# sthaha/kepler

Hardware: AMD Instinct MI355X
Metric: process attributions/sec + achieved HBM GB/s, 10k-node fleet, 1/2/4/8 MI355X (higher is better)
Workload: dtype f64+u64; 1 GPU; config3: 10000-node fleet x 2000 procs, Z=4; fleet_nodes=10000, nodes_per_gpu=10000, procs_per_gpu=20000000, containers_per_gpu=1970000, vms_per_gpu=200000, pods_per_gpu=700000, zones=4, namespaces=10000, allreduce_every=8

## Files before the change

kepler_amd/csrc/kacc_derive.hpp:

```cpp
#pragma once

#include <hip/hip_runtime.h>
#include <stdint.h>

#include "kacc_internal.hpp"

namespace kacc {

struct ProcDerive {
  const double *ratio;
  const uint32_t *node;
  const uint64_t *active_energy;
  const double *active_power;
  const double *cpu_delta;
  uint64_t nodes;
  uint32_t zones;
};

__device__ __forceinline__ double proc_power(const ProcDerive &d, uint64_t s, uint32_t z) {
  const uint32_t n = d.node[s];
  if (n >= d.nodes) return 0.0;
  const uint64_t i = static_cast<uint64_t>(n) * d.zones + z;
  const double aP = d.active_power[i];
  if (d.active_energy[i] == 0 || !(d.cpu_delta[n] != 0) || !(aP != 0)) return 0.0;
  return d.ratio[s] * aP;
}

}

inline kacc::ProcDerive kacc_derive(const kacc_ctx *ctx, kacc_kind kind) {
  kacc::ProcDerive d;
  const int tr = kind == KACC_KIND_CTR ? KACC_T_CTR_RATIO : kind == KACC_KIND_VM ? KACC_T_VM_RATIO : KACC_T_PROC_RATIO;
  d.ratio = static_cast<const double *>(ctx->tables[tr]);
  d.node = static_cast<const uint32_t *>(ctx->tables[tr + 1]);
  d.active_energy = static_cast<const uint64_t *>(ctx->tables[KACC_T_NODE_ACTIVE_ENERGY]);
  d.active_power = static_cast<const double *>(ctx->tables[KACC_T_NODE_ACTIVE_POWER]);
  d.cpu_delta = static_cast<const double *>(ctx->tables[KACC_T_NODE_CPU_DELTA]);
  d.nodes = ctx->cfg.nodes;
  d.zones = ctx->cfg.zones;
  return d;
}
inline kacc::ProcDerive kacc_proc_derive(const kacc_ctx *ctx) { return kacc_derive(ctx, KACC_KIND_PROC); }

inline int kacc_derived_kind(int t) {
  return t == KACC_T_PROC_POWER ? KACC_KIND_PROC : t == KACC_T_CTR_POWER ? KACC_KIND_CTR
                                                 : t == KACC_T_VM_POWER ? KACC_KIND_VM : -1;
}

extern "C" int kacc_internal_derived_power(kacc_ctx *ctx, int t, uint64_t first, uint64_t count, double *out,
                                           void *stream);
```

kepler_amd/csrc/kacc_device.hpp:

```cpp
#pragma once

#include <hip/hip_runtime.h>
#include <stdint.h>

namespace kacc {

constexpr double kTwo63 = 9223372036854775808.0;

__device__ __forceinline__ int64_t cvttsd2sq(double x) {
  if (!(x >= -kTwo63 && x < kTwo63)) return INT64_MIN;
  return static_cast<int64_t>(x);
}

__device__ __forceinline__ uint64_t go_f64_to_u64(double x) {
  if (__builtin_expect(x > -1.0 && x < 4294967296.0, 1)) return static_cast<uint32_t>(x);
  if (x < kTwo63) return static_cast<uint64_t>(cvttsd2sq(x));
  return static_cast<uint64_t>(cvttsd2sq(x - kTwo63)) | 0x8000000000000000ull;
}

__device__ __forceinline__ double u2f(uint64_t v) { return static_cast<double>(v); }

__device__ __forceinline__ int64_t go_sub_mono(int64_t t, int64_t u) {
  int64_t d;
  if (__builtin_sub_overflow(t, u, &d)) return t > u ? INT64_MAX : INT64_MIN;
  return d;
}

__device__ __forceinline__ double go_duration_seconds(int64_t d) {
  const int64_t sec = d / 1000000000LL;
  const int64_t nsec = d % 1000000000LL;
  return static_cast<double>(sec) + static_cast<double>(nsec) / 1e9;
}

__device__ __forceinline__ uint64_t energy_delta(uint64_t cur, uint64_t prev, uint64_t max_j) {
  if (cur >= prev) return cur - prev;
  if (max_j > 0) return (max_j - prev) + cur;
  return 0;
}

}
```

kepler_amd/csrc/kacc_engine.hip:

```cpp
#include <hip/hip_runtime.h>

#include <algorithm>
#include <atomic>
#include <thread>
#include <type_traits>
#include <cstdarg>
#include <cstddef>
#include <cstdio>
#include <cstring>
#include <mutex>
#include <string>
#include <vector>

#include "../../include/kepler_accel.h"
#include "kacc_debug.h"
#include "kacc_derive.hpp"
#include "kacc_device.hpp"
#include "kacc_internal.hpp"

namespace kacc {

constexpr int kTree = 256;
constexpr int kRowsLds = 2048;
constexpr int kBlock = 256;
// ... 51 lines not shown
#define KACC_CHUNK_WAVES 4
#endif
constexpr int kChunkThreads = KACC_CHUNK_THREADS;
constexpr int kChunkRpt = 4;
constexpr int kChunkRows = kChunkRpt * kChunkThreads;
static_assert(kChunkRows <= kRowsLds, "a chunk's rows are staged like a fast node's");
constexpr uint32_t kChunkGrid = 256u * 4u * KACC_CHUNK_WAVES / (kChunkThreads / 64);

template <int V>
constexpr int kTpb = 512;
template <int V>
constexpr int kRpt = kRowsLds / kTpb<V>;

constexpr uint32_t kErrNode = 1u << 0;
constexpr uint32_t kErrOffsets = 1u << 1;
constexpr uint32_t kErrSlot = 1u << 2;
constexpr uint32_t kErrNs = 1u << 3;
constexpr uint32_t kErrCapacity = 1u << 4;
constexpr uint32_t kErrBigNode = 1u << 5;
static_assert(kRowsLds == KACC_FAST_MAX_PROCS && kTpb<0> == KACC_FAST_MAX_AGGREGATES,
              "KACC_FAST_* must match the fast path's capacity");

struct ChunkItem {
  uint32_t node, chunk, nchunks, ctr_begin, vm_begin, pod_begin, pad[2];
};

constexpr int kColLoads = 8;
#ifndef KACC_COL_SPLIT_FROM
#define KACC_COL_SPLIT_FROM 16384
#endif
#ifndef KACC_COL_SPLIT_NODES
#define KACC_COL_SPLIT_NODES 4096
#endif
constexpr uint64_t kColSplitFrom = KACC_COL_SPLIT_FROM, kColSplitNodes = KACC_COL_SPLIT_NODES;
struct NodeTotalsArgs {
  uint64_t n_nodes;
  const uint64_t *active_total, *idle_total;
  const double *power, *active_power, *idle_power;
  const uint64_t *node_export;
  uint64_t *out_e;
  double *out_p;
  uint32_t split;
  uint64_t *part;
  uint32_t *arrived;
};

struct DevState {
  uint64_t *node_energy_total, *node_active_energy, *node_active_total, *node_idle_total;
  double *node_power, *node_active_power, *node_idle_power;
  int64_t *node_ts;
  uint32_t *node_has_prev;
  double *node_usage_ratio, *node_cpu_delta;
  uint32_t *node_status;
  uint64_t *proc_energy;
  double *proc_ratio;
  uint32_t *proc_node;
  uint64_t *ctr_energy;
  double *ctr_ratio, *ctr_cpu_delta, *ctr_cpu_total;
  uint32_t *ctr_node;
  uint64_t *vm_energy;
  double *vm_ratio, *vm_cpu_delta;
  uint32_t *vm_node;
  uint64_t *pod_energy;
  double *pod_power, *pod_cpu_delta, *pod_cpu_total;
  uint64_t proc_slots, ctr_slots, vm_slots, pod_slots;
  uint32_t *err;
  uint2 *defer;
  uint32_t *defer_ctr;
  uint32_t defer_cap;
  ChunkItem *items;
  uint32_t *item_ctr;
  uint32_t item_cap;
  uint32_t items_given, keep_items;
  uint64_t *stamps;
};

struct NodeShared {
  uint64_t active_energy[KACC_MAX_ZONES];
  double power[KACC_MAX_ZONES];
  double active_power[KACC_MAX_ZONES];
  double node_delta;
  uint32_t first;
};

__device__ __forceinline__ void raise_err(uint32_t *err, uint32_t bit) { atomicOr(err, bit); }

__device__ __forceinline__ uint64_t uniform_u64(uint64_t x) {
  const uint32_t lo = __builtin_amdgcn_readfirstlane(static_cast<uint32_t>(x));
  const uint32_t hi = __builtin_amdgcn_readfirstlane(static_cast<uint32_t>(x >> 32));
  return (static_cast<uint64_t>(hi) << 32) | lo;
}
__device__ __forceinline__ double uniform_f64(double x) {
  return __longlong_as_double(static_cast<long long>(uniform_u64(static_cast<uint64_t>(__double_as_longlong(x)))));
}
__device__ __forceinline__ uint32_t uniform_u32(uint32_t x) { return __builtin_amdgcn_readfirstlane(x); }

#ifndef KACC_FAST_EXTRA_LDS
#define KACC_FAST_EXTRA_LDS 0
#endif
#ifndef KACC_WT_PROC
#define KACC_WT_PROC 0
#endif
#ifndef KACC_WT_AGG
#define KACC_WT_AGG 0
#endif
template <typename T>
__device__ __forceinline__ void wt_store(T v, T *p) {
  if constexpr (sizeof(T) == 16)
    asm volatile("global_store_dwordx4 %0, %1, off sc0 sc1 nt" ::"v"(p), "v"(v) : "memory");
  else if constexpr (sizeof(T) == 8)
    asm volatile("global_store_dwordx2 %0, %1, off sc0 sc1 nt" ::"v"(p), "v"(v) : "memory");
  else
    asm volatile("global_store_dword %0, %1, off sc0 sc1 nt" ::"v"(p), "v"(v) : "memory");
}
template <typename T>
__device__ __forceinline__ void nt_store(T v, T *p) {
  if constexpr (KACC_WT_PROC != 0)
    wt_store(v, p);
  else
    __builtin_nontemporal_store(v, p);
}

template <int Z>
__device__ __forceinline__ void load_row(const uint64_t *__restrict__ base, uint64_t s,
                                         uint64_t (&out)[Z]) {
  if constexpr (Z % 2 == 0) {
    using u64x2 = __attribute__((ext_vector_type(2))) unsigned long long;
    const u64x2 *p = reinterpret_cast<const u64x2 *>(base + s * Z);
#pragma unroll
    for (int k = 0; k < Z / 2; ++k) {
      const u64x2 x = p[k];
      out[2 * k] = x.x;
      out[2 * k + 1] = x.y;
    }
  } else {
#pragma unroll
    for (int z = 0; z < Z; ++z) out[z] = base[s * Z + z];
  }
}

template <int Z>
__device__ __forceinline__ void load_row_f64(const double *__restrict__ base, uint64_t s,
                                             double (&out)[Z]) {
  if constexpr (Z % 2 == 0) {
    using f64x2 = __attribute__((ext_vector_type(2))) double;
    const f64x2 *p = reinterpret_cast<const f64x2 *>(base + s * Z);
#pragma unroll
    for (int k = 0; k < Z / 2; ++k) {
      const f64x2 x = p[k];
      out[2 * k] = x.x;
      out[2 * k + 1] = x.y;
    }
  } else {
#pragma unroll
    for (int z = 0; z < Z; ++z) out[z] = base[s * Z + z];
  }
}

template <int Z, bool NT, typename T>
__device__ __forceinline__ void store_row(T *__restrict__ base, uint64_t s, const T (&in)[Z]) {
  if constexpr (Z % 2 == 0) {
    using v2 = __attribute__((ext_vector_type(2))) T;
    v2 *p = reinterpret_cast<v2 *>(base + s * Z);
#pragma unroll
    for (int k = 0; k < Z / 2; ++k) {
      v2 x;
      x.x = in[2 * k];
      x.y = in[2 * k + 1];
      if constexpr (NT)
        nt_store(x, p + k);
      else
        p[k] = x;
    }
  } else {
#pragma unroll
    for (int z = 0; z < Z; ++z) {
      if constexpr (NT)
        nt_store(in[z], base + s * Z + z);
      else
        base[s * Z + z] = in[z];
    }
  }
}

constexpr uint64_t kPodRowScale = 2;
__device__ __forceinline__ uint64_t pod_row(uint64_t s) { return s * kPodRowScale; }
__device__ __forceinline__ uint64_t agg_row(uint32_t role, uint64_t s) { return role == 3 ? pod_row(s) : s; }

template <int Z>
struct Attr {
  uint64_t aE[Z];
  double aP[Z];
  uint32_t live;
  uint32_t live_pod;
  double nd;
  uint32_t first;
  uint32_t keep_node;
};

template <int Z>
__device__ __forceinline__ Attr<Z> make_attr(const NodeShared &sh, uint32_t flags) {
  Attr<Z> a;
  a.nd = uniform_f64(sh.node_delta);
  a.first = uniform_u32(sh.first);
  a.keep_node = (flags & KACC_F_STABLE_SLOT_NODES) && !a.first ? 1u : 0u;
  a.live = 0;
  a.live_pod = 0;
#pragma unroll
  for (int z = 0; z < Z; ++z) {
    a.aE[z] = uniform_u64(sh.active_energy[z]);
    a.aP[z] = uniform_f64(sh.active_power[z]);
    const double pw = uniform_f64(sh.power[z]);
    const bool ok = a.aE[z] != 0 && a.nd != 0;
    if (ok && a.aP[z] != 0) a.live |= 1u << z;
    if (ok && (a.first ? a.aP[z] : pw) != 0) a.live_pod |= 1u << z;
  }
  return a;
}

template <int Z>
__device__ __forceinline__ double attribute_row(const Attr<Z> &a, uint32_t live, double delta,
                                                bool is_new, const uint64_t (&prev)[Z],
                                                uint64_t (&E)[Z], double (&P)[Z]) {
  const double ratio = delta / a.nd;
#pragma unroll
  for (int z = 0; z < Z; ++z) {
    if (live & (1u << z)) {
      const uint64_t e = go_f64_to_u64(ratio * u2f(a.aE[z]));
      E[z] = a.first ? e : e + (is_new ? 0ull : prev[z]);
      P[z] = a.first ? 0.0 : ratio * a.aP[z];
    } else {
      E[z] = 0;
      P[z] = 0.0;
    }
  }
  return ratio;
}

template <int Z>
__device__ __forceinline__ double attribute_proc(const Attr<Z> &a, double delta, bool is_new,
                                                 const uint64_t (&prev)[Z], uint64_t (&E)[Z]) {
  const double ratio = delta / a.nd;
#pragma unroll
  for (int z = 0; z < Z; ++z) {
    if (a.live & (1u << z)) {
      const uint64_t e = go_f64_to_u64(ratio * u2f(a.aE[z]));
      E[z] = a.first ? e : e + (is_new ? 0ull : prev[z]);
    } else {
      E[z] = 0;
    }
  }
  return ratio;
}

template <int Z, bool NT>
__device__ __forceinline__ void store_proc(const DevState &st, uint64_t s, const uint64_t (&E)[Z], double ratio,
                                           uint32_t node, bool wnode) {
  store_row<Z, NT, uint64_t>(st.proc_energy, s, E);
  if constexpr (NT) {
    nt_store(ratio, st.proc_ratio + s);
    if (wnode) nt_store(node, st.proc_node + s);
  } else {
    st.proc_ratio[s] = ratio;
    if (wnode) st.proc_node[s] = node;
  }
}

__device__ __forceinline__ uint32_t export_row(const kacc_interval &b, uint32_t q, uint32_t *err) {
  if (!b.pod_export_pos) return q;
  const uint32_t r = b.pod_export_pos[q];
  if (r >= b.n_pods) {
    atomicOr(err, 1u << 1);
    return ~0u;
  }
  return r;
}
template <int Z>
__device__ __forceinline__ void export_pod_at(const kacc_interval &b, uint32_t row, const uint64_t (&E)[Z],
                                              const double (&P)[Z]) {
  if (!b.pod_export || row == ~0u) return;
  uint64_t *o = b.pod_export + static_cast<uint64_t>(row) * (2 * Z);
  store_row<Z, false, uint64_t>(o, 0, E);
  store_row<Z, false, double>(reinterpret_cast<double *>(o), 1, P);
}
template <int Z>
__device__ __forceinline__ void export_pod(const kacc_interval &b, uint32_t q, const uint64_t (&E)[Z],
                                           const double (&P)[Z], uint32_t *err) {
  if (!b.pod_export) return;
  export_pod_at<Z>(b, export_row(b, q, err), E, P);
}
template <int Z>
__device__ __forceinline__ void export_pod_zero(const kacc_interval &b, uint32_t q, uint32_t *err) {
  uint64_t E[Z];
  double P[Z];
#pragma unroll
  for (int z = 0; z < Z; ++z) {
    E[z] = 0;
    P[z] = 0.0;
  }
  export_pod<Z>(b, q, E, P, err);
}
template <int Z>
__device__ __forceinline__ void export_node_zone(const kacc_interval &b, uint32_t n, uint32_t z, uint64_t at,
                                                 uint64_t it, double p, double ap, double ip) {
  if (!b.node_export) return;
  uint64_t *o = b.node_export + static_cast<uint64_t>(n) * (5 * Z) + z;
  o[0] = at;
  o[Z] = it;
  o[2 * Z] = static_cast<uint64_t>(__double_as_longlong(p));
  o[3 * Z] = static_cast<uint64_t>(__double_as_longlong(ap));
  o[4 * Z] = static_cast<uint64_t>(__double_as_longlong(ip));
// ... 23 lines not shown
  if constexpr (KACC_WT_AGG != 0 && !NT) {
    if (role == 3) {
      wt_row<Z, uint64_t>(st.pod_energy, pod_row(s), E);
      wt_row<Z, double>(st.pod_power, pod_row(s), P);
      return;
    }
    wt_row<Z, uint64_t>(role == 1 ? st.ctr_energy : st.vm_energy, s, E);
    wt_store(ratio, (role == 1 ? st.ctr_ratio : st.vm_ratio) + s);
    wt_store(node, (role == 1 ? st.ctr_node : st.vm_node) + s);
    return;
  }
  if (role == 3) {
    store_row<Z, NT, uint64_t>(st.pod_energy, pod_row(s), E);
    store_row<Z, NT, double>(st.pod_power, pod_row(s), P);
    return;
  }
  store_row<Z, NT, uint64_t>(role == 1 ? st.ctr_energy : st.vm_energy, s, E);
  double *r = role == 1 ? st.ctr_ratio : st.vm_ratio;
  uint32_t *nd = role == 1 ? st.ctr_node : st.vm_node;
  if constexpr (NT) {
    nt_store(ratio, r + s);
    nt_store(node, nd + s);
  } else {
    r[s] = ratio;
    nd[s] = node;
  }
}

template <int kB>
__device__ __forceinline__ void segment_load(const double *s_d, uint32_t i, uint32_t e, double (&v)[kB]) {
#pragma unroll
  for (int u = 0; u < kB; ++u) v[u] = s_d[min(i + u, e - 1)];
}
template <int kB>
__device__ __forceinline__ void segment_add(const double (&v)[kB], uint32_t i, uint32_t e, double &delta,
                                            double &total) {
#pragma unroll
  for (int u = 0; u < kB; ++u) {
    const double x = i + u < e ? v[u] : 0.0;
    delta = delta + x;
    total = total + x;
  }
}
template <int kB>
__device__ __forceinline__ void segment_sum(const double *s_d, uint32_t i, uint32_t e, double &delta,
                                            double &total) {
  for (; i < e; i += kB) {
    double v[kB];
    segment_load<kB>(s_d, i, e, v);
    segment_add<kB>(v, i, e, delta, total);
  }
}
template <int Z, bool kMasked, bool kNtLoad = false>
__device__ __forceinline__ void load_group_masked(const uint64_t *__restrict__ base, uint64_t s0,
                                                  uint32_t len, uint64_t safe, uint64_t (&out)[Z]) {
  using u64x2 = __attribute__((ext_vector_type(2))) unsigned long long;
  constexpr int kHalf = Z / 2;
  const uint32_t lane = threadIdx.x & 63u;
  const u64x2 *p = reinterpret_cast<const u64x2 *>(base + s0 * Z);
  const u64x2 *q = reinterpret_cast<const u64x2 *>(base + safe * Z);
#pragma unroll
  for (int j = 0; j < kHalf; ++j) {
    const uint32_t piece = lane + 64u * j;
    if constexpr (!kMasked) {
      const u64x2 x = kNtLoad ? __builtin_nontemporal_load(p + piece) : p[piece];
      out[2 * j] = x.x;
      out[2 * j + 1] = x.y;
      continue;
    }
    const bool ok = piece / kHalf < len;
    const u64x2 *src = ok ? p + piece : q;
    const u64x2 x = kNtLoad ? __builtin_nontemporal_load(src) : *src;
    out[2 * j] = ok ? x.x : 0ull;
    out[2 * j + 1] = ok ? x.y : 0ull;
  }
}

template <int Z, bool NT, bool kInv>
__device__ __forceinline__ void attribute_group_masked(const Attr<Z> &a, const NodeShared &sh,
                                                       const double *s_d, const uint32_t *s_w,
                                                       const uint16_t *s_inv,
                                                       uint32_t row0, uint64_t s0, uint32_t len,
                                                       const uint64_t (&prev)[Z],
                                                       uint64_t *__restrict__ energy,
                                                       double *__restrict__ ratio_tab,
                                                       uint32_t *__restrict__ node_tab, uint32_t node) {
  using u64x2 = __attribute__((ext_vector_type(2))) unsigned long long;
  constexpr int kHalf = Z / 2;
  const uint32_t lane = threadIdx.x & 63u;
  u64x2 *pe = reinterpret_cast<u64x2 *>(energy + s0 * Z);
#pragma unroll
  for (int j = 0; j < kHalf; ++j) {
    const uint32_t piece = lane + 64u * j;
    const uint32_t idx = piece / kHalf;
    const uint32_t zp = piece % kHalf;
    uint32_t row = row0 + idx;
    if constexpr (kInv) {
      if (idx >= len) continue;
      row = s_inv[row];
      if (row == 0xffffu) continue;
    }
    const uint32_t wr = s_w[row];
    const bool is_new = (wr & KACC_SLOT_NEW) != 0;
    const double ratio = s_d[row] / a.nd;
    uint64_t E[2];
#pragma unroll
    for (int h = 0; h < 2; ++h) {
      const uint32_t z = 2 * zp + h;
      const uint64_t aE = sh.active_energy[z];
      if (a.live & (1u << z)) {
        const uint64_t e = go_f64_to_u64(ratio * u2f(aE));
        E[h] = a.first ? e : e + (is_new ? 0ull : prev[2 * j + h]);
      } else {
        E[h] = 0;
      }
    }
    u64x2 ev;
    ev.x = E[0];
    ev.y = E[1];
    if constexpr (NT)
      nt_store(ev, pe + piece);
    else
      pe[piece] = ev;
    if (zp == 0) {
      const bool wnode = !a.keep_node || is_new;
      if constexpr (NT) {
        nt_store(ratio, ratio_tab + s0 + idx);
        if (wnode) nt_store(node, node_tab + s0 + idx);
      } else {
        ratio_tab[s0 + idx] = ratio;
        if (wnode) node_tab[s0 + idx] = node;
      }
    }
  }
}

template <int Z>
__device__ __forceinline__ void node_zone(const kacc_interval &b, const DevState &st, uint32_t n,
                                          int z, NodeShared &sh) {
  const bool first = st.node_has_prev[n] == 0u;
  const uint64_t i = static_cast<uint64_t>(n) * Z + z;
  const double ratio = b.node_usage_ratio[n];
  const uint64_t abs_e = b.zone_energy[i];
  uint64_t active;
  double p = 0.0, ap = 0.0, ip = 0.0;
  uint64_t at, it;
  if (first) {
    active = go_f64_to_u64(u2f(abs_e) * ratio);
    at = active;
    it = abs_e - active;
  } else {
    const double dt = go_duration_seconds(go_sub_mono(b.node_ts_ns[n], st.node_ts[n]));
    const uint64_t delta = energy_delta(abs_e, st.node_energy_total[i], b.zone_max[i]);
    active = go_f64_to_u64(u2f(delta) * ratio);
    at = st.node_active_total[i] + active;
    it = st.node_idle_total[i] + (delta - active);
    p = u2f(delta) / dt;
    ap = p * ratio;
    ip = p - ap;
  }
  st.node_active_total[i] = at;
  st.node_idle_total[i] = it;
  export_node_zone<Z>(b, n, static_cast<uint32_t>(z), at, it, p, ap, ip);
  st.node_energy_total[i] = abs_e;
  st.node_active_energy[i] = active;
  st.node_power[i] = p;
  st.node_active_power[i] = ap;
  st.node_idle_power[i] = ip;
  sh.active_energy[z] = active;
  sh.power[z] = p;
  sh.active_power[z] = ap;
  if (z == 0) sh.first = first ? 1u : 0u;
}

struct NodeRanges {
  uint32_t p0, p1, c0, c1, v0, v1, q0, q1;
};

template <int Z>
__device__ __forceinline__ void export_skipped(const kacc_interval &b, const DevState &st, uint32_t n,
                                               const NodeRanges &r, uint32_t lane, uint32_t nlanes) {
  if (b.node_export) {
    for (uint32_t z = lane; z < static_cast<uint32_t>(Z); z += nlanes) {
      const uint64_t i = static_cast<uint64_t>(n) * Z + z;
      export_node_zone<Z>(b, n, z, st.node_active_total[i], st.node_idle_total[i], st.node_power[i],
                          st.node_active_power[i], st.node_idle_power[i]);
    }
// ... 295 lines not shown
  double d[kRowsPerThread];
  uint32_t w[kRowsPerThread];
#pragma unroll
  for (int k = 0; k < kRowsPerThread; ++k) {
    const uint32_t r = tid + k * kThreads;
    const bool in = r < rows;
    if constexpr (kNtLd) {
      d[k] = in ? __builtin_nontemporal_load(dcpu + r) : 0.0;
      w[k] = in ? __builtin_nontemporal_load(pslot + r) : 0xffffffffu;
    } else {
      d[k] = in ? dcpu[r] : 0.0;
      w[k] = in ? pslot[r] : 0xffffffffu;
    }
  }
  const uint32_t utid = static_cast<uint32_t>(tid);
  auto role_of = [&]() -> uint32_t {
    if ((V & kVarSkipAggregates) != 0) return 0u;
    return utid < nc ? 1u : utid < nc + nv ? 2u : utid < nc + nv + nq ? 3u : 0u;
  };
  auto index_of = [&]() -> uint32_t {
    return utid < nc ? utid : utid < nc + nv ? utid - nc : utid - nc - nv;
  };
  uint32_t a_beg = 0, a_end = 0, a_w = 0xffffffffu;
  {
    const uint32_t role = role_of(), j = index_of();
    if (role == 1) {
      a_beg = j == 0 ? p0 : b.ctr_proc_end[c0 + j - 1];
      a_end = b.ctr_proc_end[c0 + j];
      a_w = b.ctr_slot[c0 + j];
    } else if (role == 2) {
      a_beg = j == 0 ? (nc ? b.ctr_proc_end[c1 - 1] : p0) : b.vm_proc_end[v0 + j - 1];
      a_end = b.vm_proc_end[v0 + j];
      a_w = b.vm_slot[v0 + j];
    } else if (role == 3) {
      a_beg = j == 0 ? c0 : b.pod_ctr_end[q0 + j - 1];
      a_end = b.pod_ctr_end[q0 + j];
      a_w = b.pod_slot[q0 + j];
    }
  }
  auto a_cap = [&]() -> uint64_t {
    const uint32_t role = role_of();
    return role == 1 ? st.ctr_slots : role == 2 ? st.vm_slots : role == 3 ? st.pod_slots : 0;
  };
  const uint32_t a_s = a_w & KACC_SLOT_MASK;
  auto a_ok_f = [&]() -> bool { return role_of() != 0 && a_s < a_cap(); };
  const bool a_ok = a_ok_f();
  const uint32_t role = role_of();
  const uint32_t j = index_of();
  auto a_energy = [&]() { return role == 1 ? st.ctr_energy : role == 2 ? st.vm_energy : st.pod_energy; };
  auto a_cpu_total = [&]() { return role == 1 ? st.ctr_cpu_total : st.pod_cpu_total; };
  auto a_cpu_delta = [&]() {
    return role == 1 ? st.ctr_cpu_delta : role == 2 ? st.vm_cpu_delta : st.pod_cpu_delta;
  };
  uint64_t prev[kRowsPerThread][Z];
  uint32_t contig = 0;
  constexpr bool kSweepable =
      kTransposed<Z> && (V & (kVarNoTranspose | kVarNoSweep | kVarSkipProcs)) == 0;
  constexpr bool kRowSweep = !kTransposed<Z> && (V & (kVarNoSweep | kVarSkipProcs)) == 0;
  uint32_t smin = 0, span = 0;
  bool sweep = false;
  if constexpr (kSweepable || kRowSweep) {
    if (b.node_proc_span) {
      const uint32_t lo = uniform_u32(b.node_proc_span[2 * n]);
      const uint32_t hi = uniform_u32(b.node_proc_span[2 * n + 1]);
      sweep = rows > 0 && hi >= lo && hi - lo < static_cast<uint32_t>(kRowsLds) && hi < st.proc_slots;
      smin = lo;
      span = hi - lo + 1;
      if (sweep) {
#pragma unroll
        for (int k = 0; k < kRowsPerThread; ++k) s_inv[tid + k * kThreads] = 0xffffu;
      }
    }
  }
  const bool swept = (kSweepable || kRowSweep) && sweep;
  if constexpr ((V & kVarSkipProcs) == 0) {
    if (swept) {
      if constexpr (kRowSweep) {
#pragma unroll
        for (int k = 0; k < kRowsPerThread; ++k)
          load_row<Z>(st.proc_energy, static_cast<uint64_t>(smin) + min(tid + k * kThreads, span - 1), prev[k]);
      }
      if constexpr (kSweepable) {
#pragma unroll
        for (int k = 0; k < kRowsPerThread; ++k) {
          const uint32_t pos0 = static_cast<uint32_t>(tid & ~63) + k * kThreads;
          const uint32_t len = pos0 < span ? min(span - pos0, 64u) : 0u;
          load_group_masked<Z, true, kNtLd>(st.proc_energy, static_cast<uint64_t>(smin) + pos0, len, smin,
                                     prev[k]);
        }
      }
    } else {
#pragma unroll
      for (int k = 0; k < kRowsPerThread; ++k) {
        const uint64_t sl = w[k] & KACC_SLOT_MASK;
        if constexpr (kTransposed<Z> && (V & kVarNoTranspose) == 0) {
          const uint64_t g0 = uniform_u32(static_cast<uint32_t>(sl));
          if (__all((tid + k * kThreads) < rows && sl == g0 + (tid & 63) && g0 + 64 <= st.proc_slots)) {
            contig |= 1u << k;
            load_group_masked<Z, false, kNtLd>(st.proc_energy, g0, 64u, g0, prev[k]);
            continue;
          }
        }
        if (sl < st.proc_slots) {
          load_row<Z>(st.proc_energy, sl, prev[k]);
        } else {
#pragma unroll
          for (int z = 0; z < Z; ++z) prev[k][z] = 0;
        }
      }
    }
  }
  uint64_t a_prev[Z];
  double a_total = 0.0;
  if (a_ok) {
    if constexpr (!kLateAgg<V>) load_row<Z>(a_energy(), agg_row(role, a_s), a_prev);
    if (role != 2 && !(a_w & KACC_SLOT_NEW)) a_total = a_cpu_total()[a_s];
  } else {
#pragma unroll
    for (int z = 0; z < Z; ++z) a_prev[z] = 0;
  }
  if (role != 0 && !a_ok) raise_err(st.err, kErrSlot);

#pragma unroll
  for (int k = 0; k < kRowsPerThread; ++k) {
    const uint32_t r = tid + k * kThreads;
    if (r < rows) {
      s_d[r] = d[k];
      s_w[r] = w[k];
    }
  }
  __syncthreads();
  if constexpr (kStamp) {
    if (tid == 0) stamp[1] = __builtin_amdgcn_s_memrealtime();
  }
  if (swept) {
#pragma unroll
    for (int k = 0; k < kRowsPerThread; ++k) {
      const uint32_t r = tid + k * kThreads;
      if (r >= rows) continue;
      const uint32_t sl = s_w[r] & KACC_SLOT_MASK;
      if (sl - smin < span && sl < st.proc_slots)
        s_inv[sl - smin] = static_cast<uint16_t>(r);
      else
        raise_err(st.err, kErrSlot);
    }
  }
  if (b.flags & KACC_F_NODE_CPU_DELTA_GIVEN) {
    if (tid == 0) sh.node_delta = b.node_cpu_delta[n];
  } else {
    if (tid < kTree) {
      double v[kRowsLds / kTree];
#pragma unroll
      for (int u = 0; u < kRowsLds / kTree; ++u) v[u] = s_d[tid + kTree * u];
      double s = 0.0;
#pragma unroll
      for (int u = 0; u < kRowsLds / kTree; ++u) s = s + (tid + kTree * u < rows ? v[u] : 0.0);
      red[tid] = s;
// ... 56 lines not shown
    st.node_ts[n] = b.node_ts_ns[n];
    st.node_has_prev[n] = 1u;
    st.node_usage_ratio[n] = a.first ? 0.0 : b.node_usage_ratio[n];
    st.node_cpu_delta[n] = a.nd;
    st.node_status[n] = a.first ? KACC_NODE_FIRST_READ : KACC_NODE_OK;
  }
  constexpr uint32_t kStageWords = kRowsLds;
  const bool stage = kLateAgg<V> && (V & kVarSkipAggregates) == 0 && b.pod_export && !b.pod_export_pos &&
                     nq * 2u * Z <= kStageWords;
  uint64_t *s_stage = reinterpret_cast<uint64_t *>(s_d);
  auto aggregate_out = [&]() {
    if (!a_ok) {
      if (role == 3) {
        if (stage) {
#pragma unroll
          for (int z = 0; z < 2 * Z; ++z) s_stage[j * 2 * Z + z] = 0;
        } else {
          export_pod_zero<Z>(b, q0 + j, st.err);
        }
      }
      return;
    }
    if constexpr (kLateAgg<V>) load_row<Z>(a_energy(), agg_row(role, a_s), a_prev);
    const uint32_t xrow = role == 3 && b.pod_export && !stage ? export_row(b, q0 + j, st.err) : ~0u;
    uint64_t E[Z];
    double P[Z];
    const double ratio = attribute_row<Z>(a, role == 3 ? a.live_pod : a.live, a_delta,
                                          (a_w & KACC_SLOT_NEW) != 0, a_prev, E, P);
    store_agg<Z, kNtAgg>(st, role, a_s, E, P, ratio, n);
    if (role == 3) {
      if (stage) {
#pragma unroll
        for (int z = 0; z < Z; ++z) {
          s_stage[j * 2 * Z + z] = E[z];
          s_stage[j * 2 * Z + Z + z] = static_cast<uint64_t>(__double_as_longlong(P[z]));
        }
      } else {
        export_pod_at<Z>(b, xrow, E, P);
      }
    }
  };
  if constexpr (!kLateAgg<V>) aggregate_out();
  if (swept) {
    if constexpr (kRowSweep) {
#pragma unroll
      for (int k = 0; k < kRowsPerThread; ++k) {
        const uint32_t pos = tid + k * kThreads;
        if (pos >= span) continue;
        const uint32_t r = s_inv[pos];
        if (r == 0xffffu) continue;
        const uint32_t wk = s_w[r];
        uint64_t E[Z];
        const double ratio = attribute_proc<Z>(a, s_d[r], (wk & KACC_SLOT_NEW) != 0, prev[k], E);
        store_proc<Z, kNT>(st, static_cast<uint64_t>(smin) + pos, E, ratio, n, !a.keep_node || (wk & KACC_SLOT_NEW));
      }
    }
    if constexpr (kSweepable) {
#pragma unroll
      for (int k = 0; k < kRowsPerThread; ++k) {
        const uint32_t pos0 = static_cast<uint32_t>(tid & ~63) + k * kThreads;
        const uint32_t len = pos0 < span ? min(span - pos0, 64u) : 0u;
        attribute_group_masked<Z, kNT, true>(a, sh, s_d, s_w, s_inv, pos0,
                                             static_cast<uint64_t>(smin) + pos0, len, prev[k],
                                             st.proc_energy, st.proc_ratio, st.proc_node, n);
      }
    }
  } else if constexpr ((V & kVarSkipProcs) == 0) {
#pragma unroll
    for (int k = 0; k < kRowsPerThread; ++k) {
      const uint32_t r = tid + k * kThreads;
      if constexpr (kTransposed<Z> && (V & kVarNoTranspose) == 0) {
        if (contig & (1u << k)) {
          const uint32_t pos0 = r - (tid & 63);
          attribute_group_masked<Z, kNT, false>(a, sh, s_d, s_w, s_inv, pos0,
                                                uniform_u32(s_w[pos0] & KACC_SLOT_MASK), 64u, prev[k],
                                                st.proc_energy, st.proc_ratio, st.proc_node, n);
          continue;
        }
      }
      if (r >= rows) continue;
      const uint32_t wk = s_w[r];
      const uint64_t sl = wk & KACC_SLOT_MASK;
      if (sl >= st.proc_slots) {
        raise_err(st.err, kErrSlot);
        continue;
      }
      uint64_t E[Z];
      const double ratio = attribute_proc<Z>(a, s_d[r], (wk & KACC_SLOT_NEW) != 0, prev[k], E);
      store_proc<Z, kNtScat>(st, sl, E, ratio, n, !a.keep_node || (wk & KACC_SLOT_NEW));
    }
  }
  if (stage) __syncthreads();
  if constexpr (kLateAgg<V>) aggregate_out();
  if (stage) {
    __syncthreads();
    using u64x2 = __attribute__((ext_vector_type(2))) unsigned long long;
    const u64x2 *src = reinterpret_cast<const u64x2 *>(s_stage);
    u64x2 *dst = reinterpret_cast<u64x2 *>(b.pod_export + static_cast<uint64_t>(q0) * (2 * Z));
    for (uint32_t i = utid; i < nq * Z; i += kThreads) nt_store(src[i], dst + i);
  }
  if constexpr (kStamp) {
    __syncthreads();
    if (tid == 0) stamp[3] = __builtin_amdgcn_s_memrealtime();
  }
}

template <int Z, int V>
#ifndef KACC_FAST_WAVES
#define KACC_FAST_WAVES 6
#endif
__global__ __launch_bounds__(kTpb<V>, Z > 4 ? 2 : KACC_FAST_WAVES)
void interval_kernel(const kacc_interval b, const DevState st) {
  interval_node<Z, V>(b, st, blockIdx.x);
}

template <int Z, int V>
__global__ __launch_bounds__(kTpb<V>, Z > 4 ? 2 : KACC_FAST_WAVES)
void interval_sums_kernel(const kacc_interval b, const DevState st, const SumsArgs sa) {
  if (blockIdx.x < sa.node_blocks) {
    sums_block<Z, kTpb<V>>(sa, blockIdx.x, st.err);
    return;
  }
  const uint32_t x = blockIdx.x - sa.node_blocks;
  if (x >= b.n_nodes) {
    sums_block<Z, kTpb<V>>(sa, sa.node_blocks + (x - b.n_nodes), st.err);
    return;
  }
  interval_node<Z, V>(b, st, x);
}

constexpr int kCarryMaxZ = 2;

__device__ __forceinline__ void lds_barrier() {
  __builtin_amdgcn_fence(__ATOMIC_RELEASE, "workgroup", "local");
  __builtin_amdgcn_s_barrier();
  __builtin_amdgcn_fence(__ATOMIC_ACQUIRE, "workgroup", "local");
}

#define KACC_GLOBAL __attribute__((address_space(1)))
template <typename T>
__device__ __forceinline__ const T KACC_GLOBAL *gbl(const T *p) {
  return (const T KACC_GLOBAL *)p;
// ... 247 lines not shown
#pragma unroll
    for (int j = 0; j < kR; ++j) {
      const uint32_t r = tid + j * kThreads;
      if (r < rows && fits) {
        s_d[r] = rw.d[j];
        s_w[r] = rw.w[j];
        if (sweep) {
          const uint32_t pos = (rw.w[j] & KACC_SLOT_MASK) - s_lo;
          if (process && pos < span)
            s_inv[pos] = static_cast<uint16_t>(r);
          else
            outside = process;
        } else {
          moved |= (rw.w[j] & KACC_SLOT_MASK) != (s_cw[r] & KACC_SLOT_MASK);
        }
      }
    }
    if (outside) raise_err(st.err, kErrSlot);
    const uint32_t flags = b.flags;
    if constexpr (kPrefetch) {
      const uint32_t k1 = min(k + 1, K - 1);
      uint32_t bad;
      load_rows<Z, T>(bs[k1], carry_ranges(bs[k1], tab.off + (k1 - c) * 8, bad), rw);
    }
    if (bad_offsets) {
      if (tid == 0) raise_err(st.err, kErrOffsets);
    }
    if (status & KACC_NODE_READ_ERROR) {
      if (tid == 0) st.node_status[n] = KACC_NODE_SKIPPED;
    } else if (!fits) {
      if (tid == 0) raise_err(st.err, kErrBigNode);
    } else {
      const uint32_t role = (V & kCarryNoAggregates) ? 0u : is_c ? 1u : is_v ? 2u : is_q ? 3u : 0u;
      const uint32_t a_s = a_w & KACC_SLOT_MASK;
      const uint64_t a_cap = role == 1 ? st.ctr_slots : role == 2 ? st.vm_slots : role == 3 ? st.pod_slots : 0;
      const bool a_ok = role != 0 && a_s < a_cap;
      if (role != 0 && !a_ok) raise_err(st.err, kErrSlot);
      const bool a_moved = a_ok && (role != c_role || a_s != (c_aw & KACC_SLOT_MASK));
      moved |= a_moved;
      if (__any(moved) && (tid & 63) == 0) s_moved = 1u;
      const bool load_window = sweep && c_sbase != s_lo;
      mark(0);
      lds_barrier();
      mark(1);
      if (((V & kCarryNeverMoved) == 0 && s_moved) || load_window) {
        __syncthreads();
        if (load_window) {
#pragma unroll
          for (int j = 0; j < kR; ++j) {
            const uint32_t pos = tid + j * kThreads;
            const uint64_t sl = static_cast<uint64_t>(s_lo) + pos;
            uint64_t pv[Z];
            if (sl < st.proc_slots) {
              load_row<Z>(st.proc_energy, sl, pv);
#pragma unroll
              for (int z = 0; z < Z; ++z) s_cE[pos * Z + z] = pv[z];
            }
          }
          c_sbase = s_lo;
        } else if (!sweep) {
#pragma unroll
          for (int j = 0; j < kR; ++j) {
            const uint32_t r = tid + j * kThreads;
            if (r >= rows) continue;
            const uint32_t sw = s_w[r];
            const uint64_t sl = sw & KACC_SLOT_MASK;
            if (sl == (s_cw[r] & KACC_SLOT_MASK)) continue;
            uint64_t pv[Z];
            if (sl < st.proc_slots) {
              load_row<Z>(st.proc_energy, sl, pv);
            } else {
#pragma unroll
              for (int z = 0; z < Z; ++z) pv[z] = 0;
            }
#pragma unroll
            for (int z = 0; z < Z; ++z) s_cE[r * Z + z] = pv[z];
          }
        }
        if (a_moved) {
          load_row<Z>(role == 1 ? st.ctr_energy : role == 2 ? st.vm_energy : st.pod_energy, agg_row(role, a_s), c_aE);
          c_atotal = role == 1 ? st.ctr_cpu_total[a_s] : role == 3 ? st.pod_cpu_total[a_s] : 0.0;
        }
        lds_barrier();
        if (tid == 0) s_moved = 0;
      }
      double a_total = (role != 2 && a_ok && !(a_w & KACC_SLOT_NEW)) ? c_atotal : 0.0;

      const bool first = c_has_prev == 0u;
      uint64_t z_active = 0;
      double z_p = 0.0, z_ap = 0.0, z_ip = 0.0;
      if (tid < static_cast<uint32_t>(Z)) {
        const uint64_t c_etot = s_zc[tid];
        uint64_t c_atot = s_zc[Z + tid], c_itot = s_zc[2 * Z + tid];
        if (first) {
          z_active = go_f64_to_u64(u2f(ze) * ratio);
          c_atot = z_active;
          c_itot = ze - z_active;
        } else {
          const double dt = go_duration_seconds(go_sub_mono(ts, c_ts));
          const uint64_t delta = energy_delta(ze, c_etot, zm);
          z_active = go_f64_to_u64(u2f(delta) * ratio);
          c_atot = c_atot + z_active;
          c_itot = c_itot + (delta - z_active);
          z_p = u2f(delta) / dt;
          z_ap = z_p * ratio;
          z_ip = z_p - z_ap;
        }
        s_zc[tid] = ze;
        s_zc[Z + tid] = c_atot;
        s_zc[2 * Z + tid] = c_itot;
        sh.active_energy[tid] = z_active;
        sh.power[tid] = z_p;
        sh.active_power[tid] = z_ap;
        if (tid == 0) sh.first = first ? 1u : 0u;
      }
      if (flags & KACC_F_NODE_CPU_DELTA_GIVEN) {
        if (tid == 0) sh.node_delta = nd_given;
      } else if (tid >= static_cast<uint32_t>(kThreads - 64)) {
        const uint32_t t = tid - (kThreads - 64);
        constexpr int kU = kRows / kTree, kB = kU < 4 ? kU : 4;
        double leaf[4];
#pragma unroll
        for (int q = 0; q < 4; ++q) {
// ... 53 lines not shown
      mark(4);
      if (tid < static_cast<uint32_t>(Z)) {
        st.node_active_total[zi] = s_zc[Z + tid];
        st.node_idle_total[zi] = s_zc[2 * Z + tid];
        st.node_energy_total[zi] = ze;
        st.node_active_energy[zi] = z_active;
        st.node_power[zi] = z_p;
        st.node_active_power[zi] = z_ap;
        st.node_idle_power[zi] = z_ip;
      }
      const Attr<Z> a = make_attr<Z>(sh, b.flags);
      if (tid == 0) {
        st.node_ts[n] = ts;
        st.node_has_prev[n] = 1u;
        st.node_usage_ratio[n] = a.first ? 0.0 : ratio;
        st.node_cpu_delta[n] = a.nd;
        st.node_status[n] = a.first ? KACC_NODE_FIRST_READ : KACC_NODE_OK;
      }
      if (a_ok) {
        if (role == 1) {
          st.ctr_cpu_delta[a_s] = a_delta;
          st.ctr_cpu_total[a_s] = a_total;
        } else if (role == 2) {
          st.vm_cpu_delta[a_s] = a_delta;
        } else {
          st.pod_cpu_delta[a_s] = a_delta;
          st.pod_cpu_total[a_s] = a_total;
        }
        uint64_t E[Z];
        double P[Z];
        const double ratio =
            attribute_row<Z>(a, role == 3 ? a.live_pod : a.live, a_delta, (a_w & KACC_SLOT_NEW) != 0, c_aE, E, P);
        store_agg<Z, kNtAggStores || (V & kCarryNtAgg) != 0>(st, role, a_s, E, P, ratio, n);
#pragma unroll
        for (int z = 0; z < Z; ++z) c_aE[z] = E[z];
        c_atotal = a_total;
      }
      c_role = a_ok ? role : 0u;
      c_aw = a_ok ? a_w : 0xffffffffu;
      if (sweep) {
#pragma unroll
        for (int j = 0; j < kR; ++j) {
          const uint32_t pos = tid + j * kThreads;
          if (pos >= span) continue;
          const uint32_t r = s_inv[pos];
          if (r == 0xffffu) continue;
          s_inv[pos] = 0xffffu;
          const uint32_t wk = s_w[r];
          uint64_t pv[Z], E[Z];
#pragma unroll
          for (int z = 0; z < Z; ++z) pv[z] = s_cE[pos * Z + z];
          const double ratio = attribute_proc<Z>(a, s_d[r], (wk & KACC_SLOT_NEW) != 0, pv, E);
          if constexpr ((V & kCarryNoRowStores) == 0) {
            store_proc<Z, true>(st, static_cast<uint64_t>(s_lo) + pos, E, ratio, n, !a.keep_node || (wk & KACC_SLOT_NEW));
          }
#pragma unroll
          for (int z = 0; z < Z; ++z) s_cE[pos * Z + z] = E[z];
        }
      } else {
#pragma unroll
      for (int j = 0; j < kR; ++j) {
        const uint32_t r = tid + j * kThreads;
        if (r >= rows) {
          s_cw[r] = 0xffffffffu;
          continue;
        }
        const uint32_t wk = s_w[r];
        const uint64_t sl = wk & KACC_SLOT_MASK;
        if (sl >= st.proc_slots) {
          raise_err(st.err, kErrSlot);
          s_cw[r] = 0xffffffffu;
          continue;
        }
        uint64_t pv[Z], E[Z];
#pragma unroll
        for (int z = 0; z < Z; ++z) pv[z] = s_cE[r * Z + z];
        const double ratio = attribute_proc<Z>(a, s_d[r], (wk & KACC_SLOT_NEW) != 0, pv, E);
        if constexpr ((V & kCarryNoRowStores) == 0) {
          store_proc<Z, kNtScatterStores>(st, sl, E, ratio, n, !a.keep_node || (wk & KACC_SLOT_NEW));
        }
#pragma unroll
        for (int z = 0; z < Z; ++z) s_cE[r * Z + z] = E[z];
        s_cw[r] = wk;
      }
      }
      c_has_prev = 1u;
      c_ts = ts;
    }
    mark(5);
    lds_barrier();
    mark(6);
  }
  if constexpr ((V & kCarryStamps) != 0) {
    if ((tid & 63u) == 0) {
      uint64_t *out = reinterpret_cast<uint64_t *>(st.items) + (static_cast<uint64_t>(n) * 8 + tid / 64) * kCarryPhases;
#pragma unroll
      for (int ph = 0; ph < kCarryPhases; ++ph) out[ph] = t_acc[ph];
    }
  }
}

constexpr int kSmallRows = 512;
constexpr int kSmallAgg = 128;
constexpr int kSmallWaves = 4;
constexpr int kSmallGroups = kSmallRows / 64;
constexpr int kSmallBatch = 4;
static_assert(kSmallRows == KACC_SMALL_MAX_PROCS && kSmallAgg == KACC_SMALL_MAX_AGGREGATES,
              "KACC_SMALL_* must match the small-node kernel's capacity");
static_assert(kSmallRows <= 2 * kTree && kSmallGroups == 2 * kSmallBatch && kSmallAgg == 128,
              "small-node tree / batch / aggregate loops assume these sizes");

__device__ __forceinline__ void wave_sync() {
  __builtin_amdgcn_fence(__ATOMIC_RELEASE, "wavefront");
  __builtin_amdgcn_wave_barrier();
  __builtin_amdgcn_fence(__ATOMIC_ACQUIRE, "wavefront");
}

template <int Z, bool SW>
constexpr int kSmallWavesPerEu = Z <= 3 ? (SW || Z == 3 ? 5 : 6) : Z == 4 ? 4 : 1;
template <int Z, bool SW>
__global__ __launch_bounds__(64 * kSmallWaves) __attribute__((amdgpu_waves_per_eu(kSmallWavesPerEu<Z, SW>))) void small_kernel(
    const kacc_interval b, const DevState st) {
  constexpr bool kNT = true, kNtLd = true;
  __shared__ double s_d_all[kSmallWaves][kSmallRows];
  constexpr bool kSweepable = kTransposed<Z>;
  constexpr bool kRowSweep = SW && !kTransposed<Z>;
  __shared__ uint32_t s_w_all[kSmallWaves][kSweepable ? kSmallRows : 1];
  __shared__ double s_cd_all[kSmallWaves][kSmallAgg];
  __shared__ double s_ct_all[kSmallWaves][kSmallAgg];
  __shared__ uint16_t s_inv_all[kSmallWaves][kSmallRows];
  __shared__ NodeShared sh_all[kSmallWaves];

// ... 9 lines not shown
  if (blockIdx.x == 0 && threadIdx.x == 0) st.defer_ctr[0] = 0u;
  const uint32_t idx = blockIdx.x * kSmallWaves + wv;
  if (idx >= b.n_nodes) return;
  const uint32_t n = b.node_order ? uniform_u32(b.node_order[idx]) : idx;
  if (n >= b.n_nodes) {
    if (lane == 0) raise_err(st.err, kErrNode);
    return;
  }
  uint32_t status;
  NodeRanges raw;
  node_words(b, n, status, raw);
  if (status & KACC_NODE_READ_ERROR) {
    if (lane == 0) st.node_status[n] = KACC_NODE_SKIPPED;
    if (b.pod_export || b.node_export)
      export_skipped<Z>(b, st, n, clamp_ranges(b, st, raw, static_cast<int>(lane)), lane, 64u);
    return;
  }
  const NodeRanges rg = clamp_ranges(b, st, raw, static_cast<int>(lane));
  const uint32_t p0 = rg.p0, p1 = rg.p1, c0 = rg.c0, c1 = rg.c1, q0 = rg.q0, q1 = rg.q1;
  const uint32_t rows = p1 - p0, nc = c1 - c0, nv = rg.v1 - rg.v0, nq = q1 - q0;
  if (rows > static_cast<uint32_t>(kSmallRows) || nc + nv + nq > static_cast<uint32_t>(kSmallAgg)) {
    if (lane == 0) raise_err(st.err, kErrBigNode);
    return;
  }

  if (lane < static_cast<uint32_t>(Z)) node_zone<Z>(b, st, n, static_cast<int>(lane), sh);

  const double *__restrict__ dcpu = b.proc_cpu_delta + p0;
  const uint32_t *__restrict__ pslot = b.proc_slot + p0;
  double d[kSmallGroups];
  uint32_t w[kSmallGroups];
#pragma unroll
  for (int k = 0; k < kSmallGroups; ++k) {
    const uint32_t r = lane + 64u * k;
    const bool in = r < rows;
    d[k] = in ? __builtin_nontemporal_load(dcpu + r) : 0.0;
    w[k] = in ? __builtin_nontemporal_load(pslot + r) : 0xffffffffu;
  }
  uint32_t smin = 0, span = 0;
  bool swept = false;
  if constexpr (kSweepable || kRowSweep) {
    if (b.node_proc_span) {
      const uint32_t lo = uniform_u32(b.node_proc_span[2 * n]);
      const uint32_t hi = uniform_u32(b.node_proc_span[2 * n + 1]);
      swept = rows > 0 && hi >= lo && hi - lo < static_cast<uint32_t>(kSmallRows) && hi < st.proc_slots;
      smin = lo;
      span = hi - lo + 1;
      if (swept) {
#pragma unroll
        for (int k = 0; k < kSmallGroups; ++k) s_inv[lane + 64u * k] = 0xffffu;
      }
    }
  }
  uint64_t prev[kSmallBatch][Z];
  uint32_t contig = 0;
  auto load_batch = [&](int kb, bool from_regs) {
    contig = 0;
#pragma unroll
    for (int g = 0; g < kSmallBatch; ++g) {
      const int k = kb * kSmallBatch + g;
      const uint32_t pos0 = 64u * k;
      if constexpr (kRowSweep) {
        if (swept) {
          load_row<Z>(st.proc_energy, static_cast<uint64_t>(smin) + min(pos0 + lane, span - 1), prev[g]);
          continue;
        }
      }
      if constexpr (kSweepable) {
        if (swept) {
          const uint32_t len = pos0 < span ? min(span - pos0, 64u) : 0u;
          load_group_masked<Z, true, kNtLd>(st.proc_energy, static_cast<uint64_t>(smin) + pos0, len, smin,
                                            prev[g]);
          continue;
        }
      }
      const uint32_t r = pos0 + lane;
      const uint32_t wk = (from_regs || !kSweepable) ? w[k] : (r < rows ? s_w[r] : 0xffffffffu);
      const uint64_t sl = wk & KACC_SLOT_MASK;
      if constexpr (kTransposed<Z>) {
        const uint64_t g0 = uniform_u32(static_cast<uint32_t>(sl));
        if (__all(r < rows && sl == g0 + lane && g0 + 64 <= st.proc_slots)) {
          contig |= 1u << g;
          load_group_masked<Z, false, kNtLd>(st.proc_energy, g0, 64u, g0, prev[g]);
          continue;
        }
      }
      if (r < rows && sl < st.proc_slots) {
        load_row<Z>(st.proc_energy, sl, prev[g]);
      } else {
#pragma unroll
        for (int z = 0; z < Z; ++z) prev[g][z] = 0;
      }
    }
  };
  load_batch(0, true);

  auto role_of = [&](uint32_t i) -> uint32_t {
    return i < nc ? 1u : i < nc + nv ? 2u : i < nc + nv + nq ? 3u : 0u;
  };
  auto index_of = [&](uint32_t i) -> uint32_t { return i < nc ? i : i < nc + nv ? i - nc : i - nc - nv; };
  auto cap_of = [&](uint32_t role) -> uint64_t {
    return role == 1 ? st.ctr_slots : role == 2 ? st.vm_slots : role == 3 ? st.pod_slots : 0;
  };
  auto energy_of = [&](uint32_t role) { return role == 1 ? st.ctr_energy : role == 2 ? st.vm_energy : st.pod_energy; };
  auto cpu_total_of = [&](uint32_t role) { return role == 1 ? st.ctr_cpu_total : st.pod_cpu_total; };
  auto cpu_delta_of = [&](uint32_t role) {
    return role == 1 ? st.ctr_cpu_delta : role == 2 ? st.vm_cpu_delta : st.pod_cpu_delta;
  };
  uint32_t a_beg[2], a_end[2], a_w[2];
  uint64_t a_prev[2][Z];
  double a_total[2], a_delta[2];
#pragma unroll
  for (int h = 0; h < 2; ++h) {
    const uint32_t i = lane + 64u * h, role = role_of(i), j = index_of(i);
    a_beg[h] = a_end[h] = 0;
    a_w[h] = 0xffffffffu;
    if (role == 1) {
      a_beg[h] = j == 0 ? p0 : b.ctr_proc_end[c0 + j - 1];
      a_end[h] = b.ctr_proc_end[c0 + j];
      a_w[h] = b.ctr_slot[c0 + j];
    } else if (role == 2) {
      a_beg[h] = j == 0 ? (nc ? b.ctr_proc_end[c1 - 1] : p0) : b.vm_proc_end[rg.v0 + j - 1];
      a_end[h] = b.vm_proc_end[rg.v0 + j];
      a_w[h] = b.vm_slot[rg.v0 + j];
    } else if (role == 3) {
      a_beg[h] = j == 0 ? c0 : b.pod_ctr_end[q0 + j - 1];
      a_end[h] = b.pod_ctr_end[q0 + j];
      a_w[h] = b.pod_slot[q0 + j];
    }
    const uint32_t a_s = a_w[h] & KACC_SLOT_MASK;
    const bool a_ok = role != 0 && a_s < cap_of(role);
    a_total[h] = 0.0;
    a_delta[h] = 0.0;
    if (a_ok) {
      load_row<Z>(energy_of(role), agg_row(role, a_s), a_prev[h]);
      if (role != 2 && !(a_w[h] & KACC_SLOT_NEW)) a_total[h] = cpu_total_of(role)[a_s];
    } else {
#pragma unroll
      for (int z = 0; z < Z; ++z) a_prev[h][z] = 0;
    }
    if (role != 0 && !a_ok) raise_err(st.err, kErrSlot);
// ... 96 lines not shown
    }
    double ad = 0.0, at = a_total[h];
    for (uint32_t c = beg - c0; c < end - c0; ++c) {
      ad = ad + s_cd[c];
      at = at + s_ct[c];
    }
    a_delta[h] = ad;
    a_total[h] = at;
    if (a_s < st.pod_slots) {
      st.pod_cpu_delta[a_s] = ad;
      st.pod_cpu_total[a_s] = at;
    }
  }

  const Attr<Z> a = make_attr<Z>(sh, KACC_SMALL_STABLE ? b.flags : (b.flags & ~KACC_F_STABLE_SLOT_NODES));
  if (lane == 0) {
    st.node_ts[n] = b.node_ts_ns[n];
    st.node_has_prev[n] = 1u;
    st.node_usage_ratio[n] = a.first ? 0.0 : b.node_usage_ratio[n];
    st.node_cpu_delta[n] = a.nd;
    st.node_status[n] = a.first ? KACC_NODE_FIRST_READ : KACC_NODE_OK;
  }
  auto aggregate_out = [&]() {
#pragma unroll
    for (int h = 0; h < 2; ++h) {
      const uint32_t i = lane + 64u * h, role = role_of(i);
      const uint32_t a_s = a_w[h] & KACC_SLOT_MASK;
      if (role == 0) continue;
      if (a_s >= cap_of(role)) {
        if (role == 3) export_pod_zero<Z>(b, q0 + index_of(i), st.err);
        continue;
      }
      uint64_t E[Z];
      double P[Z];
      const double ratio = attribute_row<Z>(a, role == 3 ? a.live_pod : a.live, a_delta[h],
                                            (a_w[h] & KACC_SLOT_NEW) != 0, a_prev[h], E, P);
      store_agg<Z, kNT && kNtAggStores>(st, role, a_s, E, P, ratio, n);
      if (role == 3) export_pod<Z>(b, q0 + index_of(i), E, P, st.err);
    }
  };
  if constexpr (KACC_SMALL_LATE_AGG == 0) aggregate_out();
  auto attr_batch = [&](int kb) {
#pragma unroll
    for (int g = 0; g < kSmallBatch; ++g) {
      const uint32_t pos0 = 64u * (kb * kSmallBatch + g);
      if constexpr (kRowSweep) {
        if (swept) {
          const uint32_t pos = pos0 + lane;
          if (pos >= span) continue;
          const uint32_t e = s_inv[pos];
          if (e == 0xffffu) continue;
          uint64_t E[Z];
          const double ratio = attribute_proc<Z>(a, s_d[e & 0x7fffu], (e & 0x8000u) != 0, prev[g], E);
          store_proc<Z, kNT>(st, static_cast<uint64_t>(smin) + pos, E, ratio, n, !a.keep_node || (e & 0x8000u));
          continue;
        }
      }
      if constexpr (kSweepable) {
        if (swept) {
          const uint32_t len = pos0 < span ? min(span - pos0, 64u) : 0u;
          attribute_group_masked<Z, kNT, true>(a, sh, s_d, s_w, s_inv, pos0, static_cast<uint64_t>(smin) + pos0,
                                               len, prev[g], st.proc_energy, st.proc_ratio, st.proc_node, n);
          continue;
        }
        if (contig & (1u << g)) {
          attribute_group_masked<Z, kNT, false>(a, sh, s_d, s_w, s_inv, pos0,
                                                uniform_u32(s_w[pos0] & KACC_SLOT_MASK), 64u, prev[g],
                                                st.proc_energy, st.proc_ratio, st.proc_node, n);
          continue;
        }
      }
      const uint32_t r = pos0 + lane;
      if (r >= rows) continue;
      uint32_t wk;
      if constexpr (kSweepable)
        wk = s_w[r];
      else
        wk = kb == 0 ? w[g] : w[kSmallBatch + g];
      const uint64_t sl = wk & KACC_SLOT_MASK;
      if (sl >= st.proc_slots) {
        raise_err(st.err, kErrSlot);
        continue;
      }
      uint64_t E[Z];
      const double ratio = attribute_proc<Z>(a, s_d[r], (wk & KACC_SLOT_NEW) != 0, prev[g], E);
      store_proc<Z, kNT && kNtScatterStores>(st, sl, E, ratio, n, !a.keep_node || (wk & KACC_SLOT_NEW));
    }
  };
  attr_batch(0);
  const uint32_t extent = swept ? span : rows;
  if (extent > 64u * kSmallBatch) {
    load_batch(1, false);
    attr_batch(1);
  }
  if constexpr (KACC_SMALL_LATE_AGG != 0) aggregate_out();
}

template <int V, uint32_t kGen>
__device__ __forceinline__ void gen_items(const kacc_interval &b, const DevState &st, uint32_t n,
                                          const NodeRanges &rg, uint32_t base, uint32_t nch, uint32_t g) {
  constexpr int kScan = 4;
  const uint32_t p0 = rg.p0, p1 = rg.p1;
  ChunkItem *__restrict__ items = st.items + base;
  const uint32_t c0 = rg.c0, c1 = rg.c1, v0 = rg.v0, v1 = rg.v1, q0 = rg.q0, q1 = rg.q1;
  auto clampr = [&](uint32_t x) { return min(max(x, p0), p1); };
  auto clampc = [&](uint32_t x) { return min(max(x, c0), c1); };
  auto chunk_of = [&](uint32_t start) -> int {
    return static_cast<int>(min((start - p0) / kChunkRows, nch - 1));
  };
  const uint32_t ctr_rows_end = c1 > c0 ? clampr(b.ctr_proc_end[c1 - 1]) : p0;
  auto mark = [&](uint32_t i, int kc, int kp, uint32_t ChunkItem::*field) {
    if (kc < kp) raise_err(st.err, kErrOffsets);
    for (int k = kp + 1; k <= kc; ++k) items[k].*field = i;
  };
  for (uint32_t cb = c0 + g; cb < ((V & kVarBigNoScan) ? c0 : c1); cb += kGen * kScan) {
    uint32_t e1[kScan], e2[kScan];
#pragma unroll
    for (int u = 0; u < kScan; ++u) {
      const uint32_t c = cb + u * kGen;
      e1[u] = (c < c1 && c > c0) ? b.ctr_proc_end[c - 1] : p0;
      e2[u] = (c < c1 && c > c0 + 1) ? b.ctr_proc_end[c - 2] : p0;
    }
#pragma unroll
    for (int u = 0; u < kScan; ++u) {
      const uint32_t c = cb + u * kGen;
      if (c >= c1) continue;
      mark(c, chunk_of(clampr(e1[u])), c > c0 ? chunk_of(clampr(e2[u])) : -1,
           &ChunkItem::ctr_begin);
    }
  }
  for (uint32_t vb = v0 + g; vb < ((V & kVarBigNoScan) ? v0 : v1); vb += kGen * kScan) {
    uint32_t e1[kScan], e2[kScan];
#pragma unroll
    for (int u = 0; u < kScan; ++u) {
      const uint32_t v = vb + u * kGen;
      e1[u] = (v < v1 && v > v0) ? b.vm_proc_end[v - 1] : ctr_rows_end;
      e2[u] = (v < v1 && v > v0 + 1) ? b.vm_proc_end[v - 2] : ctr_rows_end;
    }
#pragma unroll
// ... 185 lines not shown
      f[2] = w0[2];
      f[3] = w0[3];
      f[4] = w0[4];
      f[5] = w0[5];
      f[6] = w1[3];
      f[7] = w1[4];
      f[8] = w1[5];
      asm volatile("" ::"v"(f[0]), "v"(f[1]), "v"(f[2]), "v"(f[3]), "v"(f[4]), "v"(f[5]), "v"(f[6]), "v"(f[7]),
                   "v"(f[8]));
#pragma unroll
      for (int q = 0; q < 9; ++q) f[q] = uniform_u32(f[q]);
    }
    const uint32_t n = f[0], k = f[1], nch = f[2];
    if (n >= b.n_nodes) {
      if (tid == 0) raise_err(st.err, kErrCapacity);
      __syncthreads();
      idx = uniform_u32(s_next[parity]);
      continue;
    }
    uint32_t status;
    NodeRanges raw;
    node_words(b, n, status, raw);
    if (status & KACC_NODE_READ_ERROR) {
      __syncthreads();
      idx = uniform_u32(s_next[parity]);
      continue;
    }
    const NodeRanges rg = clamp_ranges(b, st, raw, tid);
    const bool last = k + 1 >= nch;
    const uint32_t lo = min(rg.p0 + min(k, nch) * static_cast<uint32_t>(kChunkRows), rg.p1);
    const uint32_t hi = last ? rg.p1 : min(lo + static_cast<uint32_t>(kChunkRows), rg.p1);
    const uint32_t rows = hi - lo;
    const uint32_t cb = min(max(f[3], rg.c0), rg.c1);
    const uint32_t ce = max(min(last ? rg.c1 : f[6], rg.c1), cb);
    const uint32_t vb = min(max(f[4], rg.v0), rg.v1);
    const uint32_t ve = max(min(last ? rg.v1 : f[7], rg.v1), vb);
    const uint32_t qb = min(max(f[5], rg.q0), rg.q1);
    const uint32_t qe = max(min(last ? rg.q1 : f[8], rg.q1), qb);
    const uint32_t nca = kAgg ? ce - cb : 0u;
    const uint32_t ncv = kAgg ? nca + (ve - vb) : 0u;
    const uint32_t nagg = kAgg ? ncv + (qe - qb) : 0u;

    const double *__restrict__ dcpu = b.proc_cpu_delta + lo;
    const uint32_t *__restrict__ pslot = b.proc_slot + lo;
    double d[kR];
    uint32_t w[kR];
#pragma unroll
    for (int u = 0; u < kR; ++u) {
      const uint32_t r = utid + u * kThreads;
      const bool in = r < rows;
      d[u] = in ? (kNtLd ? __builtin_nontemporal_load(dcpu + r) : dcpu[r]) : 0.0;
      w[u] = in ? (kNtLd ? __builtin_nontemporal_load(pslot + r) : pslot[r]) : 0xffffffffu;
    }
    uint64_t prev[kR][Z];
    uint32_t contig = 0;
    if constexpr ((V & kVarSkipProcs) == 0) {
#pragma unroll
      for (int u = 0; u < kR; ++u) {
        const uint64_t sl = w[u] & KACC_SLOT_MASK;
        if constexpr (kT) {
          const uint64_t s0 = uniform_u32(static_cast<uint32_t>(sl));
          const bool mine = (utid + u * kThreads) < rows && sl == s0 + (tid & 63) &&
                            s0 + 64 <= st.proc_slots;
          if (__all(mine)) {
            contig |= 1u << u;
            load_group_masked<Z, false, kNtLd>(st.proc_energy, s0, 64u, s0, prev[u]);
            continue;
          }
        }
        if (sl < st.proc_slots) {
          load_row<Z>(st.proc_energy, sl, prev[u]);
        } else {
#pragma unroll
          for (int z = 0; z < Z; ++z) prev[u][z] = 0;
        }
      }
    }
    const uint32_t ctr_rows_end = rg.c1 > rg.c0 ? b.ctr_proc_end[rg.c1 - 1] : rg.p0;
    auto agg = [&](uint32_t j, uint32_t &beg, uint32_t &end, uint32_t &wd) -> uint32_t {
      if (j < nca) {
        const uint32_t c = cb + j;
        beg = c == rg.c0 ? rg.p0 : b.ctr_proc_end[c - 1];
        end = b.ctr_proc_end[c];
        wd = b.ctr_slot[c];
        return 1u;
      }
      if (j < ncv) {
        const uint32_t v = vb + (j - nca);
        beg = v == rg.v0 ? ctr_rows_end : b.vm_proc_end[v - 1];
        end = b.vm_proc_end[v];
        wd = b.vm_slot[v];
        return 2u;
      }
      const uint32_t q = qb + (j - ncv);
      beg = q == rg.q0 ? rg.c0 : b.pod_ctr_end[q - 1];
      end = b.pod_ctr_end[q];
      wd = b.pod_slot[q];
      return 3u;
    };
    auto cap_of = [&](uint32_t role) {
      return role == 1 ? st.ctr_slots : role == 2 ? st.vm_slots : st.pod_slots;
    };
    auto energy_of = [&](uint32_t role) {
      return role == 1 ? st.ctr_energy : role == 2 ? st.vm_energy : st.pod_energy;
    };
    uint32_t a_role = 0, a_beg = 0, a_end = 0, a_w = 0xffffffffu;
    if (utid < nagg) a_role = agg(utid, a_beg, a_end, a_w);
    const uint32_t a_s = a_w & KACC_SLOT_MASK;
    const bool a_ok = a_role != 0 && a_s < cap_of(a_role);
    uint64_t a_prev[Z];
    double a_total = 0.0;
    if (a_ok) {
      load_row<Z>(energy_of(a_role), agg_row(a_role, a_s), a_prev);
      if (a_role != 2 && !(a_w & KACC_SLOT_NEW))
        a_total = (a_role == 1 ? st.ctr_cpu_total : st.pod_cpu_total)[a_s];
    } else {
#pragma unroll
      for (int z = 0; z < Z; ++z) a_prev[z] = 0;
    }
    if (a_role != 0 && !a_ok) raise_err(st.err, kErrSlot);
    node_params_to_lds<Z>(st, n, tid, sh);
#pragma unroll
    for (int u = 0; u < kR; ++u) {
      const uint32_t r = utid + u * kThreads;
// ... 49 lines not shown
      a_delta = segment(a_role, a_beg, a_end, a_w, a_ok, a_total);
      if (a_role == 1) {
        s_cd[utid] = a_ok ? a_delta : 0.0;
        s_ct[utid] = a_ok ? a_total : 0.0;
      }
    }
    __syncthreads();
    bool defer = false;
    if (a_role == 3) {
      uint32_t beg = a_beg, end = a_end;
      if (beg < rg.c0 || end < beg || end > rg.c1) {
        raise_err(st.err, kErrOffsets);
        beg = max(min(beg, rg.c1), rg.c0);
        end = max(min(end, rg.c1), beg);
      }
      if (end <= ce && end - cb <= static_cast<uint32_t>(kThreads) && beg >= cb) {
        for (uint32_t c = beg - cb; c < end - cb; ++c) {
          a_delta = a_delta + s_cd[c];
          a_total = a_total + s_ct[c];
        }
        if (a_ok) {
          st.pod_cpu_delta[a_s] = a_delta;
          st.pod_cpu_total[a_s] = a_total;
        }
      } else {
        defer = true;
      }
    }
    if (a_ok && !defer) {
      const uint64_t s = a_w & KACC_SLOT_MASK;
      uint64_t E[Z];
      double P[Z];
      const double ratio =
          attribute_row<Z>(a, a_role == 3 ? a.live_pod : a.live, a_delta, (a_w & KACC_SLOT_NEW) != 0, a_prev, E, P);
      store_agg<Z, kNT>(st, a_role, s, E, P, ratio, n);
      if (a_role == 3) export_pod<Z>(b, qb + (utid - ncv), E, P, st.err);
    } else if (a_role == 3 && !a_ok) {
      export_pod_zero<Z>(b, qb + (utid - ncv), st.err);
    }
    if (defer && a_ok) {
      const uint32_t i = atomicAdd(st.defer_ctr, 1u);
      if (i < st.defer_cap)
        st.defer[i] = make_uint2(n, qb + (utid - ncv));
      else
        raise_err(st.err, kErrCapacity);
    }
    if constexpr ((V & kVarSkipProcs) == 0) {
#pragma unroll
      for (int u = 0; u < kR; ++u) {
        const uint32_t r = utid + u * kThreads;
        if constexpr (kT) {
          if (contig & (1u << u)) {
            const uint32_t g = r - (tid & 63);
            attribute_group_masked<Z, kNT, false>(a, sh, s_d, s_w, nullptr, g,
                                           uniform_u32(s_w[g] & KACC_SLOT_MASK), 64u, prev[u],
                                           st.proc_energy, st.proc_ratio, st.proc_node, n);
            continue;
          }
        }
        if (r >= rows) continue;
        const uint32_t wk = s_w[r];
        const uint64_t sl = wk & KACC_SLOT_MASK;
        if (sl >= st.proc_slots) {
          raise_err(st.err, kErrSlot);
          continue;
        }
        uint64_t E[Z];
        const double ratio = attribute_proc<Z>(a, s_d[r], (wk & KACC_SLOT_NEW) != 0, prev[u], E);
        store_proc<Z, kNT && kNtScatterStores>(st, sl, E, ratio, n, !a.keep_node || (wk & KACC_SLOT_NEW));
      }
    }
    for (uint32_t j = kThreads + utid; j < nagg; j += kThreads) {
      uint32_t beg, end, wd;
      const uint32_t role = agg(j, beg, end, wd);
      const uint64_t s = wd & KACC_SLOT_MASK;
      const bool ok = s < cap_of(role);
      if (!ok) {
        raise_err(st.err, kErrSlot);
        if (role == 3) export_pod_zero<Z>(b, qb + (j - ncv), st.err);
        continue;
      }
      if (role == 3) {
        const uint32_t i = atomicAdd(st.defer_ctr, 1u);
        if (i < st.defer_cap)
          st.defer[i] = make_uint2(n, qb + (j - ncv));
        else
          raise_err(st.err, kErrCapacity);
        continue;
      }
      uint64_t pv[Z];
      load_row<Z>(energy_of(role), agg_row(role, s), pv);
      double total = (role == 1 && !(wd & KACC_SLOT_NEW)) ? st.ctr_cpu_total[s] : 0.0;
      const double delta = segment(role, beg, end, wd, true, total);
      agg_out(role, wd, delta, pv);
    }
    __syncthreads();
    idx = uniform_u32(s_next[parity]);
  }
}

template <int Z, int V>
__global__ __launch_bounds__(kBlock) void pod_kernel(const kacc_interval b, const DevState st) {
  constexpr bool kNT = (V & kVarTemporalStores) == 0;
  const int tid = threadIdx.x;
  if (blockIdx.x == 0 && tid == 0) {
    if (!st.keep_items) st.item_ctr[0] = 0u;
    st.item_ctr[1] = 0u;
  }
  const uint32_t count = min(st.defer_ctr[0], st.defer_cap);
  for (uint32_t i = blockIdx.x * kBlock + tid; i < count; i += gridDim.x * kBlock) {
    const uint2 e = st.defer[i];
    const uint32_t n = e.x, q = e.y;
    if (n >= b.n_nodes || q >= b.n_pods) {
      raise_err(st.err, kErrCapacity);
      continue;
    }
    const NodeRanges rg = node_ranges(b, st, n, 1);
    uint32_t beg = q == rg.q0 ? rg.c0 : b.pod_ctr_end[q - 1];
    uint32_t end = b.pod_ctr_end[q];
    beg = max(min(beg, rg.c1), rg.c0);
    end = max(min(end, rg.c1), beg);
    const uint32_t w = b.pod_slot[q];
// ... 53 lines not shown
  node_column_block<Z, kSplit>(na, blockIdx.x, s_w);
}


constexpr int kPowWaves = kBlock / 64;
template <int Z>
__global__ __launch_bounds__(kBlock) void proc_power_kernel(const ProcDerive d, uint64_t first, uint64_t count,
                                                            double *out) {
  __shared__ double s_p[kPowWaves][64 * Z];
  const uint32_t wv = threadIdx.x >> 6, lane = threadIdx.x & 63u;
  const uint64_t s_first = first / Z, s_last = (first + count - 1) / Z;
  const uint64_t S0 = s_first + (static_cast<uint64_t>(blockIdx.x) * kPowWaves + wv) * 64u;
  if (S0 > s_last) return;
  const uint64_t s = min(S0 + lane, s_last);
  const uint32_t n = d.node[s];
  const double r = d.ratio[s];
  double *const sp = s_p[wv];
  if (n < d.nodes) {
    const bool busy = d.cpu_delta[n] != 0;
#pragma unroll
    for (int z = 0; z < Z; ++z) {
      const uint64_t k = static_cast<uint64_t>(n) * Z + z;
      const double aP = d.active_power[k];
      sp[lane * Z + z] = (d.active_energy[k] != 0 && busy && aP != 0) ? r * aP : 0.0;
    }
  } else {
#pragma unroll
    for (int z = 0; z < Z; ++z) sp[lane * Z + z] = 0.0;
  }
  __builtin_amdgcn_fence(__ATOMIC_RELEASE, "wavefront");
  __builtin_amdgcn_wave_barrier();
  __builtin_amdgcn_fence(__ATOMIC_ACQUIRE, "wavefront");
  const uint64_t e0 = S0 * Z, end = first + count;
#pragma unroll
  for (int z = 0; z < Z; ++z) {
    const uint64_t e = e0 + static_cast<uint64_t>(z) * 64u + lane;
    if (e >= first && e < end) __builtin_nontemporal_store(sp[z * 64 + lane], out + (e - first));
  }
}

__global__ __launch_bounds__(kBlock) void pod_pair_copy_kernel(uint64_t *base, uint32_t Z, uint64_t first,
                                                               uint64_t count, uint64_t *dense, int to_table) {
  for (uint64_t i = static_cast<uint64_t>(blockIdx.x) * kBlock + threadIdx.x; i < count;
       i += static_cast<uint64_t>(gridDim.x) * kBlock) {
    const uint64_t e = first + i;
    uint64_t *p = base + (e / Z) * (2ull * Z) + e % Z;
    if (to_table)
      *p = dense[i];
    else
      dense[i] = *p;
  }
}

}

namespace {

std::mutex g_err_mu;
std::string g_create_error;

struct TableDesc {
  uint32_t elem;
  int per;
  bool zoned;
  bool derived;
};

const TableDesc kTables[KACC_T_COUNT] = {
    {8, 0, true, false},  {8, 0, true, false},  {8, 0, true, false},  {8, 0, true, false},
    {8, 0, true, false},  {8, 0, true, false},  {8, 0, true, false},  {8, 0, false, false},
    {4, 0, false, false}, {8, 0, false, false}, {8, 0, false, false}, {4, 0, false, false},
    {8, 1, true, false},  {8, 1, true, true},   {8, 2, true, false},  {8, 2, true, true},
    {8, 2, false, false}, {8, 2, false, false}, {8, 3, true, false},  {8, 3, true, true},
    {8, 3, false, false}, {8, 4, true, false},  {8, 4, true, false},  {8, 4, false, false},
    {8, 4, false, false}, {8, 1, false, false}, {4, 1, false, false}, {8, 2, false, false},
    {4, 2, false, false}, {8, 3, false, false}, {4, 3, false, false},
};
static_assert(KACC_T_PROC_POWER == 13 && KACC_T_PROC_RATIO == 25 && KACC_T_PROC_NODE == 26 &&
                  KACC_T_CTR_RATIO == 27 && KACC_T_VM_NODE == 30 && KACC_T_COUNT == 31,
              "kTables rows follow the kacc_table enum");

}

int kacc_fail(kacc_ctx *ctx, int code, const char *fmt, ...) {
  char buf[512];
  va_list ap;
  va_start(ap, fmt);
  vsnprintf(buf, sizeof(buf), fmt, ap);
  va_end(ap);
  if (ctx) {
    ctx->err = buf;
  } else {
    std::lock_guard<std::mutex> lk(g_err_mu);
    g_create_error = buf;
  }
  return code;
}

namespace {

#define fail kacc_fail

bool pod_paired(int t) { return t == KACC_T_POD_ENERGY || t == KACC_T_POD_POWER; }

uint64_t table_count(const kacc_config &c, int t);
size_t table_alloc_bytes(const kacc_ctx *ctx, int t) {
  const size_t n = std::max<uint64_t>(ctx->counts[t], 1) * kTables[t].elem;
  return t == KACC_T_POD_ENERGY ? 2 * n : n;
}

uint64_t table_count(const kacc_config &c, int t) {
  const TableDesc &d = kTables[t];
  uint64_t base = 0;
  switch (d.per) {
    case 0: base = c.nodes; break;
    case 1: base = c.proc_slots; break;
    case 2: base = c.ctr_slots; break;
    case 3: base = c.vm_slots; break;
    default: base = c.pod_slots; break;
  }
  return d.zoned ? base * c.zones : base;
}

constexpr size_t kColArrivedBytes = 5 * KACC_MAX_ZONES * sizeof(uint32_t);
size_t col_part_bytes(uint64_t nodes) {
  const uint64_t split = std::max<uint64_t>((nodes + kacc::kColSplitNodes - 1) / kacc::kColSplitNodes, 1);
  return 5 * KACC_MAX_ZONES * split * sizeof(uint64_t);
}

kacc::DevState dev_state(const kacc_ctx *ctx) {
  kacc::DevState s;
  auto T = [ctx](int t) { return ctx->tables[t]; };
  s.node_energy_total = (uint64_t *)T(KACC_T_NODE_ENERGY_TOTAL);
  s.node_active_energy = (uint64_t *)T(KACC_T_NODE_ACTIVE_ENERGY);
  s.node_active_total = (uint64_t *)T(KACC_T_NODE_ACTIVE_TOTAL);
  s.node_idle_total = (uint64_t *)T(KACC_T_NODE_IDLE_TOTAL);
  s.node_power = (double *)T(KACC_T_NODE_POWER);
  s.node_active_power = (double *)T(KACC_T_NODE_ACTIVE_POWER);
  s.node_idle_power = (double *)T(KACC_T_NODE_IDLE_POWER);
  s.node_ts = (int64_t *)T(KACC_T_NODE_TS);
  s.node_has_prev = (uint32_t *)T(KACC_T_NODE_HAS_PREV);
  s.node_usage_ratio = (double *)T(KACC_T_NODE_USAGE_RATIO);
  s.node_cpu_delta = (double *)T(KACC_T_NODE_CPU_DELTA);
  s.node_status = (uint32_t *)T(KACC_T_NODE_STATUS);
  s.proc_energy = (uint64_t *)T(KACC_T_PROC_ENERGY);
  s.proc_ratio = (double *)T(KACC_T_PROC_RATIO);
  s.proc_node = (uint32_t *)T(KACC_T_PROC_NODE);
  s.ctr_energy = (uint64_t *)T(KACC_T_CTR_ENERGY);
  s.ctr_ratio = (double *)T(KACC_T_CTR_RATIO);
  s.ctr_node = (uint32_t *)T(KACC_T_CTR_NODE);
  s.ctr_cpu_delta = (double *)T(KACC_T_CTR_CPU_DELTA);
  s.ctr_cpu_total = (double *)T(KACC_T_CTR_CPU_TOTAL);
  s.vm_energy = (uint64_t *)T(KACC_T_VM_ENERGY);
  s.vm_ratio = (double *)T(KACC_T_VM_RATIO);
  s.vm_node = (uint32_t *)T(KACC_T_VM_NODE);
  s.vm_cpu_delta = (double *)T(KACC_T_VM_CPU_DELTA);
  s.pod_energy = (uint64_t *)T(KACC_T_POD_ENERGY);
  s.pod_power = (double *)T(KACC_T_POD_POWER);
  s.pod_cpu_delta = (double *)T(KACC_T_POD_CPU_DELTA);
  s.pod_cpu_total = (double *)T(KACC_T_POD_CPU_TOTAL);
  s.proc_slots = ctx->cfg.proc_slots;
  s.ctr_slots = ctx->cfg.ctr_slots;
  s.vm_slots = ctx->cfg.vm_slots;
  s.pod_slots = ctx->cfg.pod_slots;
  s.err = ctx->d_err;
  s.items = ctx->d_items;
  s.item_ctr = ctx->d_ctr;
  s.item_cap = ctx->item_cap;
  s.defer = ctx->d_defer;
  s.defer_ctr = ctx->d_ctr + 2;
  s.defer_cap = ctx->defer_cap;
  s.items_given = 0;
  s.keep_items = 0;
  s.stamps = nullptr;
  return s;
}

template <int Z>
void launch_small(const kacc_interval &b, const kacc::DevState &s, hipStream_t st) {
  const uint32_t grid = (b.n_nodes + kacc::kSmallWaves - 1) / kacc::kSmallWaves;
  if (!kacc::kTransposed<Z> && b.node_proc_span)
    KACC_LAUNCH((kacc::small_kernel<Z, true>), dim3(grid), dim3(64 * kacc::kSmallWaves), 0, st, b, s);
  else
    KACC_LAUNCH((kacc::small_kernel<Z, false>), dim3(grid), dim3(64 * kacc::kSmallWaves), 0, st, b, s);
}

template <int Z, int V>
void launch_zv(const kacc_interval &b, const kacc::DevState &s, hipStream_t st) {
  if (V == 0 && (b.flags & KACC_F_SMALL_NODES)) return launch_small<Z>(b, s, st);
  KACC_LAUNCH((kacc::interval_kernel<Z, V>), dim3(b.n_nodes), dim3(kacc::kTpb<V>),
              KACC_FAST_EXTRA_LDS, st, b, s);
  if (b.flags & (KACC_F_FAST_NODES | KACC_F_SMALL_NODES)) return;
  const uint32_t chunk_grid = std::min<uint32_t>(s.item_cap, kacc::kChunkGrid);
  KACC_LAUNCH((kacc::chunk_kernel<Z, V>), dim3(chunk_grid), dim3(kacc::kChunkThreads), 0, st,
                     b, s);
  KACC_LAUNCH((kacc::pod_kernel<Z, V>), dim3(kacc::kPodGrid), dim3(kacc::kBlock), 0, st, b, s);
}

// ... 815 lines not shown
  int rc = ensure_items(ctx, max_nodes, max_procs, max_pods);
  if (rc != KACC_OK) return rc;
  KACC_HIP(ctx, hipStreamWaitEvent(ctx->stream, bt->copied, 0));
  (void)hipGetLastError();
  const kacc::DevState ds = dev_state(ctx);
  for (uint32_t k = 0; k < K; ++k)
    if (dv[k].n_nodes) launch(ctx->cfg.zones, dv[k], ds, ctx->stream);
  KACC_HIP(ctx, hipGetLastError());
  KACC_HIP(ctx, hipMemcpyAsync(bt->h_err, ctx->d_err, sizeof(uint32_t), hipMemcpyDeviceToHost, ctx->stream));
  KACC_HIP(ctx, hipEventRecord(bt->done, ctx->stream));
  bt->submitted = true;
  ctx->live_nodes = bt->host[K - 1].n_nodes;
  return KACC_OK;
}

int kacc_batch_wait(kacc_ctx *ctx, kacc_batch *bt) {
  if (!ctx || !bt) return KACC_EINVAL;
  if (!bt->submitted) return KACC_OK;
  KACC_HIP(ctx, hipSetDevice(ctx->device));
  KACC_HIP(ctx, hipEventSynchronize(bt->done));
  if (*bt->h_err) {
    *bt->h_err = 0;
    return kacc_sync(ctx, nullptr);
  }
  return KACC_OK;
}

void kacc_batch_free(kacc_ctx *ctx, kacc_batch *bt) {
  if (!bt) return;
  if (ctx) (void)hipSetDevice(ctx->device);
  if (bt->done && bt->submitted) (void)hipEventSynchronize(bt->done);
  for (void *p : bt->allocs) (void)hipHostFree(p);
  for (void *p : bt->dev_allocs) (void)hipFree(p);
  if (bt->copied) (void)hipEventDestroy(bt->copied);
  if (bt->done) (void)hipEventDestroy(bt->done);
  if (bt->h_err) (void)hipHostFree(bt->h_err);
  delete bt;
}


int kacc_table_info(const kacc_ctx *ctx, kacc_table t, uint64_t *elem_bytes, uint64_t *count) {
  if (!ctx || t < 0 || t >= KACC_T_COUNT) return KACC_EINVAL;
  if (elem_bytes) *elem_bytes = kTables[t].elem;
  if (count) *count = ctx->counts[t];
  return KACC_OK;
}

int kacc_table_device_ptr(kacc_ctx *ctx, kacc_table t, void **dev_ptr) {
  if (!ctx || t < 0 || t >= KACC_T_COUNT || !dev_ptr) return KACC_EINVAL;
  if (kTables[t].derived) {
    *dev_ptr = nullptr;
    return fail(ctx, KACC_EINVAL, "table %d is derived on read (no device storage): see kacc_table_download", (int)t);
  }
  *dev_ptr = ctx->tables[t];
  return KACC_OK;
}

int kacc_table_row_stride(const kacc_ctx *ctx, kacc_table t, uint64_t *stride) {
  if (!ctx || t < 0 || t >= KACC_T_COUNT || !stride) return KACC_EINVAL;
  const uint64_t w = kTables[t].zoned ? ctx->cfg.zones : 1;
  *stride = pod_paired(t) ? 2 * w : w;
  return KACC_OK;
}

static int table_copy(kacc_ctx *ctx, kacc_table t, uint64_t first, uint64_t count, void *host,
                      bool down) {
  if (!ctx || t < 0 || t >= KACC_T_COUNT || (!host && count)) return KACC_EINVAL;
  if (first > ctx->counts[t] || count > ctx->counts[t] - first)
    return fail(ctx, KACC_EINVAL, "table %d range [%llu,+%llu) outside %llu", (int)t,
                (unsigned long long)first, (unsigned long long)count,
                (unsigned long long)ctx->counts[t]);
  if (kTables[t].derived && !down)
    return fail(ctx, KACC_EINVAL, "table %d is derived on read and cannot be uploaded", (int)t);
  if (!count) return KACC_OK;
  KACC_HIP(ctx, hipSetDevice(ctx->device));
  KACC_HIP(ctx, hipStreamSynchronize(ctx->stream));
  if (kTables[t].derived || pod_paired(t)) {
    void *tmp = nullptr;
    KACC_HIP(ctx, hipMalloc(&tmp, count * 8));
    hipError_t e = hipSuccess;
    int rc = KACC_OK;
    if (down) {
      rc = kacc_internal_dense_range(ctx, t, first, count, tmp, ctx->stream);
      e = rc == KACC_OK ? hipStreamSynchronize(ctx->stream) : hipSuccess;
      if (rc == KACC_OK && e == hipSuccess) e = hipMemcpy(host, tmp, count * 8, hipMemcpyDeviceToHost);
    } else {
      e = hipMemcpy(tmp, host, count * 8, hipMemcpyHostToDevice);
      if (e == hipSuccess) rc = kacc_internal_pod_scatter(ctx, t, first, count, tmp, ctx->stream);
      if (rc == KACC_OK && e == hipSuccess) e = hipStreamSynchronize(ctx->stream);
    }
    (void)hipFree(tmp);
    if (rc != KACC_OK) return rc;
    if (e != hipSuccess) return fail(ctx, KACC_EHIP, "table %d: %s", (int)t, hipGetErrorString(e));
    return KACC_OK;
  }
  char *dev = static_cast<char *>(ctx->tables[t]) + first * kTables[t].elem;
  const size_t bytes = count * kTables[t].elem;
  if (down)
    KACC_HIP(ctx, hipMemcpy(host, dev, bytes, hipMemcpyDeviceToHost));
  else
    KACC_HIP(ctx, hipMemcpy(dev, host, bytes, hipMemcpyHostToDevice));
  return KACC_OK;
}

int kacc_table_download(kacc_ctx *ctx, kacc_table t, uint64_t first, uint64_t count, void *host_dst) {
  return table_copy(ctx, t, first, count, host_dst, true);
}

int kacc_table_upload(kacc_ctx *ctx, kacc_table t, uint64_t first, uint64_t count,
                      const void *host_src) {
  return table_copy(ctx, t, first, count, const_cast<void *>(host_src), false);
}

int kacc_table_read(kacc_ctx *ctx, kacc_table t, uint64_t first, uint64_t count, void *dev_dst, void *stream) {
  if (!ctx || t < 0 || t >= KACC_T_COUNT || (!dev_dst && count)) return KACC_EINVAL;
  if (first > ctx->counts[t] || count > ctx->counts[t] - first)
    return fail(ctx, KACC_EINVAL, "table %d range [%llu,+%llu) outside %llu", (int)t, (unsigned long long)first,
                (unsigned long long)count, (unsigned long long)ctx->counts[t]);
  if (!count) return KACC_OK;
  KACC_HIP(ctx, hipSetDevice(ctx->device));
  hipStream_t st = stream ? static_cast<hipStream_t>(stream) : ctx->stream;
  if (kTables[t].derived || pod_paired(t)) return kacc_internal_dense_range(ctx, t, first, count, dev_dst, st);
  KACC_HIP(ctx, hipMemcpyAsync(dev_dst, static_cast<const char *>(ctx->tables[t]) + first * kTables[t].elem,
                               count * kTables[t].elem, hipMemcpyDeviceToDevice, st));
  return KACC_OK;
}

int kacc_namespace_totals(kacc_ctx *ctx, uint32_t n_ns, const uint32_t *off, const uint32_t *slots,
                          uint64_t *out_energy, double *out_power, void *stream) {
  if (!ctx) return KACC_EINVAL;
  if (!n_ns) return KACC_OK;
  if (!off || !slots || !out_energy || !out_power) return fail(ctx, KACC_EINVAL, "NULL argument");
  KACC_HIP(ctx, hipSetDevice(ctx->device));
  hipStream_t st = stream ? static_cast<hipStream_t>(stream) : ctx->stream;
  (void)hipGetLastError();
  switch (ctx->cfg.zones) {
    case 1: launch_ns<1>(n_ns, off, slots, ctx, out_energy, out_power, st); break;
    case 2: launch_ns<2>(n_ns, off, slots, ctx, out_energy, out_power, st); break;
    case 3: launch_ns<3>(n_ns, off, slots, ctx, out_energy, out_power, st); break;
    case 4: launch_ns<4>(n_ns, off, slots, ctx, out_energy, out_power, st); break;
    case 5: launch_ns<5>(n_ns, off, slots, ctx, out_energy, out_power, st); break;
    case 6: launch_ns<6>(n_ns, off, slots, ctx, out_energy, out_power, st); break;
    case 7: launch_ns<7>(n_ns, off, slots, ctx, out_energy, out_power, st); break;
    default: launch_ns<8>(n_ns, off, slots, ctx, out_energy, out_power, st); break;
  }
  KACC_HIP(ctx, hipGetLastError());
  return KACC_OK;
}

int kacc_internal_cluster_partials(kacc_ctx *ctx, uint32_t n_ns, const uint32_t *off, const uint32_t *slots,
                                   uint64_t *out_energy, double *out_power, uint64_t *node_energy, double *node_power,
                                   void *stream) {
  return kacc_internal_export_partials(ctx, n_ns, off, slots, nullptr, 0, nullptr, 0, 0, out_energy, out_power,
                                       node_energy, node_power, stream);
}

int kacc_internal_export_partials(kacc_ctx *ctx, uint32_t n_ns, const uint32_t *off, const uint32_t *rows,
                                  const uint64_t *pod_export, uint64_t n_pods, const uint64_t *node_export,
                                  uint64_t n_nodes, int from_exports, uint64_t *out_energy, double *out_power,
                                  uint64_t *node_energy,
                                  double *node_power, void *stream) {
  if (!ctx) return KACC_EINVAL;
  const kacc::TimingScope timing(ctx);
  if (n_ns && (!off || !rows || !out_energy || !out_power)) return fail(ctx, KACC_EINVAL, "NULL argument");
  KACC_HIP(ctx, hipSetDevice(ctx->device));
  hipStream_t st = stream ? static_cast<hipStream_t>(stream) : ctx->stream;
  const uint64_t Z = ctx->cfg.zones;
  if (from_exports && n_nodes && !node_export) return fail(ctx, KACC_EINVAL, "node export is NULL");
  const uint64_t live = from_exports ? n_nodes : std::min<uint64_t>(ctx->live_nodes, ctx->cfg.nodes);
  const uint32_t *slots = rows;
  const uint32_t node_blocks = node_energy ? static_cast<uint32_t>(5 * Z) : 0u;
  const kacc::NodeTotalsArgs na = node_totals_args(ctx, live, node_export, node_energy, node_power);
  if (!n_ns && !node_blocks) return KACC_OK;
  (void)hipGetLastError();
#define KACC_PARTIALS(Z_)                                                                                  \
// ... 69 lines not shown
      for (const auto &e : ins)
        if (overlaps(o.p, o.bytes, e.p, e.bytes))
          return fail(ctx, KACC_EINVAL, "export sums: an output of the sums overlaps an export of this launch");
  }
  hipStream_t st = stream ? static_cast<hipStream_t>(stream) : ctx->stream;
  const bool fuse = b->n_nodes > 0 && !(b->flags & KACC_F_SMALL_NODES) &&
                    !(sa.node_blocks && sa.na.n_nodes > kacc::kColSplitFrom) &&
                    (sa.n_ns || sa.node_blocks) &&
                    static_cast<uint64_t>(b->n_nodes) + sa.node_blocks + sa.ns_blocks <= 0x7fffffffull;
  if (!fuse) {
    if ((rc = run_one(ctx, b, st)) != KACC_OK) return rc;
    return kacc_run_export_sums(ctx, prev, st);
  }
  if ((rc = ensure_items(ctx, b->n_nodes, b->n_procs, b->n_pods)) != KACC_OK) return rc;
  (void)hipGetLastError();
  launch_fused_z(ctx->cfg.zones, *b, dev_state(ctx), sa, st);
  KACC_HIP(ctx, hipGetLastError());
  ctx->live_nodes = b->n_nodes;
  return KACC_OK;
}

int kacc_internal_derived_power(kacc_ctx *ctx, int t, uint64_t first, uint64_t count, double *out, void *stream) {
  if (!ctx) return KACC_EINVAL;
  const int kind = kacc_derived_kind(t);
  if (kind < 0) return fail(ctx, KACC_EINVAL, "table %d is not derived", t);
  if (!count) return KACC_OK;
  if (!out) return fail(ctx, KACC_EINVAL, "NULL argument");
  KACC_HIP(ctx, hipSetDevice(ctx->device));
  hipStream_t st = stream ? static_cast<hipStream_t>(stream) : ctx->stream;
  const uint32_t Z = ctx->cfg.zones;
  const uint64_t slots = (first + count - 1) / Z - first / Z + 1, per_block = 64ull * kacc::kPowWaves;
  const dim3 grid(static_cast<uint32_t>(std::min<uint64_t>((slots + per_block - 1) / per_block, 0x7fffffffull)));
  const kacc::ProcDerive d = kacc_derive(ctx, static_cast<kacc_kind>(kind));
  (void)hipGetLastError();
  switch (Z) {
    case 1: hipLaunchKernelGGL(kacc::proc_power_kernel<1>, grid, dim3(kacc::kBlock), 0, st, d, first, count, out); break;
    case 2: hipLaunchKernelGGL(kacc::proc_power_kernel<2>, grid, dim3(kacc::kBlock), 0, st, d, first, count, out); break;
    case 3: hipLaunchKernelGGL(kacc::proc_power_kernel<3>, grid, dim3(kacc::kBlock), 0, st, d, first, count, out); break;
    case 4: hipLaunchKernelGGL(kacc::proc_power_kernel<4>, grid, dim3(kacc::kBlock), 0, st, d, first, count, out); break;
    case 5: hipLaunchKernelGGL(kacc::proc_power_kernel<5>, grid, dim3(kacc::kBlock), 0, st, d, first, count, out); break;
    case 6: hipLaunchKernelGGL(kacc::proc_power_kernel<6>, grid, dim3(kacc::kBlock), 0, st, d, first, count, out); break;
    case 7: hipLaunchKernelGGL(kacc::proc_power_kernel<7>, grid, dim3(kacc::kBlock), 0, st, d, first, count, out); break;
    default: hipLaunchKernelGGL(kacc::proc_power_kernel<8>, grid, dim3(kacc::kBlock), 0, st, d, first, count, out); break;
  }
  KACC_HIP(ctx, hipGetLastError());
  return KACC_OK;
}

int kacc_internal_dense_range(kacc_ctx *ctx, int t, uint64_t first, uint64_t count, void *out, void *stream) {
  if (!ctx) return KACC_EINVAL;
  if (kacc_derived_kind(t) >= 0) return kacc_internal_derived_power(ctx, t, first, count, static_cast<double *>(out), stream);
  if (!count) return KACC_OK;
  hipStream_t st = stream ? static_cast<hipStream_t>(stream) : ctx->stream;
  if (!pod_paired(t)) {
    KACC_HIP(ctx, hipMemcpyAsync(out, static_cast<const char *>(ctx->tables[t]) + first * 8, count * 8,
                                 hipMemcpyDeviceToDevice, st));
    return KACC_OK;
  }
  KACC_HIP(ctx, hipSetDevice(ctx->device));
  const uint64_t blocks = (count + kacc::kBlock - 1) / kacc::kBlock;
  (void)hipGetLastError();
  hipLaunchKernelGGL(kacc::pod_pair_copy_kernel, dim3(static_cast<uint32_t>(std::min<uint64_t>(blocks, 65536))),
                     dim3(kacc::kBlock), 0, st, static_cast<uint64_t *>(ctx->tables[t]), ctx->cfg.zones, first, count,
                     static_cast<uint64_t *>(out), 0);
  KACC_HIP(ctx, hipGetLastError());
  return KACC_OK;
}

int kacc_internal_pod_scatter(kacc_ctx *ctx, int t, uint64_t first, uint64_t count, const void *in, void *stream) {
  if (!ctx || !pod_paired(t)) return KACC_EINVAL;
  if (!count) return KACC_OK;
  KACC_HIP(ctx, hipSetDevice(ctx->device));
  hipStream_t st = stream ? static_cast<hipStream_t>(stream) : ctx->stream;
  const uint64_t blocks = (count + kacc::kBlock - 1) / kacc::kBlock;
  (void)hipGetLastError();
  hipLaunchKernelGGL(kacc::pod_pair_copy_kernel, dim3(static_cast<uint32_t>(std::min<uint64_t>(blocks, 65536))),
                     dim3(kacc::kBlock), 0, st, static_cast<uint64_t *>(ctx->tables[t]), ctx->cfg.zones, first, count,
                     const_cast<uint64_t *>(static_cast<const uint64_t *>(in)), 1);
  KACC_HIP(ctx, hipGetLastError());
  return KACC_OK;
}

uint64_t kacc_intervals_bytes(uint32_t Z, uint64_t N, uint64_t P, uint64_t C, uint64_t V, uint64_t Q, uint32_t K,
                              int carried, uint32_t flags) {
  if (!carried) return static_cast<uint64_t>(K) * kacc_interval_bytes(Z, N, P, C, V, Q, flags);
  if (K == 0) return 0;
  const uint64_t state_once = N * (12 + 24ull * Z) + P * 8ull * Z + C * (8 + 8ull * Z) + V * 8ull * Z +
                              Q * (8 + 8ull * Z);
  return static_cast<uint64_t>(K) * kacc_interval_bytes(Z, N, P, C, V, Q, flags) -
         static_cast<uint64_t>(K - 1) * state_once;
}

uint64_t kacc_interval_bytes(uint32_t Z, uint64_t N, uint64_t P, uint64_t C, uint64_t V,
                             uint64_t Q, uint32_t flags) {
  const uint64_t node = 76 + 96ull * Z;
  const bool stable = (flags & KACC_F_STABLE_SLOT_NODES) && (KACC_SMALL_STABLE || !(flags & KACC_F_SMALL_NODES));
  const uint64_t proc = (stable ? 20 : 24) + 16ull * Z;
  const uint64_t ctr = 44 + 16ull * Z;
  const uint64_t vm = 28 + 16ull * Z;
  const uint64_t pod = 32 + 24ull * Z;
  return N * node + P * proc + C * ctr + V * vm + Q * pod;
}

static int reject_carry_exports(kacc_ctx *ctx, const kacc_interval *b, uint32_t count) {
  for (uint32_t k = 0; k < count; ++k)
    if (b[k].pod_export || b[k].node_export)
      return fail(ctx, KACC_EINVAL, "interval %u: the carry kernel writes no pod / node exports", k);
  return KACC_OK;
}

int kacc_debug_carry_stamps(kacc_ctx *ctx, const kacc_interval *b, uint32_t count, void *stream, int variant,
                            uint64_t *d_out) {
  if (!ctx || !b || count == 0 || !d_out) return KACC_EINVAL;
  KACC_HIP(ctx, hipSetDevice(ctx->device));
  if (ctx->cfg.zones != 2) return fail(ctx, KACC_EINVAL, "carry variants are built for Z = 2");
  hipStream_t st = stream ? static_cast<hipStream_t>(stream) : ctx->stream;
  int rc = reject_carry_exports(ctx, b, count);
  if (rc != KACC_OK) return rc;
  rc = stage_batches(ctx, b, count, st);
  if (rc != KACC_OK) return rc;
  kacc::DevState ds = dev_state(ctx);
  ds.items = reinterpret_cast<kacc::ChunkItem *>(d_out);
  const bool medium = all_medium(b, count);
  (void)hipGetLastError();
  if (variant == 0)
    launch_carry<16>(2, medium, ctx->d_batches, count, b[0].n_nodes, ds, st);
  else if (variant == 2)
    launch_carry<18>(2, medium, ctx->d_batches, count, b[0].n_nodes, ds, st);
// ... 72 lines not shown
```

kepler_amd/csrc/kacc_format.hip:

```cpp
#include <hip/hip_runtime.h>

#include <algorithm>
#include <cstring>
#include <string>
#include <vector>

#include "kacc_derive.hpp"
#include "kacc_internal.hpp"
#include "kacc_pow5_tables.h"

namespace kacc {
namespace fmt {

constexpr int kThreads = 256;
static_assert(KACC_FMT_WIDTH == 24, "three 8-byte stores per field");

__device__ __forceinline__ uint32_t pow5bits(int32_t e) {
  return static_cast<uint32_t>((static_cast<uint32_t>(e) * 1217359u) >> 19) + 1u;
}
__device__ __forceinline__ uint32_t log10_pow2(int32_t e) {
  return (static_cast<uint32_t>(e) * 78913u) >> 18;
}
__device__ __forceinline__ uint32_t log10_pow5(int32_t e) {
  return (static_cast<uint32_t>(e) * 732923u) >> 20;
// ... 629 lines not shown
    uint64_t total;
    const uint64_t ex = block_excl_scan(v, s_w, total);
    if (i < tiles) tile_sum[i] = carry + ex;
    carry += total;
  }
}

__global__ __launch_bounds__(kScanThreads) void scan_tiles(const uint64_t *in, uint64_t n, const uint64_t *tile_prefix,
                                                            uint64_t *out) {
  __shared__ uint64_t s_w[kScanThreads / 64];
  const uint64_t t0 = static_cast<uint64_t>(blockIdx.x) * kTile + static_cast<uint64_t>(threadIdx.x) * kScanPer;
  uint64_t v[kScanPer], x = 0;
#pragma unroll
  for (int k = 0; k < kScanPer; ++k) {
    v[k] = t0 + k < n ? in[t0 + k] : 0;
    x += v[k];
  }
  uint64_t total;
  uint64_t run = tile_prefix[blockIdx.x] + block_excl_scan(x, s_w, total);
#pragma unroll
  for (int k = 0; k < kScanPer; ++k) {
    if (t0 + k < n) out[t0 + k] = run;
    run += v[k];
  }
}

}
}

extern "C" {

int kacc_format_values(kacc_ctx *ctx, kacc_table t, uint64_t first, uint64_t count, char *out,
                       uint8_t *len, void *stream) {
  if (!ctx || t < 0 || t >= KACC_T_COUNT) return KACC_EINVAL;
  const bool energy = t == KACC_T_NODE_ENERGY_TOTAL || t == KACC_T_NODE_ACTIVE_ENERGY ||
                      t == KACC_T_NODE_ACTIVE_TOTAL || t == KACC_T_NODE_IDLE_TOTAL ||
                      t == KACC_T_PROC_ENERGY || t == KACC_T_CTR_ENERGY || t == KACC_T_VM_ENERGY ||
                      t == KACC_T_POD_ENERGY;
  const bool power = t == KACC_T_NODE_POWER || t == KACC_T_NODE_ACTIVE_POWER || t == KACC_T_NODE_IDLE_POWER ||
                     t == KACC_T_PROC_POWER || t == KACC_T_CTR_POWER || t == KACC_T_VM_POWER ||
                     t == KACC_T_POD_POWER;
  const bool plain = t == KACC_T_NODE_USAGE_RATIO;
  if (!energy && !power && !plain)
    return kacc_fail(ctx, KACC_EINVAL, "table %d is not an energy, power or usage-ratio table", (int)t);
  if (first > ctx->counts[t] || count > ctx->counts[t] - first)
    return kacc_fail(ctx, KACC_EINVAL, "format range outside table %d", (int)t);
  if (!count) return KACC_OK;
  if (!out || !len) return kacc_fail(ctx, KACC_EINVAL, "format: NULL output");
  KACC_HIP(ctx, hipSetDevice(ctx->device));
  hipStream_t st = stream ? static_cast<hipStream_t>(stream) : ctx->stream;
  kacc::fmt::Args a{};
  a.src = static_cast<const char *>(ctx->tables[t]) + first * 8;
  double *derived = nullptr;
  if (kacc_derived_kind(t) >= 0 || t == KACC_T_POD_ENERGY || t == KACC_T_POD_POWER) {
    KACC_HIP(ctx, hipMallocAsync(reinterpret_cast<void **>(&derived), count * 8, st));
    const int rc = kacc_internal_dense_range(ctx, t, first, count, derived, st);
    if (rc != KACC_OK) {
      (void)hipFreeAsync(derived, st);
      return rc;
    }
    a.src = derived;
  }
  a.count = count;
  a.is_energy = energy ? 1u : 0u;
  a.div = plain ? 1.0 : 1e6;
  a.out = out;
  a.len = len;
  (void)hipGetLastError();
  const uint64_t grid = (count + kacc::fmt::kThreads - 1) / kacc::fmt::kThreads;
  if (grid > 0x7fffffffull) {
    if (derived) (void)hipFreeAsync(derived, st);
    return kacc_fail(ctx, KACC_EINVAL, "format: count too large for one launch");
  }
  hipLaunchKernelGGL(kacc::fmt::format_kernel, dim3(static_cast<uint32_t>(grid)), dim3(kacc::fmt::kThreads), 0,
                     st, a);
  if (derived) (void)hipFreeAsync(derived, st);
  KACC_HIP(ctx, hipGetLastError());
  return KACC_OK;
}

}

namespace {

int format_lines_impl(kacc_ctx *ctx, int t, const void *dense, bool energy, uint64_t first, uint64_t count,
                      const char *name, const char *const *zone_names, const uint32_t *zone_order, uint32_t n_zones,
                      const char *labels, const uint64_t *label_off, const uint32_t *row_order, uint64_t *line_off,
                      char *out, uint64_t out_cap, uint64_t *total, void *stream) {
  const uint32_t Z = ctx->cfg.zones;
  if (!name || !zone_names || n_zones == 0 || n_zones > Z)
    return kacc_fail(ctx, KACC_EINVAL, "format_lines: name / zone names missing or n_zones > %u", Z);
  if (count && (!labels || !label_off || !line_off))
    return kacc_fail(ctx, KACC_EINVAL, "format_lines: NULL device array");
  kacc::fmt::LineArgs a{};
  std::string consts(name);
  a.name_len = static_cast<uint32_t>(consts.size());
  auto pad4 = [&consts]() { consts.resize((consts.size() + 3) & ~size_t{3}, '\0'); };
  pad4();
  for (uint32_t j = 0; j < n_zones; ++j) {
    const uint32_t z = zone_order ? zone_order[j] : j;
    if (z >= Z || !zone_names[j]) return kacc_fail(ctx, KACC_EINVAL, "format_lines: bad zone %u", j);
    a.zone_table[j] = z;
    a.zone_pos[j] = static_cast<uint32_t>(consts.size());
    a.zone_len[j] = static_cast<uint32_t>(strlen(zone_names[j]));
    consts += zone_names[j];
    pad4();
  }
  a.zone_pos[n_zones] = static_cast<uint32_t>(consts.size());
  if (consts.size() > kacc::fmt::kConstCap)
    return kacc_fail(ctx, KACC_EINVAL, "format_lines: name + zone names exceed %u bytes", kacc::fmt::kConstCap);
  if (!count) return KACC_OK;
  KACC_HIP(ctx, hipSetDevice(ctx->device));
  hipStream_t st = stream ? static_cast<hipStream_t>(stream) : ctx->stream;
  const uint64_t lines = count * n_zones;
  a.src = t >= 0 ? ctx->tables[t] : dense;
  a.Z = Z;
  a.is_energy = energy ? 1u : 0u;
  a.first = first;
  a.count = count;
  a.n_zones = n_zones;
  a.row_order = row_order;
  a.labels = labels;
  a.label_off = label_off;
  a.const_len = static_cast<uint32_t>(consts.size());
  a.line_off = line_off;
  a.out = out;
  a.out_cap = out_cap;
  a.err = ctx->d_err;
  const uint64_t tiles = (lines + 1 + kacc::fmt::kTile - 1) / kacc::fmt::kTile;
  if (tiles > 0x7fffffffull) return kacc_fail(ctx, KACC_EINVAL, "format_lines: too many lines");
  const size_t scan_bytes = 8 * tiles;
  char *tmp = nullptr;
  auto al = [](uint64_t x) { return (x + 255) & ~255ull; };
  const uint64_t off_len = 1024, off_scan = al(off_len + 8 * (lines + 1));
  const bool derived = t >= 0 && (kacc_derived_kind(t) >= 0 || t == KACC_T_POD_ENERGY || t == KACC_T_POD_POWER);
  const uint64_t off_derived = al(off_scan + scan_bytes);
  KACC_HIP(ctx, hipMallocAsync(reinterpret_cast<void **>(&tmp), derived ? off_derived + 8 * count * Z : off_scan + scan_bytes,
                               st));
  a.consts = tmp;
  a.len = reinterpret_cast<uint64_t *>(tmp + off_len);
  int rc = KACC_OK;
  auto done = [&](int code) {
    (void)hipFreeAsync(tmp, st);
    return code;
  };
  if (derived) {
    a.src = tmp + off_derived;
    a.src_first = first * Z;
    if ((rc = kacc_internal_dense_range(ctx, t, first * Z, count * Z, tmp + off_derived, st)) != KACC_OK)
      return done(rc);
  }
  if (hipMemcpyAsync(tmp, consts.data(), consts.size(), hipMemcpyHostToDevice, st) != hipSuccess)
    return done(kacc_fail(ctx, KACC_EHIP, "format_lines: constants upload"));
  (void)hipGetLastError();
  const uint64_t g1 = std::min<uint64_t>((lines + kacc::fmt::kThreads - 1) / kacc::fmt::kThreads, 1u << 20);
  hipLaunchKernelGGL(kacc::fmt::line_len_kernel, dim3(static_cast<uint32_t>(g1)), dim3(kacc::fmt::kThreads), 0, st, a);
  uint64_t *tile_sum = reinterpret_cast<uint64_t *>(tmp + off_scan);
  (void)kacc_internal_scan_u64(ctx, a.len, lines + 1, tile_sum, line_off, st);
  if (hipGetLastError() != hipSuccess) return done(kacc_fail(ctx, KACC_EHIP, "format_lines: scan launch"));
  if (hipMemcpyAsync(total, line_off + lines, sizeof(uint64_t), hipMemcpyDeviceToHost, st) != hipSuccess ||
      hipStreamSynchronize(st) != hipSuccess)
    return done(kacc_fail(ctx, KACC_EHIP, "format_lines: %s", hipGetErrorString(hipGetLastError())));
  if (!out) return done(KACC_OK);
  if (out_cap < *total)
    return done(kacc_fail(ctx, KACC_ERANGE, "format_lines: %llu bytes of text, out_cap %llu",
                          (unsigned long long)*total, (unsigned long long)out_cap));
  const uint64_t g2 = std::min<uint64_t>((lines + 64 * kacc::fmt::kLineWaves - 1) / (64 * kacc::fmt::kLineWaves),
                                         1u << 14);
  hipLaunchKernelGGL(kacc::fmt::line_write_kernel, dim3(static_cast<uint32_t>(g2)), dim3(64 * kacc::fmt::kLineWaves),
                     0, st, a);
  if (hipGetLastError() != hipSuccess) rc = kacc_fail(ctx, KACC_EHIP, "format_lines: launch");
  return done(rc);
}

}

extern "C" {

uint64_t kacc_internal_scan_tiles(uint64_t n) { return (n + kacc::fmt::kTile - 1) / kacc::fmt::kTile; }

int kacc_internal_scan_u64(kacc_ctx *ctx, const uint64_t *in, uint64_t n, uint64_t *tile_sum, uint64_t *out,
                           void *stream) {
  const uint64_t tiles = kacc_internal_scan_tiles(n);
  if (tiles == 0) return KACC_OK;
  if (tiles > 0x7fffffffull) return kacc_fail(ctx, KACC_EINVAL, "scan: too many values");
  hipStream_t st = static_cast<hipStream_t>(stream);
  const dim3 gt(static_cast<uint32_t>(tiles)), bt(kacc::fmt::kScanThreads);
  hipLaunchKernelGGL(kacc::fmt::scan_tile_sums, gt, bt, 0, st, in, n, tile_sum);
// ... 42 lines not shown
```

kepler_amd/csrc/kacc_internal.hpp:

```cpp
#pragma once

#include <hip/hip_runtime.h>
#include <hip/hip_ext.h>

#include <string>
#include <utility>
#include <vector>

#include "../../include/kepler_accel.h"

namespace kacc {
struct ChunkItem;
}

struct kacc_ctx {
  int device = 0;
  kacc_config cfg{};
  hipStream_t stream = nullptr;
  hipStream_t copy_stream = nullptr;
  void *tables[KACC_T_COUNT] = {};
  uint64_t counts[KACC_T_COUNT] = {};
  uint32_t *d_err = nullptr;
  uint32_t *d_ctr = nullptr;
  kacc::ChunkItem *d_items = nullptr;
  uint64_t *d_colpart = nullptr;
  uint32_t *d_colarrived = nullptr;
  uint32_t item_cap = 0;
  uint2 *d_defer = nullptr;
  uint32_t defer_cap = 0;
  kacc_interval *d_batches = nullptr;
  kacc_interval *h_batches = nullptr;
  uint32_t batch_cap = 0;
  hipEvent_t batch_copied = nullptr;
  uint32_t live_nodes = 0;
  hipEvent_t time_start = nullptr, time_stop = nullptr;
  std::string err;
};

struct kacc_batch {
  kacc_shape cap{};
  std::vector<kacc_interval> host;
  std::vector<kacc_interval> dev;
  std::vector<kacc_interval> orig;
  std::vector<void *> allocs;
  std::vector<void *> dev_allocs;
  hipEvent_t copied = nullptr;
  hipEvent_t done = nullptr;
  uint32_t *h_err = nullptr;
  bool submitted = false;
};

extern "C" int kacc_internal_dense_range(kacc_ctx *ctx, int t, uint64_t first, uint64_t count, void *out,
                                         void *stream);
extern "C" int kacc_internal_pod_scatter(kacc_ctx *ctx, int t, uint64_t first, uint64_t count, const void *in,
                                         void *stream);

extern "C" uint64_t kacc_internal_scan_tiles(uint64_t n);
extern "C" int kacc_internal_scan_u64(kacc_ctx *ctx, const uint64_t *in, uint64_t n, uint64_t *tile_sum,
                                      uint64_t *out, void *stream);

namespace kacc {
struct LaunchTiming {
  hipEvent_t start = nullptr, stop = nullptr;
};
inline LaunchTiming *&launch_timing() {
  static thread_local LaunchTiming *t = nullptr;
  return t;
}
class TimingScope {
 public:
  explicit TimingScope(kacc_ctx *ctx) {
    if (ctx && (ctx->time_start || ctx->time_stop)) {
      t_.start = ctx->time_start;
      t_.stop = ctx->time_stop;
      ctx->time_start = ctx->time_stop = nullptr;
      launch_timing() = &t_;
      on_ = true;
    }
  }
  ~TimingScope() {
    if (on_) launch_timing() = nullptr;
  }
  TimingScope(const TimingScope &) = delete;
  TimingScope &operator=(const TimingScope &) = delete;

 private:
  LaunchTiming t_;
  bool on_ = false;
};
}

#define KACC_LAUNCH(kernel, grid, block, shmem, stream, ...)                                             \
  do {                                                                                                    \
    kacc::LaunchTiming *kacc_lt_ = kacc::launch_timing();                                                 \
    if (kacc_lt_) {                                                                                       \
      hipExtLaunchKernelGGL(kernel, grid, block, shmem, stream, kacc_lt_->start, kacc_lt_->stop, 0,       \
                            __VA_ARGS__);                                                                 \
      kacc_lt_->start = nullptr;                                                                          \
    } else {                                                                                              \
      hipLaunchKernelGGL(kernel, grid, block, shmem, stream, __VA_ARGS__);                                \
    }                                                                                                     \
  } while (0)

struct kacc_slotmap {
  kacc_ctx *ctx = nullptr;
  int device = 0;
  kacc_kind kind = KACC_KIND_PROC;
  uint32_t n_nodes = 0;
// ... 33 lines not shown
```

kepler_amd/csrc/kacc_packer.hip:

```cpp
#include <hip/hip_runtime.h>

#include <algorithm>
#include <atomic>
#include <thread>
#include <vector>

#include "kacc_derive.hpp"
#include "kacc_internal.hpp"

namespace {

constexpr uint32_t kNone = 0xffffffffu;

struct KeyMap {
  std::vector<uint64_t> keys;
  std::vector<uint32_t> vals;
  uint64_t mask = 0;
  void reset(size_t n) {
    size_t cap = 16;
    while (cap < 2 * n) cap <<= 1;
    if (keys.size() < cap) {
      keys.assign(cap, KACC_KEY_EMPTY);
      vals.assign(cap, 0);
    } else {
// ... 122 lines not shown
    cend += s.pods[q].rows;
    o->pod_ctr_end[b->q + q] = cend;
    o->pod_key[b->q + q] = s.pods[q].key;
    o->pod_ns[b->q + q] = s.pods[q].ns;
  }
  for (uint32_t r = r0; r < r1; ++r) {
    const uint8_t t = in.type[r];
    uint32_t dst;
    if (t == KACC_PROC_CONTAINER)
      dst = s.ctrs[s.grp[r - r0]].cursor++;
    else if (t == KACC_PROC_VM)
      dst = s.vms[s.grp[r - r0]].cursor++;
    else
      dst = rest++;
    o->proc_cpu_delta[dst] = in.cpu_delta[r];
    o->proc_key[dst] = in.pid[r];
    if (o->row_record) o->row_record[dst] = r;
  }
  (void)regular;
  return 0;
}

template <typename F>
void for_node_ranges(const kacc_records &in, uint32_t threads, F fn) {
  const uint32_t N = in.n_nodes;
  const uint32_t T = std::max<uint32_t>(1, std::min<uint32_t>(threads, std::max<uint32_t>(N, 1)));
  if (T == 1) {
    fn(0u, N, 0u);
    return;
  }
  std::vector<uint32_t> cut(T + 1, N);
  cut[0] = 0;
  const uint64_t total = in.rec_off[N];
  uint32_t n = 0;
  for (uint32_t t = 1; t < T; ++t) {
    const uint64_t target = total * t / T;
    while (n < N && in.rec_off[n] < target) ++n;
    cut[t] = n;
  }
  std::vector<std::thread> pool;
  for (uint32_t t = 0; t < T; ++t) pool.emplace_back(fn, cut[t], std::max(cut[t], cut[t + 1]), t);
  for (auto &th : pool) th.join();
}

}

namespace kacc {
namespace unpack {

constexpr int kThreads = 256;

template <int Z>
__global__ __launch_bounds__(kThreads) void unpack_kernel(uint32_t n, const uint32_t *w, const uint32_t *dest,
                                                          uint64_t cap, const uint64_t *te, const double *tp,
                                                          uint32_t stride, const ProcDerive pd, uint64_t *oe,
                                                          double *op, uint32_t *err) {
  const uint32_t i = blockIdx.x * kThreads + threadIdx.x;
  if (i >= n) return;
  const uint64_t s = w[i] & KACC_SLOT_MASK;
  const uint64_t o = static_cast<uint64_t>(dest ? dest[i] : i) * Z;
  if (s >= cap) {
    atomicOr(err, 1u << 2);
    return;
  }
#pragma unroll
  for (int z = 0; z < Z; ++z) {
    oe[o + z] = te[s * stride + z];
    op[o + z] = tp ? tp[s * stride + z] : proc_power(pd, s, z);
  }
}

}
}

extern "C" {

int kacc_pack(const kacc_records *in, kacc_packed *out, uint32_t threads) {
  if (!in || !out) return kacc_fail(nullptr, KACC_EINVAL, "kacc_pack: NULL argument");
  const uint32_t N = in->n_nodes;
  if (!in->rec_off) return kacc_fail(nullptr, KACC_EINVAL, "kacc_pack: rec_off is NULL");
  const uint32_t R = in->rec_off[N];
  if (in->rec_off[0] != 0) return kacc_fail(nullptr, KACC_EINVAL, "kacc_pack: rec_off[0] != 0");
  for (uint32_t n = 0; n < N; ++n)
    if (in->rec_off[n + 1] < in->rec_off[n]) return kacc_fail(nullptr, KACC_EINVAL, "kacc_pack: rec_off not monotonic");
  if (R && (!in->pid || !in->cpu_delta || !in->type || !in->ctr_key || !in->vm_key))
    return kacc_fail(nullptr, KACC_EINVAL, "kacc_pack: NULL record array");
  if (!out->proc_off || !out->ctr_off || !out->vm_off || !out->pod_off)
    return kacc_fail(nullptr, KACC_EINVAL, "kacc_pack: NULL offset array");
  std::vector<Counts> cnt(N);
  std::atomic<int> bad{0};
  std::atomic<uint32_t> bad_node{0};
  for_node_ranges(*in, threads ? threads : 1, [&](uint32_t nb, uint32_t ne, uint32_t) {
    Scratch s;
    for (uint32_t n = nb; n < ne; ++n) {
      const int rc = pack_node(*in, n, s, &cnt[n], nullptr, nullptr);
      if (rc) {
        bad = rc;
        bad_node = n;
        return;
      }
    }
  });
  if (bad == -1)
    return kacc_fail(nullptr, KACC_EINVAL, "kacc_pack: node %u: a container / VM key, or a pod key other than KACC_KEY_EMPTY, is a reserved value",
                     bad_node.load());
  if (bad == -2) return kacc_fail(nullptr, KACC_EINVAL, "kacc_pack: node %u: unknown process type", bad_node.load());
  uint64_t C = 0, V = 0, Q = 0;
  out->proc_off[0] = out->ctr_off[0] = out->vm_off[0] = out->pod_off[0] = 0;
  for (uint32_t n = 0; n < N; ++n) {
    C += cnt[n].c;
    V += cnt[n].v;
    Q += cnt[n].q;
    if (C > 0xffffffffull || V > 0xffffffffull || Q > 0xffffffffull)
      return kacc_fail(nullptr, KACC_EINVAL, "kacc_pack: more than 2^32 aggregates");
    out->proc_off[n + 1] = in->rec_off[n + 1];
    out->ctr_off[n + 1] = static_cast<uint32_t>(C);
    out->vm_off[n + 1] = static_cast<uint32_t>(V);
    out->pod_off[n + 1] = static_cast<uint32_t>(Q);
  }
  const bool fits = R <= out->n_procs && C <= out->n_ctrs && V <= out->n_vms && Q <= out->n_pods;
  const uint32_t cap_p = out->n_procs, cap_c = out->n_ctrs, cap_v = out->n_vms, cap_q = out->n_pods;
  out->n_procs = R;
  out->n_ctrs = static_cast<uint32_t>(C);
  out->n_vms = static_cast<uint32_t>(V);
  out->n_pods = static_cast<uint32_t>(Q);
  if (!fits)
    return kacc_fail(nullptr, KACC_ERANGE,
                     "kacc_pack: needs %u rows / %llu containers / %llu VMs / %llu pods, capacity %u / %u / %u / %u", R,
                     (unsigned long long)C, (unsigned long long)V, (unsigned long long)Q, cap_p, cap_c, cap_v, cap_q);
  if ((R && (!out->proc_cpu_delta || !out->proc_key)) || (C && (!out->ctr_proc_end || !out->ctr_key)) ||
      (V && (!out->vm_proc_end || !out->vm_key)) || (Q && (!out->pod_ctr_end || !out->pod_key || !out->pod_ns)))
    return kacc_fail(nullptr, KACC_EINVAL, "kacc_pack: NULL output array");
  for_node_ranges(*in, threads ? threads : 1, [&](uint32_t nb, uint32_t ne, uint32_t) {
    Scratch s;
    for (uint32_t n = nb; n < ne; ++n) {
      const Bases b{out->proc_off[n], out->ctr_off[n], out->vm_off[n], out->pod_off[n]};
      Counts c;
      pack_node(*in, n, s, &c, out, &b);
    }
  });
  return KACC_OK;
}

int kacc_unpack(kacc_ctx *ctx, kacc_kind kind, uint32_t n, const uint32_t *slot_words, const uint32_t *dest,
                uint64_t *out_energy, double *out_power, void *stream) {
  if (!ctx) return KACC_EINVAL;
  if (!n) return KACC_OK;
  if (!slot_words || !out_energy || !out_power) return kacc_fail(ctx, KACC_EINVAL, "kacc_unpack: NULL argument");
  if (kind < KACC_KIND_PROC || kind > KACC_KIND_POD) return kacc_fail(ctx, KACC_EINVAL, "bad kind");
  KACC_HIP(ctx, hipSetDevice(ctx->device));
  hipStream_t st = stream ? static_cast<hipStream_t>(stream) : ctx->stream;
  const int te = kind == KACC_KIND_PROC ? KACC_T_PROC_ENERGY
                 : kind == KACC_KIND_CTR ? KACC_T_CTR_ENERGY
                 : kind == KACC_KIND_VM ? KACC_T_VM_ENERGY
                                        : KACC_T_POD_ENERGY;
  const uint64_t cap = kind == KACC_KIND_PROC ? ctx->cfg.proc_slots
                       : kind == KACC_KIND_CTR ? ctx->cfg.ctr_slots
                       : kind == KACC_KIND_VM ? ctx->cfg.vm_slots
                                              : ctx->cfg.pod_slots;
  const uint64_t *e = static_cast<const uint64_t *>(ctx->tables[te]);
  const double *p = kind == KACC_KIND_POD ? static_cast<const double *>(ctx->tables[te + 1]) : nullptr;
  const kacc::ProcDerive pd = kacc_derive(ctx, kind);
  const uint32_t grid = (n + kacc::unpack::kThreads - 1) / kacc::unpack::kThreads;
  (void)hipGetLastError();
#define KACC_UNPACK(Z)                                                                                          \
  hipLaunchKernelGGL((kacc::unpack::unpack_kernel<Z>), dim3(grid), dim3(kacc::unpack::kThreads), 0, st, n,   \
                     slot_words, dest, cap, e, p, kind == KACC_KIND_POD ? 2 * Z : Z, pd, out_energy, out_power,   \
                     ctx->d_err)
  switch (ctx->cfg.zones) {
    case 1: KACC_UNPACK(1); break;
    case 2: KACC_UNPACK(2); break;
    case 3: KACC_UNPACK(3); break;
    case 4: KACC_UNPACK(4); break;
    case 5: KACC_UNPACK(5); break;
    case 6: KACC_UNPACK(6); break;
    case 7: KACC_UNPACK(7); break;
    default: KACC_UNPACK(8); break;
  }
#undef KACC_UNPACK
  KACC_HIP(ctx, hipGetLastError());
  return KACC_OK;
}

}
```

kepler_amd/csrc/kacc_top.hip:

```cpp
#include <hip/hip_runtime.h>

#include <algorithm>

#include "kacc_derive.hpp"
#include "kacc_internal.hpp"

namespace kacc {
namespace top {

constexpr uint32_t kBuf = 2048;
constexpr uint32_t kMinTake = 256;
constexpr uint32_t kGroup = 8;
constexpr uint32_t kMinFan = 8;
constexpr uint32_t kErrTop = 1u << 9;
constexpr uint32_t kNone = 0xffffffffu;

enum Src { kEnergy = 0, kStored = 1, kDerived = 2, kCand = 3 };
enum Out { kNodes = 0, kList = 1, kFleet = 2 };
constexpr int threads_of(int out) { return out == kNodes ? 256 : 512; }

struct Cand {
  uint2 *ikey;
  uint32_t *row;
  uint32_t *node;
  uint32_t *count;
};

struct Args {
  const uint64_t *words;
  uint32_t stride;
  uint32_t mode;
  ProcDerive pd;
  uint32_t zone;
  uint64_t cap;
  uint32_t n_nodes, n_rows;
  const uint32_t *row_off, *slot, *node_status;
  uint32_t k;
  uint32_t group;
  uint32_t n_lists;
  Cand in, out;
  uint32_t *out_count, *out_row, *out_slot, *out_node;
  uint64_t *out_value;
  uint32_t *err;
};

__device__ __forceinline__ uint64_t power_key(uint64_t b) {
  const uint32_t hi = static_cast<uint32_t>(b >> 32), lo = static_cast<uint32_t>(b);
  const uint32_t mag = hi & 0x7fffffffu;
  if (mag > 0x7ff00000u || (mag == 0x7ff00000u && lo != 0)) return 0;
  if ((mag | lo) == 0) return 0x8000000000000000ull;
  return (hi >> 31) ? ~b : (b | 0x8000000000000000ull);
}

struct NodeGuard {
  double aP;
  bool live;
};
__device__ __forceinline__ NodeGuard node_guard(const ProcDerive &d, uint32_t n, uint32_t zone) {
  const uint64_t i = static_cast<uint64_t>(n) * d.zones + zone;
  NodeGuard g;
  g.aP = d.active_power[i];
  g.live = !(d.active_energy[i] == 0 || !(d.cpu_delta[n] != 0) || !(g.aP != 0));
  return g;
}

template <int kSrc>
__device__ __forceinline__ uint64_t slot_value(const Args &a, uint64_t s, const NodeGuard &g) {
  if constexpr (kSrc == kDerived) {
    return static_cast<uint64_t>(__double_as_longlong(g.live ? a.pd.ratio[s] * g.aP : 0.0));
  } else {
    return a.words[s * a.stride];
  }
}

__device__ __forceinline__ bool after(uint2 ak, uint32_t ar, uint2 bk, uint32_t br) {
  return ak.y != bk.y ? ak.y > bk.y : (ak.x != bk.x ? ak.x > bk.x : ar > br);
}

template <int kSrc, int kOut>
__global__ __launch_bounds__(threads_of(kOut)) void select_kernel(const Args a) {
  constexpr uint32_t kThreads = threads_of(kOut), kPer = kBuf / kThreads;
  constexpr bool kCarry = kOut != kNodes;
  __shared__ uint2 s_key[kBuf];
  __shared__ uint32_t s_row[kBuf];
  __shared__ uint32_t s_node[kCarry ? kBuf : 1];
  __shared__ uint32_t s_fill;
  const uint32_t tid = threadIdx.x, lane = tid & 63u;
  const uint32_t k = a.k;
  uint32_t first_trigger = 256;
  while (first_trigger < 4 * k && first_trigger < kBuf) first_trigger <<= 1;

  uint32_t fill = 0, kept = 0;
  bool have_thr = false;
  uint2 thr_key = make_uint2(kNone, kNone);
  uint32_t thr_row = kNone;
  if (tid == 0) s_fill = 0;
  __syncthreads();

  auto sort_and_cut = [&]() {
    uint32_t P = 64;
    while (P < fill) P <<= 1;
    for (uint32_t i = fill + tid; i < P; i += kThreads) {
      s_key[i] = make_uint2(kNone, kNone);
      s_row[i] = kNone;
    }
    __syncthreads();
    for (uint32_t sz = 2; sz <= P; sz <<= 1) {
      for (uint32_t st = sz >> 1; st > 0; st >>= 1) {
        for (uint32_t t = tid; t < (P >> 1); t += kThreads) {
          const uint32_t i = 2 * t - (t & (st - 1)), j = i + st;
          const uint2 ki = s_key[i], kj = s_key[j];
          const uint32_t ri = s_row[i], rj = s_row[j];
          const bool up = (i & sz) == 0;
          if (after(ki, ri, kj, rj) == up) {
            s_key[i] = kj;
            s_key[j] = ki;
            s_row[i] = rj;
            s_row[j] = ri;
            if constexpr (kCarry) {
              const uint32_t ni = s_node[i];
              s_node[i] = s_node[j];
              s_node[j] = ni;
            }
          }
// ... 81 lines not shown
  while (pos < total) {
    const uint32_t limit = have_thr ? kBuf : first_trigger;
    const uint32_t take = min(limit - fill, total - pos);
    bool ok[kPer];
    uint2 key[kPer];
    uint32_t row[kPer], node[kPer];
    const uint32_t last = pos + take - 1;
    if constexpr (kSrc == kCand) {
      uint32_t j[kPer], cnt[kPer];
      uint64_t e[kPer];
#pragma unroll
      for (uint32_t u = 0; u < kPer; ++u) {
        const uint32_t i = u * kThreads + tid, f = min(pos + i, last);
        const uint32_t l = f / k;
        j[u] = f - l * k;
        ok[u] = i < take;
        e[u] = static_cast<uint64_t>(src0 + l) * k;
        cnt[u] = a.in.count[src0 + l];
      }
#pragma unroll
      for (uint32_t u = 0; u < kPer; ++u) {
        ok[u] = ok[u] && j[u] < min(cnt[u], k);
        e[u] += ok[u] ? j[u] : 0u;
        key[u] = a.in.ikey[e[u]];
        row[u] = a.in.row[e[u]];
        node[u] = a.in.node[e[u]];
      }
    } else {
      uint32_t w[kPer], ln[kPer];
#pragma unroll
      for (uint32_t u = 0; u < kPer; ++u) {
        const uint32_t i = u * kThreads + tid, f = min(pos + i, last);
        uint32_t n = 0;
        for (uint32_t s = 1; s < ng; ++s) n += f >= s_pre[s];
        ok[u] = i < take;
        ln[u] = n;
        row[u] = s_r0[n] + (f - s_pre[n]);
        node[u] = src0 + n;
        w[u] = a.slot[row[u]];
      }
      uint64_t v[kPer];
      bool bad = false;
#pragma unroll
      for (uint32_t u = 0; u < kPer; ++u) {
        const uint64_t sl = w[u] & KACC_SLOT_MASK;
        const bool in = sl < a.cap;
        bad = bad || (ok[u] && !in);
        ok[u] = ok[u] && in;
        v[u] = 0;
        if (a.cap != 0) {
          if constexpr (kSrc == kDerived)
            v[u] = static_cast<uint64_t>(__double_as_longlong(a.pd.ratio[in ? sl : 0]));
          else
            v[u] = a.words[(in ? sl : 0) * a.stride];
        }
      }
      if (bad) atomicOr(a.err, kErrTop);
#pragma unroll
      for (uint32_t u = 0; u < kPer; ++u) {
        if constexpr (kSrc == kDerived) {
          const double p = s_live[ln[u]] ? __longlong_as_double(static_cast<long long>(v[u])) * s_aP[ln[u]] : 0.0;
          v[u] = static_cast<uint64_t>(__double_as_longlong(p));
        }
        const uint64_t ik = ~(kSrc == kEnergy ? v[u] : power_key(v[u]));
        key[u] = make_uint2(static_cast<uint32_t>(ik), static_cast<uint32_t>(ik >> 32));
      }
    }
#pragma unroll
    for (uint32_t u = 0; u < kPer; ++u)
      if (u * kThreads < take) append(ok[u], key[u], row[u], node[u]);
    pos += take;
    __syncthreads();
    fill = s_fill;
    __syncthreads();
    const uint32_t trigger = have_thr ? kBuf - kMinTake : first_trigger;
    if (fill >= trigger) sort_and_cut();
  }
  if (fill > kept) sort_and_cut();
  const uint32_t count = min(fill, k);

  if constexpr (kOut == kList) {
    const uint64_t o = static_cast<uint64_t>(blockIdx.x) * k;
    if (tid == 0) a.out.count[blockIdx.x] = count;
    for (uint32_t j = tid; j < count; j += kThreads) {
      a.out.ikey[o + j] = s_key[j];
      a.out.row[o + j] = s_row[j];
      a.out.node[o + j] = s_node[j];
    }
  } else {
    const uint64_t o = static_cast<uint64_t>(blockIdx.x) * k;
    if (tid == 0) a.out_count[blockIdx.x] = count;
    for (uint32_t j = tid; j < k; j += kThreads) {
      uint32_t row = kNone, sl = kNone, node = kNone;
      uint64_t v = 0;
      if (j < count) {
        row = s_row[j];
        node = kOut == kFleet ? s_node[j] : blockIdx.x;
        sl = a.slot[row] & KACC_SLOT_MASK;
        if (a.mode == kDerived)
          v = slot_value<kDerived>(a, sl, node_guard(a.pd, node, a.zone));
        else
          v = a.words[static_cast<uint64_t>(sl) * a.stride];
      }
      a.out_row[o + j] = row;
      if (a.out_slot) a.out_slot[o + j] = sl;
      if (kOut == kFleet && a.out_node) a.out_node[o + j] = node;
      if (a.out_value) a.out_value[o + j] = v;
    }
  }
}

}
}

namespace {

using kacc::top::Args;

int table_kind(int t) {
  switch (t) {
    case KACC_T_PROC_ENERGY: case KACC_T_PROC_POWER: return KACC_KIND_PROC;
    case KACC_T_CTR_ENERGY: case KACC_T_CTR_POWER: return KACC_KIND_CTR;
    case KACC_T_VM_ENERGY: case KACC_T_VM_POWER: return KACC_KIND_VM;
    case KACC_T_POD_ENERGY: case KACC_T_POD_POWER: return KACC_KIND_POD;
    default: return -1;
  }
}

int fill_args(kacc_ctx *ctx, const char *fn, kacc_table t, uint32_t zone, uint32_t k, const kacc_top_rows *rows,
              const void *out_count, const void *out_row, Args *a) {
  const int kind = table_kind(t);
  if (kind < 0) return kacc_fail(ctx, KACC_EINVAL, "%s: table %d is not a workload energy / power table", fn, (int)t);
  const uint32_t Z = ctx->cfg.zones;
  if (zone >= Z) return kacc_fail(ctx, KACC_EINVAL, "%s: zone %u >= Z = %u", fn, zone, Z);
  if (k < 1 || k > KACC_TOP_MAX) return kacc_fail(ctx, KACC_EINVAL, "%s: k = %u outside 1 .. %u", fn, k, KACC_TOP_MAX);
  if (!rows || !out_count || !out_row) return kacc_fail(ctx, KACC_EINVAL, "%s: NULL argument", fn);
  if (rows->n_nodes > ctx->cfg.nodes)
    return kacc_fail(ctx, KACC_EINVAL, "%s: n_nodes %u > the context's %llu nodes", fn, rows->n_nodes,
                     (unsigned long long)ctx->cfg.nodes);
  if (!rows->row_off || (rows->n_rows && !rows->slot)) return kacc_fail(ctx, KACC_EINVAL, "%s: NULL row array", fn);
  *a = Args{};
  a->cap = kind == KACC_KIND_PROC ? ctx->cfg.proc_slots
           : kind == KACC_KIND_CTR ? ctx->cfg.ctr_slots
           : kind == KACC_KIND_VM ? ctx->cfg.vm_slots
                                  : ctx->cfg.pod_slots;
  a->pd = kacc_derive(ctx, static_cast<kacc_kind>(kind == KACC_KIND_POD ? KACC_KIND_PROC : kind));
  if (kacc_derived_kind(t) >= 0) {
    a->mode = kacc::top::kDerived;
  } else {
    const bool power = t == KACC_T_POD_POWER;
    a->mode = power ? kacc::top::kStored : kacc::top::kEnergy;
    a->words = static_cast<const uint64_t *>(ctx->tables[t]) + zone;
    a->stride = kind == KACC_KIND_POD ? 2 * Z : Z;
  }
  a->zone = zone;
  a->n_nodes = rows->n_nodes;
  a->n_rows = rows->n_rows;
  a->row_off = rows->row_off;
  a->slot = rows->slot;
  a->node_status = rows->node_status;
  a->k = k;
  a->err = ctx->d_err;
  return KACC_OK;
}

template <int kOut>
void launch_rows(const Args &a, uint32_t grid, hipStream_t st) {
  using namespace kacc::top;
  switch (a.mode) {
    case kEnergy: KACC_LAUNCH((select_kernel<kEnergy, kOut>), dim3(grid), dim3(threads_of(kOut)), 0, st, a); break;
    case kStored: KACC_LAUNCH((select_kernel<kStored, kOut>), dim3(grid), dim3(threads_of(kOut)), 0, st, a); break;
    default: KACC_LAUNCH((select_kernel<kDerived, kOut>), dim3(grid), dim3(threads_of(kOut)), 0, st, a); break;
  }
}

}

extern "C" {

int kacc_top_nodes(kacc_ctx *ctx, kacc_table t, uint32_t zone, uint32_t k, const kacc_top_rows *rows,
                   uint32_t *out_count, uint32_t *out_row, uint32_t *out_slot, uint64_t *out_value, void *stream) {
  if (!ctx) return KACC_EINVAL;
  Args a;
  const int rc = fill_args(ctx, "kacc_top_nodes", t, zone, k, rows, out_count, out_row, &a);
  if (rc != KACC_OK) return rc;
  if (a.n_nodes == 0) return KACC_OK;
  if (a.n_nodes > 0x7fffffffu) return kacc_fail(ctx, KACC_EINVAL, "kacc_top_nodes: too many nodes for one launch");
  KACC_HIP(ctx, hipSetDevice(ctx->device));
  hipStream_t st = stream ? static_cast<hipStream_t>(stream) : ctx->stream;
  kacc::TimingScope timing(ctx);
  a.group = 1;
  a.out_count = out_count;
  a.out_row = out_row;
  a.out_slot = out_slot;
  a.out_value = out_value;
  (void)hipGetLastError();
  launch_rows<kacc::top::kNodes>(a, a.n_nodes, st);
  KACC_HIP(ctx, hipGetLastError());
  return KACC_OK;
}

int kacc_top_fleet(kacc_ctx *ctx, kacc_table t, uint32_t zone, uint32_t k, const kacc_top_rows *rows,
                   uint32_t *out_count, uint32_t *out_row, uint32_t *out_slot, uint32_t *out_node,
                   uint64_t *out_value, void *stream) {
  using namespace kacc::top;
  if (!ctx) return KACC_EINVAL;
// ... 55 lines not shown
```

kepler_amd/csrc/kacc_tracker.hip:

```cpp
#include <hip/hip_runtime.h>

#include <algorithm>
#include <cstring>
#include <vector>

#include "kacc_derive.hpp"
#include "kacc_internal.hpp"

namespace kacc {
namespace trk {

constexpr int kThreads = 256;
constexpr uint32_t kSetLds = 512;
constexpr uint32_t kErrCap = 1u << 10;

struct Args {
  const uint64_t *tab_e;
  const double *tab_p;
  ProcDerive pd;
  uint64_t min_e;
  int64_t max_size;
  uint32_t Z, z0, cap, n_nodes;
  uint32_t tab_stride;
  const uint32_t *slot_off;
  const uint64_t *term_key;
  const uint32_t *term_slot;
  const uint32_t *term_count;
  uint64_t *set_key;
  uint64_t *set_e;
  double *set_p;
  uint32_t *size;
  uint32_t *err;
};

constexpr int kWaveNodes = kThreads / 64;
template <uint32_t kZ>
__global__ __launch_bounds__(kThreads) __attribute__((amdgpu_waves_per_eu(kZ <= 4 ? 8 : 4))) void node_add_wave_kernel(
    const Args a) {
  __shared__ uint64_t s_te_all[kWaveNodes][kSetLds];
  __shared__ uint64_t s_se_all[kWaveNodes][64];
  const uint32_t wv = __builtin_amdgcn_readfirstlane(threadIdx.x >> 6), lane = threadIdx.x & 63u;
  const uint32_t n = blockIdx.x * kWaveNodes + wv;
  if (n >= a.n_nodes) return;
  uint64_t *const s_te = s_te_all[wv];
  uint64_t *const s_se = s_se_all[wv];
  const uint32_t Z = a.Z, z0 = a.z0, cap = a.cap;
  const uint64_t base = static_cast<uint64_t>(n) * cap;
  const uint32_t b0 = a.slot_off[n];
  const uint32_t c = min(a.term_count[n], a.slot_off[n + 1] - b0);
  const uint32_t K = a.max_size > 0 ? static_cast<uint32_t>(a.max_size) : cap;
  uint32_t size = min(a.size[n], cap);
  for (uint32_t c0 = 0; c0 < c; c0 += 64) {
    const uint32_t m0 = min(64u, c - c0);
    const bool full = a.max_size > 0 && size >= K;
    const uint64_t min_full = full ? a.set_e[(base + size - 1) * Z + z0] : 0ull;
    uint64_t key = 0, e = 0;
    uint32_t slot = 0;
    bool pass = false;
    if (lane < m0) {
      slot = a.term_slot[b0 + c0 + lane];
      key = a.term_key[b0 + c0 + lane];
      e = a.tab_e[static_cast<uint64_t>(slot) * a.tab_stride + z0];
      pass = e >= a.min_e && !(full && e <= min_full);
    }
    if (__ballot(pass) == 0) continue;
    const bool lds_set = size <= kSetLds;
    for (uint32_t t0 = 0; t0 < size; t0 += 64) {
      const uint32_t t = t0 + lane;
      const uint64_t tk = t < size ? a.set_key[base + t] : 0ull;
      if (lds_set && t < size) s_te[t] = a.set_e[(base + t) * Z + z0];
      const uint32_t tn = min(64u, size - t0);
      const uint32_t tk_lo = static_cast<uint32_t>(tk), tk_hi = static_cast<uint32_t>(tk >> 32);
      for (uint32_t j = 0; j < tn; ++j) {
        const uint64_t kj = (static_cast<uint64_t>(static_cast<uint32_t>(__builtin_amdgcn_readlane(static_cast<int>(tk_hi), j))) << 32) |
                            static_cast<uint32_t>(__builtin_amdgcn_readlane(static_cast<int>(tk_lo), j));
        pass = pass && key != kj;
      }
    }
    const uint64_t pmask = __ballot(pass);
    const uint32_t m = static_cast<uint32_t>(__popcll(pmask));
    if (m == 0) continue;
    uint64_t k1 = pass ? ~e : ~0ull;
    uint32_t k2 = pass ? slot : ~0u, ix = lane;
    for (uint32_t sz = 2; sz <= 64; sz <<= 1) {
      for (uint32_t stride = sz >> 1; stride > 0; stride >>= 1) {
        const uint64_t b1 = __shfl_xor(k1, static_cast<int>(stride), 64);
        const uint32_t b2 = __shfl_xor(k2, static_cast<int>(stride), 64);
        const uint32_t b3 = __shfl_xor(ix, static_cast<int>(stride), 64);
        const bool up = (lane & sz) == 0, lower = (lane & stride) == 0;
        const bool a_gt = k1 > b1 || (k1 == b1 && k2 > b2), b_gt = b1 > k1 || (b1 == k1 && b2 > k2);
        const bool take = lower == up ? a_gt : b_gt;
        k1 = take ? b1 : k1;
        k2 = take ? b2 : k2;
        ix = take ? b3 : ix;
      }
    }
    const uint64_t skey = __shfl(key, static_cast<int>(ix), 64);
    const uint32_t sslot = static_cast<uint32_t>(__shfl(static_cast<int>(slot), static_cast<int>(ix), 64));
    const uint64_t se = ~k1;
    s_se[lane] = se;
    __builtin_amdgcn_fence(__ATOMIC_RELEASE, "wavefront");
    __builtin_amdgcn_wave_barrier();
    __builtin_amdgcn_fence(__ATOMIC_ACQUIRE, "wavefront");
    uint32_t new_size = size + m;
    if (a.max_size > 0) {
      new_size = min(new_size, K);
    } else if (new_size > cap) {
      if (lane == 0) atomicOr(a.err, kErrCap);
      new_size = cap;
    }
    uint32_t rank = ~0u;
    if (lane < m) {
      uint32_t lo = 0, hi = size;
      while (lo < hi) {
        const uint32_t mid = (lo + hi) >> 1;
        if ((lds_set ? s_te[mid] : a.set_e[(base + mid) * Z + z0]) >= se)
          lo = mid + 1;
        else
          hi = mid;
      }
      rank = lane + lo;
    }
    if (size > 0) {
      for (int64_t blk = static_cast<int64_t>((size - 1) & ~63u); blk >= 0; blk -= 64) {
        const uint32_t i = static_cast<uint32_t>(blk) + lane;
        if (i >= size) continue;
        const uint64_t ei = lds_set ? s_te[i] : a.set_e[(base + i) * Z + z0];
        uint32_t lo = 0, hi = m;
        while (lo < hi) {
          const uint32_t mid = (lo + hi) >> 1;
          if (s_se[mid] > ei)
            lo = mid + 1;
          else
            hi = mid;
        }
        const uint32_t r = i + lo;
        if (r == i || r >= new_size) continue;
        const uint64_t k = a.set_key[base + i];
        uint64_t E[kZ];
        double P[kZ];
        for (uint32_t z = 0; z < kZ && z < Z; ++z) {
          E[z] = a.set_e[(base + i) * Z + z];
          P[z] = a.set_p[(base + i) * Z + z];
        }
        a.set_key[base + r] = k;
        for (uint32_t z = 0; z < kZ && z < Z; ++z) {
          a.set_e[(base + r) * Z + z] = E[z];
          a.set_p[(base + r) * Z + z] = P[z];
        }
      }
    }
    if (lane < m && rank < new_size) {
      a.set_key[base + rank] = skey;
      for (uint32_t z = 0; z < Z; ++z) {
        a.set_e[(base + rank) * Z + z] = a.tab_e[static_cast<uint64_t>(sslot) * a.tab_stride + z];
        a.set_p[(base + rank) * Z + z] =
            a.tab_p ? a.tab_p[static_cast<uint64_t>(sslot) * a.tab_stride + z] : proc_power(a.pd, sslot, z);
      }
    }
    size = new_size;
    __builtin_amdgcn_fence(__ATOMIC_ACQ_REL, "workgroup");
  }
  if (lane == 0) a.size[n] = size;
}

__global__ __launch_bounds__(kThreads) void pack_kernel(const Args a, const uint64_t *off, uint64_t *out_key,
                                                        uint32_t *out_node, uint64_t *out_e, double *out_p) {
  const uint32_t n = blockIdx.x;
  const uint64_t o = off[n], cnt = off[n + 1] - o, base = static_cast<uint64_t>(n) * a.cap;
  for (uint64_t i = threadIdx.x; i < cnt; i += kThreads) {
    out_key[o + i] = a.set_key[base + i];
    out_node[o + i] = n;
    for (uint32_t z = 0; z < a.Z; ++z) {
      out_e[(o + i) * a.Z + z] = a.set_e[(base + i) * a.Z + z];
      out_p[(o + i) * a.Z + z] = a.set_p[(base + i) * a.Z + z];
    }
  }
}

constexpr uint32_t kErrRead = 1u << 11;
constexpr uint32_t kReadMaxBlocks = 2048;

__global__ __launch_bounds__(kThreads) void read_count_kernel(const uint32_t *size, const uint32_t *mask,
                                                              uint32_t n_nodes, uint32_t cap, uint64_t *cnt) {
  const uint32_t n = blockIdx.x * kThreads + threadIdx.x;
  if (n > n_nodes) return;
  cnt[n] = n < n_nodes && (!mask || mask[n]) ? min(size[n], cap) : 0u;
}

struct ReadArgs {
  const uint64_t *off;
  const uint64_t *set_key;
  const uint64_t *set_e;
  const double *set_p;
  uint32_t *size;
  const uint32_t *mask;
  uint32_t n_nodes, cap, Z, item_cap, clear;
  uint32_t *node_off;
  uint64_t *out_key;
  uint32_t *out_node;
  uint64_t *out_e;
  double *out_p;
  uint32_t *err;
};

__device__ __forceinline__ void node_search_round(const uint64_t *off, uint64_t x, uint32_t lane, uint32_t &lo,
                                                  uint32_t &hi) {
  const uint64_t st = (hi - lo) / 64u + 1u;
// ... 38 lines not shown
      else
        lo = mid + 1;
    }
    const uint64_t o = a.off[lo];
    const uint64_t j = min(i >= o ? i - o : 0ull, static_cast<uint64_t>(a.cap - 1));
    const uint64_t row = static_cast<uint64_t>(lo) * a.cap + j;
    if (c0 + lane < limit) {
      if (a.out_key) a.out_key[i] = a.set_key[row];
      if (a.out_node) a.out_node[i] = lo;
    }
    const uint32_t words = static_cast<uint32_t>(last - c0 + 1) * Z;
    const uint64_t w0 = c0 * Z;
#pragma unroll
    for (uint32_t k = 0; k < (kZ ? kZ : KACC_MAX_ZONES) / kW; ++k) {
      const uint32_t w = (k * 64 + lane) * kW;
      const uint32_t it = min(w / Z, 63u), z = w - it * Z;
      const uint64_t r = __shfl(row, static_cast<int>(it), 64);
      if (w < words) {
        if (kW == 2) {
          if (a.out_e) *reinterpret_cast<u64x2 *>(a.out_e + w0 + w) = *reinterpret_cast<const u64x2 *>(a.set_e + r * Z + z);
          if (a.out_p) *reinterpret_cast<u64x2 *>(a.out_p + w0 + w) = *reinterpret_cast<const u64x2 *>(a.set_p + r * Z + z);
        } else {
          if (a.out_e) a.out_e[w0 + w] = a.set_e[r * Z + z];
          if (a.out_p) a.out_p[w0 + w] = a.set_p[r * Z + z];
        }
      }
    }
  }
}

__global__ __launch_bounds__(kThreads) void clear_kernel(uint32_t *size, uint32_t n_nodes, const uint32_t *mask) {
  const uint32_t n = blockIdx.x * kThreads + threadIdx.x;
  if (n < n_nodes && (!mask || mask[n])) size[n] = 0;
}

}
}

struct kacc_tracker {
  kacc_ctx *ctx = nullptr;
  int device = 0;
  kacc_kind kind = KACC_KIND_PROC;
  int64_t max_size = 0;
  uint32_t cap = 0, zone = 0, Z = 0, nodes = 0;
  uint64_t min_e = 0;
  uint64_t *d_set_key = nullptr;
  uint64_t *d_set_e = nullptr;
  double *d_set_p = nullptr;
  uint32_t *d_size = nullptr;
};

namespace {

void kind_tables(const kacc_ctx *ctx, kacc_kind k, const uint64_t **e, const double **p) {
  const int base = k == KACC_KIND_PROC ? KACC_T_PROC_ENERGY
                   : k == KACC_KIND_CTR ? KACC_T_CTR_ENERGY
                   : k == KACC_KIND_VM ? KACC_T_VM_ENERGY
                                       : KACC_T_POD_ENERGY;
  *e = static_cast<const uint64_t *>(ctx->tables[base]);
  *p = k == KACC_KIND_POD ? static_cast<const double *>(ctx->tables[base + 1]) : nullptr;
}

kacc::trk::Args tracker_args(const kacc_tracker *t) {
  kacc::trk::Args a{};
  kind_tables(t->ctx, t->kind, &a.tab_e, &a.tab_p);
  a.pd = kacc_derive(t->ctx, t->kind);
  a.min_e = t->min_e;
  a.max_size = t->max_size;
  a.Z = t->Z;
  a.tab_stride = t->kind == KACC_KIND_POD ? 2 * t->Z : t->Z;
  a.z0 = t->zone;
  a.cap = t->cap;
  a.n_nodes = t->nodes;
  a.set_key = t->d_set_key;
  a.set_e = t->d_set_e;
  a.set_p = t->d_set_p;
  a.size = t->d_size;
  a.err = t->ctx->d_err;
  return a;
}

}

extern "C" {

int kacc_tracker_create(kacc_ctx *ctx, kacc_kind kind, int64_t max_size, uint32_t capacity,
                        uint32_t zone, uint64_t min_energy, kacc_tracker **out) {
  if (!ctx || !out) return KACC_EINVAL;
  *out = nullptr;
  if (kind < KACC_KIND_PROC || kind > KACC_KIND_POD) return kacc_fail(ctx, KACC_EINVAL, "bad kind");
  if (zone >= ctx->cfg.zones) return kacc_fail(ctx, KACC_EINVAL, "zone %u >= Z", zone);
  if (max_size > static_cast<int64_t>(KACC_TRACKER_MAX_BOUNDED))
    return kacc_fail(ctx, KACC_EINVAL, "max_size > %u", KACC_TRACKER_MAX_BOUNDED);
  const uint32_t cap = max_size > 0 ? static_cast<uint32_t>(max_size) : max_size < 0 ? capacity : 0u;
  if (max_size < 0 && capacity == 0) return kacc_fail(ctx, KACC_EINVAL, "unlimited tracker needs a capacity");
  KACC_HIP(ctx, hipSetDevice(ctx->device));
  auto *t = new kacc_tracker;
  t->ctx = ctx;
  t->device = ctx->device;
  t->kind = kind;
  t->max_size = max_size;
  t->cap = std::max<uint32_t>(cap, 1);
  t->zone = zone;
  t->Z = ctx->cfg.zones;
  t->nodes = static_cast<uint32_t>(std::max<uint64_t>(ctx->cfg.nodes, 1));
  t->min_e = min_energy;
  const size_t items = static_cast<size_t>(t->nodes) * t->cap, Z = t->Z;
  const size_t need = items * (8 + 16 * Z) + 4ull * t->nodes;
  size_t free_b = 0, total_b = 0;
  if (hipMemGetInfo(&free_b, &total_b) == hipSuccess && need > free_b) {
    const uint32_t nodes = t->nodes, per = t->cap;
    delete t;
    return kacc_fail(ctx, KACC_ENOMEM,
// ... 179 lines not shown
```

Baseline: 54.86 billion proc-attr/s.

## Split process energy table into low and high 32-bit planes

Stores the per-process u64 energy as two separate u32 planes (low and high words). The hot attribution kernel then loads only the low plane for previous values and writes the high plane only when it is known or changes, which cuts HBM traffic in the bandwidth-bound process sweep. Readers such as top, tracker, packer and format reconstruct full words through an EnergyTab helper. The risk is that the carry into the high word relies on a read-modify-write, which is subtle to get right, and the change touches many consumers of the table.

```diff
diff --git a/kepler_amd/csrc/kacc_derive.hpp b/kepler_amd/csrc/kacc_derive.hpp
--- a/kepler_amd/csrc/kacc_derive.hpp
+++ b/kepler_amd/csrc/kacc_derive.hpp
@@ -3,6 +3,7 @@
 #include <hip/hip_runtime.h>
 #include <stdint.h>
 
+#include "kacc_device.hpp"
 #include "kacc_internal.hpp"
 
 namespace kacc {
@@ -42,10 +43,26 @@
 }
 inline kacc::ProcDerive kacc_proc_derive(const kacc_ctx *ctx) { return kacc_derive(ctx, KACC_KIND_PROC); }
 
+inline kacc::EnergyTab kacc_energy_tab(const kacc_ctx *ctx, kacc_kind kind) {
+  const int t = kind == KACC_KIND_PROC ? KACC_T_PROC_ENERGY
+                : kind == KACC_KIND_CTR ? KACC_T_CTR_ENERGY
+                : kind == KACC_KIND_VM ? KACC_T_VM_ENERGY
+                                       : KACC_T_POD_ENERGY;
+  kacc::EnergyTab e;
+  e.base = ctx->tables[t];
+  e.planes = kind == KACC_KIND_PROC ? ctx->counts[t] : 0;
+  e.stride = kind == KACC_KIND_POD ? 2 * ctx->cfg.zones : ctx->cfg.zones;
+  return e;
+}
+
 inline int kacc_derived_kind(int t) {
   return t == KACC_T_PROC_POWER ? KACC_KIND_PROC : t == KACC_T_CTR_POWER ? KACC_KIND_CTR
                                                  : t == KACC_T_VM_POWER ? KACC_KIND_VM : -1;
 }
 
+inline bool kacc_indirect_table(int t) {
+  return kacc_derived_kind(t) >= 0 || t == KACC_T_POD_ENERGY || t == KACC_T_POD_POWER || t == KACC_T_PROC_ENERGY;
+}
+
 extern "C" int kacc_internal_derived_power(kacc_ctx *ctx, int t, uint64_t first, uint64_t count, double *out,
                                            void *stream);
diff --git a/kepler_amd/csrc/kacc_device.hpp b/kepler_amd/csrc/kacc_device.hpp
--- a/kepler_amd/csrc/kacc_device.hpp
+++ b/kepler_amd/csrc/kacc_device.hpp
@@ -38,4 +38,15 @@
   return 0;
 }
 
+struct EnergyTab {
+  const void *base;
+  uint64_t planes;
+  uint32_t stride;
+};
+__device__ __forceinline__ uint64_t energy_word(const EnergyTab &t, uint64_t i) {
+  if (t.planes == 0) return static_cast<const uint64_t *>(t.base)[i];
+  const uint32_t *lo = static_cast<const uint32_t *>(t.base);
+  return (static_cast<uint64_t>(lo[t.planes + i]) << 32) | lo[i];
 }
+
+}
diff --git a/kepler_amd/csrc/kacc_engine.hip b/kepler_amd/csrc/kacc_engine.hip
--- a/kepler_amd/csrc/kacc_engine.hip
+++ b/kepler_amd/csrc/kacc_engine.hip
@@ -127,7 +127,7 @@
   uint32_t *node_has_prev;
   double *node_usage_ratio, *node_cpu_delta;
   uint32_t *node_status;
-  uint64_t *proc_energy;
+  uint32_t *proc_lo, *proc_hi;
   double *proc_ratio;
   uint32_t *proc_node;
   uint64_t *ctr_energy;
@@ -214,6 +214,59 @@
   }
 }
 
+template <int Z, bool kNtLoad = false>
+__device__ __forceinline__ void load_proc_lo(const uint32_t *__restrict__ lo, uint64_t s, uint32_t (&out)[Z]) {
+  constexpr int kW = Z % 4 == 0 ? 4 : Z % 2 == 0 ? 2 : 1;
+  using piece = __attribute__((ext_vector_type(kW))) uint32_t;
+  if constexpr (kW > 1) {
+    const piece *p = reinterpret_cast<const piece *>(lo + s * Z);
+#pragma unroll
+    for (int k = 0; k < Z / kW; ++k) {
+      const piece x = kNtLoad ? __builtin_nontemporal_load(p + k) : p[k];
+#pragma unroll
+      for (int i = 0; i < kW; ++i) out[kW * k + i] = x[i];
+    }
+  } else {
+#pragma unroll
+    for (int z = 0; z < Z; ++z) out[z] = kNtLoad ? __builtin_nontemporal_load(lo + s * Z + z) : lo[s * Z + z];
+  }
+}
+template <int Z, bool NT>
+__device__ __forceinline__ void store_proc_lo(uint32_t *__restrict__ lo, uint64_t s, const uint32_t (&in)[Z]) {
+  constexpr int kW = Z % 4 == 0 ? 4 : Z % 2 == 0 ? 2 : 1;
+  using piece = __attribute__((ext_vector_type(kW))) uint32_t;
+  if constexpr (kW > 1) {
+    piece *p = reinterpret_cast<piece *>(lo + s * Z);
+#pragma unroll
+    for (int k = 0; k < Z / kW; ++k) {
+      piece x;
+#pragma unroll
+      for (int i = 0; i < kW; ++i) x[i] = in[kW * k + i];
+      if constexpr (NT)
+        nt_store(x, p + k);
+      else
+        p[k] = x;
+    }
+  } else {
+#pragma unroll
+    for (int z = 0; z < Z; ++z) {
+      if constexpr (NT)
+        nt_store(in[z], lo + s * Z + z);
+      else
+        lo[s * Z + z] = in[z];
+    }
+  }
+}
+template <int Z>
+__device__ __forceinline__ void load_proc_full(const uint32_t *__restrict__ lo, const uint32_t *__restrict__ hi,
+                                               uint64_t s, uint64_t (&out)[Z]) {
+  uint32_t l[Z], h[Z];
+  load_proc_lo<Z>(lo, s, l);
+  load_proc_lo<Z>(hi, s, h);
+#pragma unroll
+  for (int z = 0; z < Z; ++z) out[z] = (static_cast<uint64_t>(h[z]) << 32) | l[z];
+}
+
 template <int Z>
 __device__ __forceinline__ void load_row_f64(const double *__restrict__ base, uint64_t s,
                                              double (&out)[Z]) {
@@ -312,9 +365,9 @@
   return ratio;
 }
 
-template <int Z>
+template <int Z, typename PT>
 __device__ __forceinline__ double attribute_proc(const Attr<Z> &a, double delta, bool is_new,
-                                                 const uint64_t (&prev)[Z], uint64_t (&E)[Z]) {
+                                                 const PT (&prev)[Z], uint64_t (&E)[Z]) {
   const double ratio = delta / a.nd;
 #pragma unroll
   for (int z = 0; z < Z; ++z) {
@@ -328,10 +381,39 @@
   return ratio;
 }
 
+template <int Z>
+__device__ __forceinline__ uint32_t proc_known(const Attr<Z> &a, bool is_new) {
+  constexpr uint32_t kAll = (1u << Z) - 1u;
+  return (a.first || is_new) ? kAll : (~a.live & kAll);
+}
+
 template <int Z, bool NT>
-__device__ __forceinline__ void store_proc(const DevState &st, uint64_t s, const uint64_t (&E)[Z], double ratio,
-                                           uint32_t node, bool wnode) {
-  store_row<Z, NT, uint64_t>(st.proc_energy, s, E);
+__device__ __forceinline__ void store_proc(const DevState &st, uint64_t s, const uint64_t (&E)[Z], uint32_t known,
+                                           double ratio, uint32_t node, bool wnode) {
+  uint32_t L[Z];
+#pragma unroll
+  for (int z = 0; z < Z; ++z) L[z] = static_cast<uint32_t>(E[z]);
+  store_proc_lo<Z, NT>(st.proc_lo, s, L);
+  if (known == (1u << Z) - 1u) {
+    uint32_t H[Z];
+#pragma unroll
+    for (int z = 0; z < Z; ++z) H[z] = static_cast<uint32_t>(E[z] >> 32);
+    store_proc_lo<Z, NT>(st.proc_hi, s, H);
+  } else {
+    uint32_t *__restrict__ hi = st.proc_hi + s * Z;
+#pragma unroll
+    for (int z = 0; z < Z; ++z) {
+      const uint32_t h = static_cast<uint32_t>(E[z] >> 32);
+      if (known & (1u << z)) {
+        if constexpr (NT)
+          nt_store(h, hi + z);
+        else
+          hi[z] = h;
+      } else if (h != 0) {
+        hi[z] = hi[z] + h;
+      }
+    }
+  }
   if constexpr (NT) {
     nt_store(ratio, st.proc_ratio + s);
     if (wnode) nt_store(node, st.proc_node + s);
@@ -461,87 +543,29 @@
   }
 }
 template <int Z, bool kMasked, bool kNtLoad = false>
-__device__ __forceinline__ void load_group_masked(const uint64_t *__restrict__ base, uint64_t s0,
-                                                  uint32_t len, uint64_t safe, uint64_t (&out)[Z]) {
-  using u64x2 = __attribute__((ext_vector_type(2))) unsigned long long;
-  constexpr int kHalf = Z / 2;
+__device__ __forceinline__ void load_proc_group(const uint32_t *__restrict__ lo, uint64_t s0, uint32_t len,
+                                                uint64_t safe, uint32_t (&out)[Z]) {
   const uint32_t lane = threadIdx.x & 63u;
-  const u64x2 *p = reinterpret_cast<const u64x2 *>(base + s0 * Z);
-  const u64x2 *q = reinterpret_cast<const u64x2 *>(base + safe * Z);
-#pragma unroll
-  for (int j = 0; j < kHalf; ++j) {
-    const uint32_t piece = lane + 64u * j;
-    if constexpr (!kMasked) {
-      const u64x2 x = kNtLoad ? __builtin_nontemporal_load(p + piece) : p[piece];
-      out[2 * j] = x.x;
-      out[2 * j + 1] = x.y;
-      continue;
-    }
-    const bool ok = piece / kHalf < len;
-    const u64x2 *src = ok ? p + piece : q;
-    const u64x2 x = kNtLoad ? __builtin_nontemporal_load(src) : *src;
-    out[2 * j] = ok ? x.x : 0ull;
-    out[2 * j + 1] = ok ? x.y : 0ull;
-  }
+  const bool ok = !kMasked || lane < len;
+  load_proc_lo<Z, kNtLoad>(lo, ok ? s0 + lane : safe, out);
 }
 
 template <int Z, bool NT, bool kInv>
-__device__ __forceinline__ void attribute_group_masked(const Attr<Z> &a, const NodeShared &sh,
-                                                       const double *s_d, const uint32_t *s_w,
-                                                       const uint16_t *s_inv,
-                                                       uint32_t row0, uint64_t s0, uint32_t len,
-                                                       const uint64_t (&prev)[Z],
-                                                       uint64_t *__restrict__ energy,
-                                                       double *__restrict__ ratio_tab,
-                                                       uint32_t *__restrict__ node_tab, uint32_t node) {
-  using u64x2 = __attribute__((ext_vector_type(2))) unsigned long long;
-  constexpr int kHalf = Z / 2;
+__device__ __forceinline__ void attribute_proc_group(const Attr<Z> &a, const DevState &st, const double *s_d,
+                                                     const uint32_t *s_w, const uint16_t *s_inv, uint32_t row0,
+                                                     uint64_t s0, uint32_t len, const uint32_t (&prev)[Z],
+                                                     uint32_t node) {
   const uint32_t lane = threadIdx.x & 63u;
-  u64x2 *pe = reinterpret_cast<u64x2 *>(energy + s0 * Z);
-#pragma unroll
-  for (int j = 0; j < kHalf; ++j) {
-    const uint32_t piece = lane + 64u * j;
-    const uint32_t idx = piece / kHalf;
-    const uint32_t zp = piece % kHalf;
-    uint32_t row = row0 + idx;
-    if constexpr (kInv) {
-      if (idx >= len) continue;
-      row = s_inv[row];
-      if (row == 0xffffu) continue;
-    }
-    const uint32_t wr = s_w[row];
-    const bool is_new = (wr & KACC_SLOT_NEW) != 0;
-    const double ratio = s_d[row] / a.nd;
-    uint64_t E[2];
-#pragma unroll
-    for (int h = 0; h < 2; ++h) {
-      const uint32_t z = 2 * zp + h;
-      const uint64_t aE = sh.active_energy[z];
-      if (a.live & (1u << z)) {
-        const uint64_t e = go_f64_to_u64(ratio * u2f(aE));
-        E[h] = a.first ? e : e + (is_new ? 0ull : prev[2 * j + h]);
-      } else {
-        E[h] = 0;
-      }
-    }
-    u64x2 ev;
-    ev.x = E[0];
-    ev.y = E[1];
-    if constexpr (NT)
-      nt_store(ev, pe + piece);
-    else
-      pe[piece] = ev;
-    if (zp == 0) {
-      const bool wnode = !a.keep_node || is_new;
-      if constexpr (NT) {
-        nt_store(ratio, ratio_tab + s0 + idx);
-        if (wnode) nt_store(node, node_tab + s0 + idx);
-      } else {
-        ratio_tab[s0 + idx] = ratio;
-        if (wnode) node_tab[s0 + idx] = node;
-      }
-    }
-  }
+  uint32_t row = row0 + lane;
+  if constexpr (kInv) {
+    if (lane >= len) return;
+    row = s_inv[row];
+    if (row == 0xffffu) return;
+  }
+  const bool is_new = (s_w[row] & KACC_SLOT_NEW) != 0;
+  uint64_t E[Z];
+  const double ratio = attribute_proc<Z>(a, s_d[row], is_new, prev, E);
+  store_proc<Z, NT>(st, s0 + lane, E, proc_known<Z>(a, is_new), ratio, node, !a.keep_node || is_new);
 }
 
 template <int Z>
@@ -943,7 +967,7 @@
   auto a_cpu_delta = [&]() {
     return role == 1 ? st.ctr_cpu_delta : role == 2 ? st.vm_cpu_delta : st.pod_cpu_delta;
   };
-  uint64_t prev[kRowsPerThread][Z];
+  uint32_t prev[kRowsPerThread][Z];
   uint32_t contig = 0;
   constexpr bool kSweepable =
       kTransposed<Z> && (V & (kVarNoTranspose | kVarNoSweep | kVarSkipProcs)) == 0;
@@ -969,14 +993,14 @@
       if constexpr (kRowSweep) {
 #pragma unroll
         for (int k = 0; k < kRowsPerThread; ++k)
-          load_row<Z>(st.proc_energy, static_cast<uint64_t>(smin) + min(tid + k * kThreads, span - 1), prev[k]);
+          load_proc_lo<Z>(st.proc_lo, static_cast<uint64_t>(smin) + min(tid + k * kThreads, span - 1), prev[k]);
       }
       if constexpr (kSweepable) {
 #pragma unroll
         for (int k = 0; k < kRowsPerThread; ++k) {
           const uint32_t pos0 = static_cast<uint32_t>(tid & ~63) + k * kThreads;
           const uint32_t len = pos0 < span ? min(span - pos0, 64u) : 0u;
-          load_group_masked<Z, true, kNtLd>(st.proc_energy, static_cast<uint64_t>(smin) + pos0, len, smin,
+          load_proc_group<Z, true, kNtLd>(st.proc_lo, static_cast<uint64_t>(smin) + pos0, len, smin,
                                      prev[k]);
         }
       }
@@ -988,12 +1012,12 @@
           const uint64_t g0 = uniform_u32(static_cast<uint32_t>(sl));
           if (__all((tid + k * kThreads) < rows && sl == g0 + (tid & 63) && g0 + 64 <= st.proc_slots)) {
             contig |= 1u << k;
-            load_group_masked<Z, false, kNtLd>(st.proc_energy, g0, 64u, g0, prev[k]);
+            load_proc_group<Z, false, kNtLd>(st.proc_lo, g0, 64u, g0, prev[k]);
             continue;
           }
         }
         if (sl < st.proc_slots) {
-          load_row<Z>(st.proc_energy, sl, prev[k]);
+          load_proc_lo<Z>(st.proc_lo, sl, prev[k]);
         } else {
 #pragma unroll
           for (int z = 0; z < Z; ++z) prev[k][z] = 0;
@@ -1156,7 +1180,8 @@
         const uint32_t wk = s_w[r];
         uint64_t E[Z];
         const double ratio = attribute_proc<Z>(a, s_d[r], (wk & KACC_SLOT_NEW) != 0, prev[k], E);
-        store_proc<Z, kNT>(st, static_cast<uint64_t>(smin) + pos, E, ratio, n, !a.keep_node || (wk & KACC_SLOT_NEW));
+        store_proc<Z, kNT>(st, static_cast<uint64_t>(smin) + pos, E, proc_known<Z>(a, (wk & KACC_SLOT_NEW) != 0), ratio, n,
+                           !a.keep_node || (wk & KACC_SLOT_NEW));
       }
     }
     if constexpr (kSweepable) {
@@ -1164,9 +1189,8 @@
       for (int k = 0; k < kRowsPerThread; ++k) {
         const uint32_t pos0 = static_cast<uint32_t>(tid & ~63) + k * kThreads;
         const uint32_t len = pos0 < span ? min(span - pos0, 64u) : 0u;
-        attribute_group_masked<Z, kNT, true>(a, sh, s_d, s_w, s_inv, pos0,
-                                             static_cast<uint64_t>(smin) + pos0, len, prev[k],
-                                             st.proc_energy, st.proc_ratio, st.proc_node, n);
+        attribute_proc_group<Z, kNT, true>(a, st, s_d, s_w, s_inv, pos0, static_cast<uint64_t>(smin) + pos0, len,
+                                           prev[k], n);
       }
     }
   } else if constexpr ((V & kVarSkipProcs) == 0) {
@@ -1176,9 +1200,8 @@
       if constexpr (kTransposed<Z> && (V & kVarNoTranspose) == 0) {
         if (contig & (1u << k)) {
           const uint32_t pos0 = r - (tid & 63);
-          attribute_group_masked<Z, kNT, false>(a, sh, s_d, s_w, s_inv, pos0,
-                                                uniform_u32(s_w[pos0] & KACC_SLOT_MASK), 64u, prev[k],
-                                                st.proc_energy, st.proc_ratio, st.proc_node, n);
+          attribute_proc_group<Z, kNT, false>(a, st, s_d, s_w, s_inv, pos0,
+                                              uniform_u32(s_w[pos0] & KACC_SLOT_MASK), 64u, prev[k], n);
           continue;
         }
       }
@@ -1191,7 +1214,8 @@
       }
       uint64_t E[Z];
       const double ratio = attribute_proc<Z>(a, s_d[r], (wk & KACC_SLOT_NEW) != 0, prev[k], E);
-      store_proc<Z, kNtScat>(st, sl, E, ratio, n, !a.keep_node || (wk & KACC_SLOT_NEW));
+      store_proc<Z, kNtScat>(st, sl, E, proc_known<Z>(a, (wk & KACC_SLOT_NEW) != 0), ratio, n,
+                             !a.keep_node || (wk & KACC_SLOT_NEW));
     }
   }
   if (stage) __syncthreads();
@@ -1545,7 +1569,7 @@
             const uint64_t sl = static_cast<uint64_t>(s_lo) + pos;
             uint64_t pv[Z];
             if (sl < st.proc_slots) {
-              load_row<Z>(st.proc_energy, sl, pv);
+              load_proc_full<Z>(st.proc_lo, st.proc_hi, sl, pv);
 #pragma unroll
               for (int z = 0; z < Z; ++z) s_cE[pos * Z + z] = pv[z];
             }
@@ -1561,7 +1585,7 @@
             if (sl == (s_cw[r] & KACC_SLOT_MASK)) continue;
             uint64_t pv[Z];
             if (sl < st.proc_slots) {
-              load_row<Z>(st.proc_energy, sl, pv);
+              load_proc_full<Z>(st.proc_lo, st.proc_hi, sl, pv);
             } else {
 #pragma unroll
               for (int z = 0; z < Z; ++z) pv[z] = 0;
@@ -1721,7 +1745,8 @@
           for (int z = 0; z < Z; ++z) pv[z] = s_cE[pos * Z + z];
           const double ratio = attribute_proc<Z>(a, s_d[r], (wk & KACC_SLOT_NEW) != 0, pv, E);
           if constexpr ((V & kCarryNoRowStores) == 0) {
-            store_proc<Z, true>(st, static_cast<uint64_t>(s_lo) + pos, E, ratio, n, !a.keep_node || (wk & KACC_SLOT_NEW));
+            store_proc<Z, true>(st, static_cast<uint64_t>(s_lo) + pos, E, (1u << Z) - 1u, ratio, n,
+                                !a.keep_node || (wk & KACC_SLOT_NEW));
           }
 #pragma unroll
           for (int z = 0; z < Z; ++z) s_cE[pos * Z + z] = E[z];
@@ -1746,7 +1771,7 @@
         for (int z = 0; z < Z; ++z) pv[z] = s_cE[r * Z + z];
         const double ratio = attribute_proc<Z>(a, s_d[r], (wk & KACC_SLOT_NEW) != 0, pv, E);
         if constexpr ((V & kCarryNoRowStores) == 0) {
-          store_proc<Z, kNtScatterStores>(st, sl, E, ratio, n, !a.keep_node || (wk & KACC_SLOT_NEW));
+          store_proc<Z, kNtScatterStores>(st, sl, E, (1u << Z) - 1u, ratio, n, !a.keep_node || (wk & KACC_SLOT_NEW));
         }
 #pragma unroll
         for (int z = 0; z < Z; ++z) s_cE[r * Z + z] = E[z];
@@ -1862,7 +1887,7 @@
       }
     }
   }
-  uint64_t prev[kSmallBatch][Z];
+  uint32_t prev[kSmallBatch][Z];
   uint32_t contig = 0;
   auto load_batch = [&](int kb, bool from_regs) {
     contig = 0;
@@ -1872,14 +1897,14 @@
       const uint32_t pos0 = 64u * k;
       if constexpr (kRowSweep) {
         if (swept) {
-          load_row<Z>(st.proc_energy, static_cast<uint64_t>(smin) + min(pos0 + lane, span - 1), prev[g]);
+          load_proc_lo<Z>(st.proc_lo, static_cast<uint64_t>(smin) + min(pos0 + lane, span - 1), prev[g]);
           continue;
         }
       }
       if constexpr (kSweepable) {
         if (swept) {
           const uint32_t len = pos0 < span ? min(span - pos0, 64u) : 0u;
-          load_group_masked<Z, true, kNtLd>(st.proc_energy, static_cast<uint64_t>(smin) + pos0, len, smin,
+          load_proc_group<Z, true, kNtLd>(st.proc_lo, static_cast<uint64_t>(smin) + pos0, len, smin,
                                             prev[g]);
           continue;
         }
@@ -1891,12 +1916,12 @@
         const uint64_t g0 = uniform_u32(static_cast<uint32_t>(sl));
         if (__all(r < rows && sl == g0 + lane && g0 + 64 <= st.proc_slots)) {
           contig |= 1u << g;
-          load_group_masked<Z, false, kNtLd>(st.proc_energy, g0, 64u, g0, prev[g]);
+          load_proc_group<Z, false, kNtLd>(st.proc_lo, g0, 64u, g0, prev[g]);
           continue;
         }
       }
       if (r < rows && sl < st.proc_slots) {
-        load_row<Z>(st.proc_energy, sl, prev[g]);
+        load_proc_lo<Z>(st.proc_lo, sl, prev[g]);
       } else {
 #pragma unroll
         for (int z = 0; z < Z; ++z) prev[g][z] = 0;
@@ -2099,21 +2124,21 @@
           if (e == 0xffffu) continue;
           uint64_t E[Z];
           const double ratio = attribute_proc<Z>(a, s_d[e & 0x7fffu], (e & 0x8000u) != 0, prev[g], E);
-          store_proc<Z, kNT>(st, static_cast<uint64_t>(smin) + pos, E, ratio, n, !a.keep_node || (e & 0x8000u));
+          store_proc<Z, kNT>(st, static_cast<uint64_t>(smin) + pos, E, proc_known<Z>(a, (e & 0x8000u) != 0), ratio, n,
+                             !a.keep_node || (e & 0x8000u));
           continue;
         }
       }
       if constexpr (kSweepable) {
         if (swept) {
           const uint32_t len = pos0 < span ? min(span - pos0, 64u) : 0u;
-          attribute_group_masked<Z, kNT, true>(a, sh, s_d, s_w, s_inv, pos0, static_cast<uint64_t>(smin) + pos0,
-                                               len, prev[g], st.proc_energy, st.proc_ratio, st.proc_node, n);
+          attribute_proc_group<Z, kNT, true>(a, st, s_d, s_w, s_inv, pos0, static_cast<uint64_t>(smin) + pos0, len,
+                                             prev[g], n);
           continue;
         }
         if (contig & (1u << g)) {
-          attribute_group_masked<Z, kNT, false>(a, sh, s_d, s_w, s_inv, pos0,
-                                                uniform_u32(s_w[pos0] & KACC_SLOT_MASK), 64u, prev[g],
-                                                st.proc_energy, st.proc_ratio, st.proc_node, n);
+          attribute_proc_group<Z, kNT, false>(a, st, s_d, s_w, s_inv, pos0,
+                                              uniform_u32(s_w[pos0] & KACC_SLOT_MASK), 64u, prev[g], n);
           continue;
         }
       }
@@ -2131,7 +2156,8 @@
       }
       uint64_t E[Z];
       const double ratio = attribute_proc<Z>(a, s_d[r], (wk & KACC_SLOT_NEW) != 0, prev[g], E);
-      store_proc<Z, kNT && kNtScatterStores>(st, sl, E, ratio, n, !a.keep_node || (wk & KACC_SLOT_NEW));
+      store_proc<Z, kNT && kNtScatterStores>(st, sl, E, proc_known<Z>(a, (wk & KACC_SLOT_NEW) != 0), ratio, n,
+                                             !a.keep_node || (wk & KACC_SLOT_NEW));
     }
   };
   attr_batch(0);
@@ -2423,7 +2449,7 @@
       d[u] = in ? (kNtLd ? __builtin_nontemporal_load(dcpu + r) : dcpu[r]) : 0.0;
       w[u] = in ? (kNtLd ? __builtin_nontemporal_load(pslot + r) : pslot[r]) : 0xffffffffu;
     }
-    uint64_t prev[kR][Z];
+    uint32_t prev[kR][Z];
     uint32_t contig = 0;
     if constexpr ((V & kVarSkipProcs) == 0) {
 #pragma unroll
@@ -2435,12 +2461,12 @@
                             s0 + 64 <= st.proc_slots;
           if (__all(mine)) {
             contig |= 1u << u;
-            load_group_masked<Z, false, kNtLd>(st.proc_energy, s0, 64u, s0, prev[u]);
+            load_proc_group<Z, false, kNtLd>(st.proc_lo, s0, 64u, s0, prev[u]);
             continue;
           }
         }
         if (sl < st.proc_slots) {
-          load_row<Z>(st.proc_energy, sl, prev[u]);
+          load_proc_lo<Z>(st.proc_lo, sl, prev[u]);
         } else {
 #pragma unroll
           for (int z = 0; z < Z; ++z) prev[u][z] = 0;
@@ -2596,9 +2622,8 @@
         if constexpr (kT) {
           if (contig & (1u << u)) {
             const uint32_t g = r - (tid & 63);
-            attribute_group_masked<Z, kNT, false>(a, sh, s_d, s_w, nullptr, g,
-                                           uniform_u32(s_w[g] & KACC_SLOT_MASK), 64u, prev[u],
-                                           st.proc_energy, st.proc_ratio, st.proc_node, n);
+            attribute_proc_group<Z, kNT, false>(a, st, s_d, s_w, nullptr, g, uniform_u32(s_w[g] & KACC_SLOT_MASK), 64u,
+                                                prev[u], n);
             continue;
           }
         }
@@ -2611,7 +2636,8 @@
         }
         uint64_t E[Z];
         const double ratio = attribute_proc<Z>(a, s_d[r], (wk & KACC_SLOT_NEW) != 0, prev[u], E);
-        store_proc<Z, kNT && kNtScatterStores>(st, sl, E, ratio, n, !a.keep_node || (wk & KACC_SLOT_NEW));
+        store_proc<Z, kNT && kNtScatterStores>(st, sl, E, proc_known<Z>(a, (wk & KACC_SLOT_NEW) != 0), ratio, n,
+                                             !a.keep_node || (wk & KACC_SLOT_NEW));
       }
     }
     for (uint32_t j = kThreads + utid; j < nagg; j += kThreads) {
@@ -2771,6 +2797,20 @@
   }
 }
 
+__global__ __launch_bounds__(kBlock) void plane_copy_kernel(uint32_t *lo, uint64_t planes, uint64_t first,
+                                                            uint64_t count, uint64_t *dense, int to_table) {
+  for (uint64_t i = static_cast<uint64_t>(blockIdx.x) * kBlock + threadIdx.x; i < count;
+       i += static_cast<uint64_t>(gridDim.x) * kBlock) {
+    const uint64_t e = first + i;
+    if (to_table) {
+      lo[e] = static_cast<uint32_t>(dense[i]);
+      lo[planes + e] = static_cast<uint32_t>(dense[i] >> 32);
+    } else {
+      dense[i] = (static_cast<uint64_t>(lo[planes + e]) << 32) | lo[e];
+    }
+  }
+}
+
 }
 
 namespace {
@@ -2821,6 +2861,8 @@
 #define fail kacc_fail
 
 bool pod_paired(int t) { return t == KACC_T_POD_ENERGY || t == KACC_T_POD_POWER; }
+bool split_planes(int t) { return t == KACC_T_PROC_ENERGY; }
+bool indirect(int t) { return kTables[t].derived || pod_paired(t) || split_planes(t); }
 
 uint64_t table_count(const kacc_config &c, int t);
 size_t table_alloc_bytes(const kacc_ctx *ctx, int t) {
@@ -2862,7 +2904,8 @@
   s.node_usage_ratio = (double *)T(KACC_T_NODE_USAGE_RATIO);
   s.node_cpu_delta = (double *)T(KACC_T_NODE_CPU_DELTA);
   s.node_status = (uint32_t *)T(KACC_T_NODE_STATUS);
-  s.proc_energy = (uint64_t *)T(KACC_T_PROC_ENERGY);
+  s.proc_lo = (uint32_t *)T(KACC_T_PROC_ENERGY);
+  s.proc_hi = s.proc_lo + ctx->counts[KACC_T_PROC_ENERGY];
   s.proc_ratio = (double *)T(KACC_T_PROC_RATIO);
   s.proc_node = (uint32_t *)T(KACC_T_PROC_NODE);
   s.ctr_energy = (uint64_t *)T(KACC_T_CTR_ENERGY);
@@ -3784,6 +3827,11 @@
     *dev_ptr = nullptr;
     return fail(ctx, KACC_EINVAL, "table %d is derived on read (no device storage): see kacc_table_download", (int)t);
   }
+  if (split_planes(t)) {
+    *dev_ptr = nullptr;
+    return fail(ctx, KACC_EINVAL, "table %d is stored as low / high 32-bit planes (no u64 rows to point at): see "
+                                  "kacc_table_read / kacc_table_download", (int)t);
+  }
   *dev_ptr = ctx->tables[t];
   return KACC_OK;
 }
@@ -3807,7 +3855,7 @@
   if (!count) return KACC_OK;
   KACC_HIP(ctx, hipSetDevice(ctx->device));
   KACC_HIP(ctx, hipStreamSynchronize(ctx->stream));
-  if (kTables[t].derived || pod_paired(t)) {
+  if (indirect(t)) {
     void *tmp = nullptr;
     KACC_HIP(ctx, hipMalloc(&tmp, count * 8));
     hipError_t e = hipSuccess;
@@ -3818,7 +3866,7 @@
       if (rc == KACC_OK && e == hipSuccess) e = hipMemcpy(host, tmp, count * 8, hipMemcpyDeviceToHost);
     } else {
       e = hipMemcpy(tmp, host, count * 8, hipMemcpyHostToDevice);
-      if (e == hipSuccess) rc = kacc_internal_pod_scatter(ctx, t, first, count, tmp, ctx->stream);
+      if (e == hipSuccess) rc = kacc_internal_table_scatter(ctx, t, first, count, tmp, ctx->stream);
       if (rc == KACC_OK && e == hipSuccess) e = hipStreamSynchronize(ctx->stream);
     }
     (void)hipFree(tmp);
@@ -3852,7 +3900,7 @@
   if (!count) return KACC_OK;
   KACC_HIP(ctx, hipSetDevice(ctx->device));
   hipStream_t st = stream ? static_cast<hipStream_t>(stream) : ctx->stream;
-  if (kTables[t].derived || pod_paired(t)) return kacc_internal_dense_range(ctx, t, first, count, dev_dst, st);
+  if (indirect(t)) return kacc_internal_dense_range(ctx, t, first, count, dev_dst, st);
   KACC_HIP(ctx, hipMemcpyAsync(dev_dst, static_cast<const char *>(ctx->tables[t]) + first * kTables[t].elem,
                                count * kTables[t].elem, hipMemcpyDeviceToDevice, st));
   return KACC_OK;
@@ -4028,7 +4076,7 @@
   if (kacc_derived_kind(t) >= 0) return kacc_internal_derived_power(ctx, t, first, count, static_cast<double *>(out), stream);
   if (!count) return KACC_OK;
   hipStream_t st = stream ? static_cast<hipStream_t>(stream) : ctx->stream;
-  if (!pod_paired(t)) {
+  if (!pod_paired(t) && !split_planes(t)) {
     KACC_HIP(ctx, hipMemcpyAsync(out, static_cast<const char *>(ctx->tables[t]) + first * 8, count * 8,
                                  hipMemcpyDeviceToDevice, st));
     return KACC_OK;
@@ -4036,6 +4084,13 @@
   KACC_HIP(ctx, hipSetDevice(ctx->device));
   const uint64_t blocks = (count + kacc::kBlock - 1) / kacc::kBlock;
   (void)hipGetLastError();
+  if (split_planes(t)) {
+    hipLaunchKernelGGL(kacc::plane_copy_kernel, dim3(static_cast<uint32_t>(std::min<uint64_t>(blocks, 65536))),
+                       dim3(kacc::kBlock), 0, st, static_cast<uint32_t *>(ctx->tables[t]), ctx->counts[t], first, count,
+                       static_cast<uint64_t *>(out), 0);
+    KACC_HIP(ctx, hipGetLastError());
+    return KACC_OK;
+  }
   hipLaunchKernelGGL(kacc::pod_pair_copy_kernel, dim3(static_cast<uint32_t>(std::min<uint64_t>(blocks, 65536))),
                      dim3(kacc::kBlock), 0, st, static_cast<uint64_t *>(ctx->tables[t]), ctx->cfg.zones, first, count,
                      static_cast<uint64_t *>(out), 0);
@@ -4043,13 +4098,20 @@
   return KACC_OK;
 }
 
-int kacc_internal_pod_scatter(kacc_ctx *ctx, int t, uint64_t first, uint64_t count, const void *in, void *stream) {
-  if (!ctx || !pod_paired(t)) return KACC_EINVAL;
+int kacc_internal_table_scatter(kacc_ctx *ctx, int t, uint64_t first, uint64_t count, const void *in, void *stream) {
+  if (!ctx || !(pod_paired(t) || split_planes(t))) return KACC_EINVAL;
   if (!count) return KACC_OK;
   KACC_HIP(ctx, hipSetDevice(ctx->device));
   hipStream_t st = stream ? static_cast<hipStream_t>(stream) : ctx->stream;
   const uint64_t blocks = (count + kacc::kBlock - 1) / kacc::kBlock;
   (void)hipGetLastError();
+  if (split_planes(t)) {
+    hipLaunchKernelGGL(kacc::plane_copy_kernel, dim3(static_cast<uint32_t>(std::min<uint64_t>(blocks, 65536))),
+                       dim3(kacc::kBlock), 0, st, static_cast<uint32_t *>(ctx->tables[t]), ctx->counts[t], first, count,
+                       const_cast<uint64_t *>(static_cast<const uint64_t *>(in)), 1);
+    KACC_HIP(ctx, hipGetLastError());
+    return KACC_OK;
+  }
   hipLaunchKernelGGL(kacc::pod_pair_copy_kernel, dim3(static_cast<uint32_t>(std::min<uint64_t>(blocks, 65536))),
                      dim3(kacc::kBlock), 0, st, static_cast<uint64_t *>(ctx->tables[t]), ctx->cfg.zones, first, count,
                      const_cast<uint64_t *>(static_cast<const uint64_t *>(in)), 1);
diff --git a/kepler_amd/csrc/kacc_format.hip b/kepler_amd/csrc/kacc_format.hip
--- a/kepler_amd/csrc/kacc_format.hip
+++ b/kepler_amd/csrc/kacc_format.hip
@@ -705,7 +705,7 @@
   kacc::fmt::Args a{};
   a.src = static_cast<const char *>(ctx->tables[t]) + first * 8;
   double *derived = nullptr;
-  if (kacc_derived_kind(t) >= 0 || t == KACC_T_POD_ENERGY || t == KACC_T_POD_POWER) {
+  if (kacc_indirect_table(t)) {
     KACC_HIP(ctx, hipMallocAsync(reinterpret_cast<void **>(&derived), count * 8, st));
     const int rc = kacc_internal_dense_range(ctx, t, first, count, derived, st);
     if (rc != KACC_OK) {
@@ -786,7 +786,7 @@
   char *tmp = nullptr;
   auto al = [](uint64_t x) { return (x + 255) & ~255ull; };
   const uint64_t off_len = 1024, off_scan = al(off_len + 8 * (lines + 1));
-  const bool derived = t >= 0 && (kacc_derived_kind(t) >= 0 || t == KACC_T_POD_ENERGY || t == KACC_T_POD_POWER);
+  const bool derived = t >= 0 && kacc_indirect_table(t);
   const uint64_t off_derived = al(off_scan + scan_bytes);
   KACC_HIP(ctx, hipMallocAsync(reinterpret_cast<void **>(&tmp), derived ? off_derived + 8 * count * Z : off_scan + scan_bytes,
                                st));
diff --git a/kepler_amd/csrc/kacc_internal.hpp b/kepler_amd/csrc/kacc_internal.hpp
--- a/kepler_amd/csrc/kacc_internal.hpp
+++ b/kepler_amd/csrc/kacc_internal.hpp
@@ -52,8 +52,8 @@
 
 extern "C" int kacc_internal_dense_range(kacc_ctx *ctx, int t, uint64_t first, uint64_t count, void *out,
                                          void *stream);
-extern "C" int kacc_internal_pod_scatter(kacc_ctx *ctx, int t, uint64_t first, uint64_t count, const void *in,
-                                         void *stream);
+extern "C" int kacc_internal_table_scatter(kacc_ctx *ctx, int t, uint64_t first, uint64_t count, const void *in,
+                                           void *stream);
 
 extern "C" uint64_t kacc_internal_scan_tiles(uint64_t n);
 extern "C" int kacc_internal_scan_u64(kacc_ctx *ctx, const uint64_t *in, uint64_t n, uint64_t *tile_sum,
diff --git a/kepler_amd/csrc/kacc_packer.hip b/kepler_amd/csrc/kacc_packer.hip
--- a/kepler_amd/csrc/kacc_packer.hip
+++ b/kepler_amd/csrc/kacc_packer.hip
@@ -198,8 +198,8 @@
 
 template <int Z>
 __global__ __launch_bounds__(kThreads) void unpack_kernel(uint32_t n, const uint32_t *w, const uint32_t *dest,
-                                                          uint64_t cap, const uint64_t *te, const double *tp,
-                                                          uint32_t stride, const ProcDerive pd, uint64_t *oe,
+                                                          uint64_t cap, const EnergyTab te, const double *tp,
+                                                          const ProcDerive pd, uint64_t *oe,
                                                           double *op, uint32_t *err) {
   const uint32_t i = blockIdx.x * kThreads + threadIdx.x;
   if (i >= n) return;
@@ -211,8 +211,8 @@
   }
 #pragma unroll
   for (int z = 0; z < Z; ++z) {
-    oe[o + z] = te[s * stride + z];
-    op[o + z] = tp ? tp[s * stride + z] : proc_power(pd, s, z);
+    oe[o + z] = energy_word(te, s * te.stride + z);
+    op[o + z] = tp ? tp[s * te.stride + z] : proc_power(pd, s, z);
   }
 }
 
@@ -304,14 +304,14 @@
                        : kind == KACC_KIND_CTR ? ctx->cfg.ctr_slots
                        : kind == KACC_KIND_VM ? ctx->cfg.vm_slots
                                               : ctx->cfg.pod_slots;
-  const uint64_t *e = static_cast<const uint64_t *>(ctx->tables[te]);
+  const kacc::EnergyTab e = kacc_energy_tab(ctx, kind);
   const double *p = kind == KACC_KIND_POD ? static_cast<const double *>(ctx->tables[te + 1]) : nullptr;
   const kacc::ProcDerive pd = kacc_derive(ctx, kind);
   const uint32_t grid = (n + kacc::unpack::kThreads - 1) / kacc::unpack::kThreads;
   (void)hipGetLastError();
 #define KACC_UNPACK(Z)                                                                                          \
   hipLaunchKernelGGL((kacc::unpack::unpack_kernel<Z>), dim3(grid), dim3(kacc::unpack::kThreads), 0, st, n,   \
-                     slot_words, dest, cap, e, p, kind == KACC_KIND_POD ? 2 * Z : Z, pd, out_energy, out_power,   \
+                     slot_words, dest, cap, e, p, pd, out_energy, out_power,                                      \
                      ctx->d_err)
   switch (ctx->cfg.zones) {
     case 1: KACC_UNPACK(1); break;
diff --git a/kepler_amd/csrc/kacc_top.hip b/kepler_amd/csrc/kacc_top.hip
--- a/kepler_amd/csrc/kacc_top.hip
+++ b/kepler_amd/csrc/kacc_top.hip
@@ -27,8 +27,7 @@
 };
 
 struct Args {
-  const uint64_t *words;
-  uint32_t stride;
+  EnergyTab tab;
   uint32_t mode;
   ProcDerive pd;
   uint32_t zone;
@@ -69,7 +68,7 @@
   if constexpr (kSrc == kDerived) {
     return static_cast<uint64_t>(__double_as_longlong(g.live ? a.pd.ratio[s] * g.aP : 0.0));
   } else {
-    return a.words[s * a.stride];
+    return energy_word(a.tab, s * a.tab.stride + a.zone);
   }
 }
 
@@ -257,7 +256,7 @@
           if constexpr (kSrc == kDerived)
             v[u] = static_cast<uint64_t>(__double_as_longlong(a.pd.ratio[in ? sl : 0]));
           else
-            v[u] = a.words[(in ? sl : 0) * a.stride];
+            v[u] = energy_word(a.tab, (in ? sl : 0) * a.tab.stride + a.zone);
         }
       }
       if (bad) atomicOr(a.err, kErrTop);
@@ -305,7 +304,7 @@
         if (a.mode == kDerived)
           v = slot_value<kDerived>(a, sl, node_guard(a.pd, node, a.zone));
         else
-          v = a.words[static_cast<uint64_t>(sl) * a.stride];
+          v = energy_word(a.tab, static_cast<uint64_t>(sl) * a.tab.stride + a.zone);
       }
       a.out_row[o + j] = row;
       if (a.out_slot) a.out_slot[o + j] = sl;
@@ -355,8 +354,8 @@
   } else {
     const bool power = t == KACC_T_POD_POWER;
     a->mode = power ? kacc::top::kStored : kacc::top::kEnergy;
-    a->words = static_cast<const uint64_t *>(ctx->tables[t]) + zone;
-    a->stride = kind == KACC_KIND_POD ? 2 * Z : Z;
+    a->tab = kacc_energy_tab(ctx, static_cast<kacc_kind>(kind));
+    if (power) a->tab.base = ctx->tables[t];
   }
   a->zone = zone;
   a->n_nodes = rows->n_nodes;
diff --git a/kepler_amd/csrc/kacc_tracker.hip b/kepler_amd/csrc/kacc_tracker.hip
--- a/kepler_amd/csrc/kacc_tracker.hip
+++ b/kepler_amd/csrc/kacc_tracker.hip
@@ -15,7 +15,7 @@
 constexpr uint32_t kErrCap = 1u << 10;
 
 struct Args {
-  const uint64_t *tab_e;
+  EnergyTab tab_e;
   const double *tab_p;
   ProcDerive pd;
   uint64_t min_e;
@@ -60,7 +60,7 @@
     if (lane < m0) {
       slot = a.term_slot[b0 + c0 + lane];
       key = a.term_key[b0 + c0 + lane];
-      e = a.tab_e[static_cast<uint64_t>(slot) * a.tab_stride + z0];
+      e = energy_word(a.tab_e, static_cast<uint64_t>(slot) * a.tab_e.stride + z0);
       pass = e >= a.min_e && !(full && e <= min_full);
     }
     if (__ballot(pass) == 0) continue;
@@ -153,7 +153,7 @@
     if (lane < m && rank < new_size) {
       a.set_key[base + rank] = skey;
       for (uint32_t z = 0; z < Z; ++z) {
-        a.set_e[(base + rank) * Z + z] = a.tab_e[static_cast<uint64_t>(sslot) * a.tab_stride + z];
+        a.set_e[(base + rank) * Z + z] = energy_word(a.tab_e, static_cast<uint64_t>(sslot) * a.tab_e.stride + z);
         a.set_p[(base + rank) * Z + z] =
             a.tab_p ? a.tab_p[static_cast<uint64_t>(sslot) * a.tab_stride + z] : proc_power(a.pd, sslot, z);
       }
@@ -298,13 +298,9 @@
 
 namespace {
 
-void kind_tables(const kacc_ctx *ctx, kacc_kind k, const uint64_t **e, const double **p) {
-  const int base = k == KACC_KIND_PROC ? KACC_T_PROC_ENERGY
-                   : k == KACC_KIND_CTR ? KACC_T_CTR_ENERGY
-                   : k == KACC_KIND_VM ? KACC_T_VM_ENERGY
-                                       : KACC_T_POD_ENERGY;
-  *e = static_cast<const uint64_t *>(ctx->tables[base]);
-  *p = k == KACC_KIND_POD ? static_cast<const double *>(ctx->tables[base + 1]) : nullptr;
+void kind_tables(const kacc_ctx *ctx, kacc_kind k, kacc::EnergyTab *e, const double **p) {
+  *e = kacc_energy_tab(ctx, k);
+  *p = k == KACC_KIND_POD ? static_cast<const double *>(ctx->tables[KACC_T_POD_POWER]) : nullptr;
 }
 
 kacc::trk::Args tracker_args(const kacc_tracker *t) {
```

After: 55.25 billion proc-attr/s, median of 6. No clear change (+0.7%).
